# Enigmatisms/AdaPT

Measured on AMD Instinct MI355X. Metric: Msamples/s (W*H*spp/s), unidirectional MIS path tracing, higher is better.
Workload: dtype f32

## Files before the change

adapt_amd/_lib.py:

```python
from __future__ import annotations

import ctypes as C
import os

_HERE = os.path.dirname(os.path.abspath(__file__))
LIB_PATHS = {"fast": os.environ.get("ADAPT_MI_LIB") or os.path.join(_HERE, "libadapt_mi.so"),
             "exact": os.environ.get("ADAPT_MI_LIB_EXACT") or os.path.join(_HERE, "libadapt_mi_exact.so")}
_variant = "exact" if os.environ.get("APT_EXACT", "0") not in ("", "0") else "fast"
LIB_PATH = LIB_PATHS[_variant]

f32p = C.POINTER(C.c_float)
i32p = C.POINTER(C.c_int32)
u32p = C.POINTER(C.c_uint32)
u8p = C.POINTER(C.c_uint8)
f64p = C.POINTER(C.c_double)
APT_N_KERNELS = 5
KERNEL_NAMES = ("generate", "extend", "shade", "shadow", "finalize")


class AptError(RuntimeError):
    pass


class SceneDesc(C.Structure):
# ... 51 lines not shown
    "apt_bvh_wide_export": (C.c_int, [C.c_void_p, u32p, i32p]),
    "apt_bvh_wide_frame": (C.c_int, [C.c_void_p, f32p, f32p]),
    "apt_bvh_free": (None, [C.c_void_p]),
    "apt_bvh_build_device": (C.c_int, [f32p, C.c_int32, i32p, C.c_int32, C.c_int32, C.c_int32, C.POINTER(C.c_void_p), i32p]),
    "apt_bvh_build_linear": (C.c_int, [f32p, C.c_int32, i32p, i32p, C.c_int32, f32p, f32p, C.POINTER(C.c_void_p)]),
    "apt_linear_bvh_counts": (C.c_int, [C.c_void_p, i32p, i32p]),
    "apt_linear_bvh_export": (C.c_int, [C.c_void_p, f32p, f32p, i32p, i32p]),
    "apt_linear_bvh_free": (None, [C.c_void_p]),
    "apt_scene_create": (C.c_int, [C.POINTER(SceneDesc), C.c_int32, C.POINTER(C.c_void_p)]),
    "apt_scene_destroy": (None, [C.c_void_p]),
    "apt_scene_bvh_builder": (C.c_int, [C.c_void_p, i32p]),
    "apt_renderer_create": (C.c_int, [C.c_void_p, C.POINTER(RenderCfg), C.POINTER(C.c_void_p)]),
    "apt_renderer_destroy": (None, [C.c_void_p]),
    "apt_render": (C.c_int, [C.c_void_p, C.c_int32]),
    "apt_synchronize": (C.c_int, [C.c_void_p]),
    "apt_tile_shape": (C.c_int, [C.c_void_p, i32p, i32p]),
    "apt_read_pixels": (C.c_int, [C.c_void_p, f32p]),
    "apt_get_accum": (C.c_int, [C.c_void_p, f32p, i32p]),
    "apt_set_accum": (C.c_int, [C.c_void_p, f32p, C.c_int32]),
    "apt_reset": (C.c_int, [C.c_void_p]),
    "apt_read_transient": (C.c_int, [C.c_void_p, f32p]),
    "apt_set_transient": (C.c_int, [C.c_void_p, f32p]),
    "apt_read_path_lengths": (C.c_int, [C.c_void_p, f32p]),
    "apt_set_path_lengths": (C.c_int, [C.c_void_p, f32p]),
    "apt_read_light_groups": (C.c_int, [C.c_void_p, f32p]),
    "apt_set_light_groups": (C.c_int, [C.c_void_p, f32p]),
    "apt_relight": (C.c_int, [C.c_void_p, f32p, f32p]),
    "apt_read_sample_counts": (C.c_int, [C.c_void_p, i32p, u8p]),
    "apt_read_moments": (C.c_int, [C.c_void_p, f64p]),
    "apt_set_adaptive_state": (C.c_int, [C.c_void_p, i32p, f64p, u8p]),
    "apt_render_aov": (C.c_int, [C.c_void_p, C.c_int32, C.c_int32]),
    "apt_read_aov": (C.c_int, [C.c_void_p, f32p]),
    "apt_set_aov": (C.c_int, [C.c_void_p, f32p]),
    "apt_clear_aov": (C.c_int, [C.c_void_p]),
    "apt_denoise": (C.c_int, [C.c_void_p, C.POINTER(DenoiseCfg), f32p, f32p]),
    "apt_get_stats": (C.c_int, [C.c_void_p, C.POINTER(Stats)]),
    "apt_device_ptr": (C.c_int, [C.c_void_p, C.POINTER(C.c_void_p), i32p]),
    "apt_stream": (C.c_int, [C.c_void_p, C.POINTER(C.c_void_p)]),
    "apt_intersect": (C.c_int, [C.c_void_p, C.c_int32, f32p, f32p, i32p, f32p, f32p]),
    "apt_occluded": (C.c_int, [C.c_void_p, C.c_int32, f32p, f32p, f32p, i32p]),
    "apt_rng_stream": (C.c_int, [C.c_int32, C.c_uint32, C.c_uint32, C.c_uint32, C.c_int32, u32p]),
    "apt_bxdf_probe": (C.c_int, [C.c_int32, C.c_int32, i32p, f32p, f32p, C.c_float, C.c_int32, C.c_uint32, f32p]),
    "apt_medium_probe": (C.c_int, [C.c_int32, C.c_int32, i32p, f32p, C.c_int32, f32p, C.c_uint32, f32p]),
    "apt_volume_probe": (C.c_int, [C.c_int32, C.c_int32, i32p, f32p, f32p, C.c_int32, f32p, C.c_uint32, f32p]),
    "apt_emitter_probe": (C.c_int, [C.c_void_p, C.c_int32, f32p, C.c_uint32, f32p]),
    "apt_texture_probe": (C.c_int, [C.c_void_p, C.c_int32, i32p, f32p, f32p]),
    "apt_surface_maps_probe": (C.c_int, [C.c_void_p, C.c_int32, i32p, f32p, f32p]),
    "apt_transient_bin_probe": (C.c_int, [C.c_int32, C.c_int32, f32p, C.c_float, C.c_float, C.c_int32, i32p]),
    "apt_renderer_info": (C.c_int, [C.c_void_p, i32p, i32p, C.POINTER(C.c_int64), i32p, C.POINTER(C.c_char_p), i32p]),
    "apt_renderer_camera_fused": (C.c_int, [C.c_void_p, i32p]),
    "apt_renderer_light_strips": (C.c_int, [C.c_void_p, i32p]),
    "apt_renderer_record_staged": (C.c_int, [C.c_void_p, i32p]),
    "apt_renderer_live_rows": (C.c_int, [C.c_void_p, i32p]),
    "apt_measure_sclk_mhz": (C.c_int, [C.c_int32, f32p]),
    "apt_last_error": (C.c_char_p, []),
    "apt_version": (C.c_char_p, []),
}

_libs = {}


def use(variant: str) -> str:
    global _variant, LIB_PATH
    if variant not in LIB_PATHS:
        raise ValueError(f"unknown build variant {variant!r}")
    prev, _variant = _variant, variant
    LIB_PATH = LIB_PATHS[variant]
    return prev


def variant() -> str:
    return _variant


def load(variant: str | None = None):
    v = variant or _variant
    if v in _libs:
        return _libs[v]
    path = LIB_PATHS[v]
    if not os.path.exists(path):
        raise AptError(f"{path} is missing: build it with `python -m adapt_amd.build` (needs hipcc); "
                       "adapt_amd has no CPU fallback")
    lib = C.CDLL(path)
    for name, (res, args) in SYMBOLS.items():
        fn = getattr(lib, name)
        fn.restype, fn.argtypes = res, args
    tag = lib.apt_version()
    overridden = os.environ.get("ADAPT_MI_LIB" if v == "fast" else "ADAPT_MI_LIB_EXACT")
    if f"arithmetic: {v}".encode() not in tag and not overridden:
        raise AptError(f"{path} reports {tag!r}: not the {v} build")
    _libs[v] = lib
    return lib


def arithmetic(lib=None) -> str:
    tag = (lib or load()).apt_version().decode()
    return "exact" if "arithmetic: exact" in tag else "fast"


def check(rc: int, what: str = "", lib=None):
    if rc != 0:
        msg = (lib or load()).apt_last_error()
        raise AptError(f"{what or 'adapt_mi'} failed ({rc}): {msg.decode() if msg else '?'}")
```

adapt_amd/csrc/api.hip:

```cpp
#include <hip/hip_runtime.h>
#include <chrono>

#include <algorithm>
#include <cmath>
#include <cstdio>
#include <cstdlib>
#include <cstring>
#include <limits>
#include <memory>
#include <string>
#include <vector>

#include "../../include/adapt_mi.h"
#include "bvh_build.hpp"
#include "shade_stage.hpp"
#include "unit_kernels.hpp"
#include "aov.hpp"
#include "volumetric.hpp"

#define APT_EXPORT extern "C" __attribute__((visibility("default")))

static thread_local std::string g_err;
static int fail(int code, const std::string& msg) { g_err = msg; return code; }
#define HIP_TRY(expr)                                                                              \
    do {                                                                                           \
        hipError_t e_ = (expr);                                                                    \
        if (e_ != hipSuccess)                                                                      \
            return fail(APT_E_HIP, std::string(#expr) + ": " + hipGetErrorString(e_));             \
    } while (0)

typedef void (*shade_fn)(DevScene, Params, Queues, Counters*, ShadeIn, int, int);
typedef void (*shade_traced_fn)(DevScene, Params, Queues, Counters*, int, int);
typedef void (*shade_cam_fn)(DevScene, Params, Queues, Counters*, const unsigned long long*);
typedef void (*shade_tr_fn)(DevScene, Params, Queues, Counters*, ShadeIn, int, int, TransQ);
struct TracedKernels { shade_traced_fn queue[2][2]; shade_cam_fn cam[2]; };
struct ShadeVariant { int bm, sm; const char* name; shade_fn fn; shade_tr_fn transient; TracedKernels traced; };
#if APT_FAST
#define APT_FLAT_FN(...) __VA_ARGS__
#else
#define APT_FLAT_FN(...) nullptr
#endif
#define APT_TRACED_PLAIN(BM, SM, TEX) {{{APT_FLAT_FN(k_shade_traced<BM, SM, TEX>), nullptr}, {nullptr, nullptr}}, {APT_FLAT_FN(k_shade_traced_cam<BM, SM, TEX>), nullptr}}
#define APT_TRACED_LEAN(BM, SM, TEX) {{{APT_FLAT_FN(k_shade_traced_lean<BM, SM>), nullptr}, {APT_FLAT_FN(k_shade_traced_lean_staged<BM, SM>), APT_FLAT_FN(k_shade_traced_lean_staged_live<BM, SM>)}}, \
                                      {APT_FLAT_FN(k_shade_traced_lean_cam<BM, SM>), APT_FLAT_FN(k_shade_traced_lean_cam_live<BM, SM>)}}
#define APT_SHADE_VARIANT(BM, SM, TEX, NAME, TRACED) {BM, SM, NAME, k_shade<BM, SM, TEX>, k_shade_tr<BM, SM, TEX>, APT_TRACED_##TRACED(BM, SM, TEX)}
static const ShadeVariant kShadeVariants[] = {
    APT_SHADE_VARIANT(APT_BX_LAMBERTIAN, APT_SRC_POINT, 0, "lambertian/point", LEAN),
    APT_SHADE_VARIANT(APT_BX_BLINN_PHONG | APT_BX_LAMBERTIAN, APT_SRC_POINT_AREA, 0, "phong+lambertian/point+area", PLAIN),
    APT_SHADE_VARIANT(APT_BX_BLINN_PHONG | APT_BX_LAMBERTIAN | APT_BX_MIRROR | APT_BX_GLASS, APT_SRC_POINT_AREA, 0, "phong+lambertian+mirror+glass/point+area", PLAIN),
    APT_SHADE_VARIANT(APT_BX_ALL, APT_SRC_ALL, 0, "all models", PLAIN),
};
static const ShadeVariant kTexturedShade = APT_SHADE_VARIANT(APT_BX_ALL, APT_SRC_ALL, 1, "all models + image textures", PLAIN);
struct ClassDef { int mask; const char* name; int group, slot, vgroup, vslot; };
constexpr int APT_N_GROUPS = 2, APT_N_VGROUPS = 3, APT_VGROUP_SLOTS = 4;
static constexpr ClassDef kClass[] = {
    {APT_BX_LAMBERTIAN, "lambertian", 0, 0, 0, 0},
    {APT_BX_BLINN_PHONG, "blinn-phong", 1, 0, 2, 0},
    {APT_BX_OREN_NAYAR, "oren-nayar", 1, 1, 0, 1},
    {APT_BX_MIRROR | APT_BX_GLASS | APT_BX_NULL, "delta", 0, 1, 0, 2},
    {APT_BX_MOD_PHONG, "mod-phong", 1, 4, 2, 1},
    {APT_BX_FRESNEL_BLEND, "fresnel-blend", 1, 5, 2, 2},
    {APT_BX_THIN_COAT, "thin-coat", 1, 2, 1, 1},
    {APT_BX_LAMBERT_TRANS, "lambert-trans", 0, 2, 0, 3},
    {APT_BX_MICROFACET, "microfacet", 1, 3, 1, 2},
    {APT_BX_BLINN_PHONG | APT_BX_NO_LOBE, "blinn-phong(no lobe)", 0, 3, 2, 3},
};
constexpr int APT_N_CLASS_DEFS = sizeof(kClass) / sizeof(kClass[0]), APT_CLASS_PHONG = 1, APT_CLASS_PHONG_NO_LOBE = APT_N_CLASS_DEFS - 1;
static constexpr int group_mask(int g, int s) { for (const ClassDef& c : kClass) if (c.group == g && c.slot == s) return c.mask; return 0; }
static constexpr int vgroup_mask(int g, int s) {
    for (const ClassDef& c : kClass) if (c.vgroup == g && c.vslot == s) return c.mask & ~APT_BX_NO_LOBE;
    return (g == 1 && s == 0) ? APT_VEV_MEDIUM_CODE : 0;
}
static constexpr bool class_masks_partition_all() {
    int all = 0;
    for (int c = 0; c < APT_N_CLASS_DEFS - 1; c++) { if (all & kClass[c].mask) return false; all |= kClass[c].mask; }
    return all == APT_BX_ALL;
}
static constexpr bool class_slots_ok() {
    for (int a = 0; a < APT_N_CLASS_DEFS; a++) {
        const ClassDef& c = kClass[a];
        if ((unsigned)c.group >= APT_N_GROUPS || (unsigned)c.slot >= APT_GROUP_SLOTS || (unsigned)c.vgroup >= APT_N_VGROUPS || (unsigned)c.vslot >= APT_VGROUP_SLOTS) return false;
        if (c.vgroup == 1 && c.vslot == 0) return false;
        for (int b = 0; b < a; b++)
            if ((kClass[b].group == c.group && kClass[b].slot == c.slot) || (kClass[b].vgroup == c.vgroup && kClass[b].vslot == c.vslot)) return false;
    }
    return true;
}
static_assert(class_masks_partition_all(), "every surface model belongs to exactly one of the classes in front of the lobe-free one");
static_assert(class_slots_ok(), "every class needs a member slot of its own, inside APT_GROUP_SLOTS / APT_VGROUP_SLOTS, in a surface and in a volumetric group");
static_assert(kClass[APT_CLASS_PHONG].mask == APT_BX_BLINN_PHONG && kClass[APT_CLASS_PHONG_NO_LOBE].mask == (APT_BX_BLINN_PHONG | APT_BX_NO_LOBE), "APT_CLASS_PHONG / APT_CLASS_PHONG_NO_LOBE name these entries");
static int class_of(int is_bsdf, int type, bool no_lobe) {
    const int bit = bx_bit(is_bsdf, type);
    if (bit == APT_BX_BLINN_PHONG && no_lobe) return APT_CLASS_PHONG_NO_LOBE;
    for (int c = 0; c < APT_N_CLASS_DEFS - 1; c++) if (kClass[c].mask & bit) return c;
    return 0;
}
static int group_emitter_set(int src_mask) { return (src_mask & ~APT_SRC_POINT_AREA) == 0 ? 0 : ((src_mask & ~APT_SRC_POINT_SPOT) == 0 ? 2 : 1); }
static int vgroup_emitter_set(int src_mask) { return (src_mask & ~APT_SRC_POINT_AREA) == 0 ? 0 : 1; }
// ... 74 lines not shown
    std::vector<uint8_t> obj_null;
    float box_min[3] = {1e3f, 1e3f, 1e3f}, box_max[3] = {-1e3f, -1e3f, -1e3f};
    int n_classes = 0;
    int class_def[APT_N_CLASS_DEFS] = {};
    int n_prims = 0, n_objects = 0, n_sources = 0, max_obj_prims = 0;
    int bx_mask = 0, src_mask = 0;
    bool has_aabb = false;
    bool has_sweep = false;
};

struct EventPair { hipEvent_t a, b; int kernel; bool own_a; };

struct Lane {
    hipStream_t stream = nullptr;
    DevBuf pool, counters, ovf;
    Queues q{};
    hipEvent_t fin = nullptr;
    LdsPlan plan{};
    Counters* cnt() const { return counters.as<Counters>(); }
};

enum Pipeline { PIPE_STAGED, PIPE_SORTED, PIPE_TRACED, PIPE_VOLUMETRIC };

enum SplitMode { SPLIT_NONE, SPLIT_TRANSIENT, SPLIT_LENGTHS, SPLIT_LIGHTS };
struct SplitWords {
    const char* noun;
    const char* subject;
    bool plural;
    const char* field;
    const char* tag;
};
static constexpr SplitWords kSplit[] = {
    {"", "", false, "", ""},
    {"transient bins", "transient rendering", false, "transient_bins", " [transient]"},
    {"path-length planes", "path-length images", true, "path_lengths", " [path lengths]"},
    {"light-group planes", "light groups", true, "light_groups", " [light groups]"},
};

struct apt_renderer {
    const apt_scene* scene = nullptr;
    apt_render_cfg cfg{};
    Params par{};
    int n_cols = 0, npix = 0, spp_batch = 1;
    int cnt = 0;
    std::vector<Lane> lanes;
    int n_lanes = 1;
    hipStream_t stream() const { return lanes[0].stream; }
    DevBuf accum, scratch, pix_key;
    DevBuf cam_strips;
    int record_stage = 0;
    shade_traced_fn traced_fn = nullptr;
    int live_rows = 0;
    shade_cam_fn traced_cam_fn = nullptr;
    int camera_fuse = 0;
    int light_strips = 0;
    Counters host_counters{};
    int grid_small = 0, grid_trace = 0, nq = APT_MAX_NQ;
    const ShadeVariant* shade = nullptr;
    int trace_mode = TRACE_BVH;
    int trace_nt = BLOCK;
    int trace_items = BLOCK;
    Pipeline pipeline = PIPE_STAGED;
    int dyn_fetch = 0;
    bool tile_ok = false;
    extend_fn extend = nullptr, fix = nullptr;
    int ovf_levels = 0;
    int n_cq = 0;
    int vev_single = 0;
    vev_shade_fn vev_all = nullptr;
    bool vev_live[APT_MAX_CLASSES] = {};
    vev_group_fn vgroup_fn[APT_N_VGROUPS] = {};
    int vgroup_cls[APT_N_VGROUPS][APT_VGROUP_SLOTS] = {};
    group_fn group_fn_[APT_N_GROUPS] = {};
    int group_cls[APT_N_GROUPS][APT_GROUP_SLOTS] = {};
    std::string shade_name;
    size_t lds_bytes = 0, lds_bytes_any = 0;
    int grid_shadow = 0;
    int grid_fix = 0;
    int grid_vshadow = 0;
    int vshadow_nt = BLOCK;
    int vshadow_mode = TRACE_BVH;
    size_t vshadow_lds = 0;
    std::vector<EventPair> pending;
    std::vector<hipEvent_t> free_events;
    std::vector<std::pair<hipStream_t, hipEvent_t>> chain;
    double kernel_ms[APT_N_KERNELS] = {0, 0, 0, 0, 0};
    int64_t launches[APT_N_KERNELS] = {0, 0, 0, 0, 0};
    double render_ms = 0.0;
    hipEvent_t ev_r0 = nullptr, ev_r1 = nullptr;
    bool render_pending = false;
    SplitMode split_mode = SPLIT_NONE;
    bool split() const { return split_mode != SPLIT_NONE; }
    TransQ tq{};
    DevBuf tr_pool;
    DevBuf split_cells;
    group_tr_fn group_tr_[APT_N_GROUPS] = {};
    DevBuf lg_aux;
    int adaptive = 0;
    AdaptQ aq{};
    DevBuf ad_n, ad_s2, ad_active, ad_live;
    std::vector<uint8_t> ad_start;
    uint32_t* ad_live_host = nullptr;
    hipEvent_t ad_ev = nullptr;
    bool ad_pending = false;
    uint32_t n_live = 0;
    DevBuf aov_rec, aov_sum;
// ... 427 lines not shown
        B = (int)((32u << 20) / (uint32_t)r->npix); if (B < 1) B = 1; if (B > 1024) B = 1024;
        const size_t n_cq = c.volumetric ? (size_t)sc->n_classes + 1 : ((sc->n_classes >= 2 && sc->n_classes <= APT_MAX_CLASSES) ? (size_t)sc->n_classes : 1);
        while (B > 1 && n_cq * subcap_of(B) * nq >= ((size_t)1 << 28)) B--;
        size_t free_b = 0, total_b = 0;
        if (hipMemGetInfo(&free_b, &total_b) == hipSuccess) {
            const size_t per_path = 4u * (64u + 16u * n_cq + 11u * (size_t)std::max(1, c.num_shadow_ray));
            while (B > 1 && (size_t)r->npix * (size_t)B * (size_t)r->n_lanes * per_path > free_b / 3) B = (B + 1) / 2;
        }
    }
    r->spp_batch = B;
    const int S = c.num_shadow_ray;
    const size_t subcap = subcap_of(B), cap = subcap * nq;
    if (cap >= (1ull << 31)) { return fail(APT_E_INVALID, "apt_renderer_create: batch too large (spp_per_batch * pixels must stay below 2^31)"); }
    Params& p = r->par;
    memcpy(p.cam_r, c.cam_r, sizeof(p.cam_r)); memcpy(p.cam_t, c.cam_t, sizeof(p.cam_t));
    p.inv_focal = c.inv_focal; p.half_w = c.half_w; p.half_h = c.half_h;
    p.W = c.width; p.H = c.height; p.n_cols = r->n_cols; p.npix = r->npix;
    p.band_width = c.band_width; p.rank = c.rank; p.world = c.world_size;
    p.do_crop = c.do_crop; p.sx = c.start_x; p.ex = c.end_x; p.sy = c.start_y; p.ey = c.end_y;
    p.max_bounce = c.max_bounce; p.S = S; p.inv_S = (S > 0) ? 1.f / (float)S : 1.f;
    p.use_rr = c.use_rr; p.use_mis = c.use_mis; p.anti_alias = c.anti_alias; p.stratified = c.stratified; p.two_sides = c.brdf_two_sides;
    p.rr_bounce_th = c.rr_bounce_th; p.rr_threshold = c.rr_threshold; p.seed = c.seed; p.cap = (uint32_t)cap; p.subcap = (uint32_t)subcap; p.nq = r->nq;
    p.inv_ns = 1.f / (float)sc->n_sources; p.inv_ns1 = (sc->n_sources > 1) ? 1.f / (float)(sc->n_sources - 1) : 1.f;
    p.volumetric_flat = c.volumetric ? 1 : 0; p.fix_par = 0;
    p.pix_bits = 0; while ((1u << p.pix_bits) < (uint32_t)r->npix) p.pix_bits++;
    if (((uint64_t)B << p.pix_bits) > (1ull << 32)) { return fail(APT_E_INVALID, "apt_renderer_create: spp_per_batch x pixels does not fit the 32-bit path id"); }
    std::vector<uint32_t> key((size_t)r->npix);
    for (int lp = 0; lp < r->npix; lp++) {
        const int lc = lp / c.height, j = lp % c.height, lb = lc / c.band_width, w_ = lc % c.band_width;
        const int i = (lb * c.world_size + c.rank) * c.band_width + w_;
        key[(size_t)lp] = (uint32_t)(i * c.height + j);
    }
    hipError_t e_ = upload(r->pix_key, key);
    if (e_ != hipSuccess) { return fail(APT_E_HIP, std::string("upload pix_key: ") + hipGetErrorString(e_)); }
    p.pix_key = r->pix_key.as<uint32_t>();
    return APT_OK;
}

static int small_scene_sweep(const apt_renderer* r) { return (r->tile_ok && r->scene->max_obj_prims >= APT_SWEEP_LIST_MIN) ? TRACE_TILE : TRACE_SWEEP; }
static void pick_traversal(apt_renderer* r) {
    const apt_scene* sc = r->scene;
    r->tile_ok = sc->has_aabb && sc->has_sweep && sc->n_objects <= APT_TILE_MAX_OBJECTS && sc->n_prims < 65536 &&
                 APT_TILE_LDS_BYTES(APT_TILE_NT, sc->n_objects) <= 160 * 1024;
    const bool can[4] = {true, sc->has_aabb && sc->has_sweep, r->tile_ok, sc->has_flat};
    r->trace_mode = sc->has_flat ? TRACE_FLAT
                  : (sc->n_prims <= APT_SWEEP_MAX_PRIMS && can[TRACE_SWEEP]) ? small_scene_sweep(r) : TRACE_BVH;
    if (const char* force = getenv("APT_TRAVERSAL"))
        for (int m = TRACE_BVH; m <= TRACE_FLAT; m++) if (!strcmp(force, kTraversalName[m]) && can[m]) r->trace_mode = m;
    r->dyn_fetch = (r->trace_mode == TRACE_BVH) ? 1 : 0;
    if (const char* f = getenv("APT_DYN_FETCH")) r->dyn_fetch = (atoi(f) != 0 && r->trace_mode == TRACE_BVH) ? 1 : 0;
}

static void pick_traced_kernels(apt_renderer* r) {
    const TracedKernels& t = r->shade->traced;
    const bool traced = r->pipeline == PIPE_TRACED;
    const bool want_stage = !(getenv("APT_RECORD_STAGE") && atoi(getenv("APT_RECORD_STAGE")) == 0);
    const bool want_live = !(getenv("APT_LIVE_ROWS") && atoi(getenv("APT_LIVE_ROWS")) == 0);
    r->record_stage = (traced && want_stage && t.queue[1][0] != nullptr) ? 1 : 0;
    r->live_rows = (traced && want_live && t.queue[1][1] != nullptr && t.cam[1] != nullptr) ? 1 : 0;
    r->traced_fn = t.queue[r->record_stage][r->record_stage & r->live_rows];
    r->traced_cam_fn = t.cam[r->live_rows];
}

static int pick_shading(apt_renderer* r) {
    const apt_scene* sc = r->scene;
    const apt_render_cfg& c = r->cfg;
    Params& p = r->par;
    const int S = c.num_shadow_ray;
    for (const ShadeVariant& v : kShadeVariants)
        if ((sc->bx_mask & ~v.bm) == 0 && (sc->src_mask & ~v.sm) == 0) { r->shade = &v; break; }
    if (!r->shade) { return fail(APT_E_INVALID, "apt_renderer_create: scene uses a material or emitter type the kernels do not know"); }
    const bool textured = sc->dev.tex_i != nullptr;
    if (textured) r->shade = &kTexturedShade;
    const char* env_sorted = getenv("APT_SORTED");
    const bool fits = sc->n_classes <= APT_MAX_CLASSES;
    const bool sorted = !textured && fits && (env_sorted ? (atoi(env_sorted) != 0 && sc->n_classes >= 1) : sc->n_classes >= 2);
    bool want_traced = true;
    if (const char* f = getenv("APT_FUSED")) {
        const int want = atoi(f);
        if (want == 1) fprintf(stderr, "adapt_mi: APT_FUSED=1 (light samples only traced in place) was retired in round 5; running the staged pipeline (APT_FUSED=0). Use 2 for rays traced in place.\n");
        want_traced = want >= 2;
    }
    const bool can_trace = r->trace_mode == TRACE_FLAT && S == 1 && !r->split() && r->shade->traced.queue[0][0] != nullptr;
    r->pipeline = c.volumetric ? PIPE_VOLUMETRIC : (sorted ? PIPE_SORTED : ((can_trace && want_traced) ? PIPE_TRACED : PIPE_STAGED));
    p.traced = (r->pipeline == PIPE_TRACED) ? 1 : 0;
    pick_traced_kernels(r);
    p.nee_vm = (!c.volumetric && !r->split() && r->trace_mode == TRACE_FLAT && S > 1) ? 1 : 0;
    p.l_planes = (!p.nee_vm && S >= 2 && S <= 4) ? S : 1;
    if (r->pipeline == PIPE_VOLUMETRIC) {
        if (c.max_bounce > 255) { return fail(APT_E_INVALID, "apt_renderer_create: the volumetric tracer keeps the bounce count in 8 bits (max_bounce <= 255)"); }
        if (!sc->has_aabb) { return fail(APT_E_INVALID, "apt_renderer_create: the volumetric tracer needs the object boxes (world bound)"); }
        r->vev_single = (textured || sc->n_classes + 1 > APT_MAX_CLASSES) ? 1 : 0;
        const int n_surf = r->vev_single ? 1 : sc->n_classes;
        r->n_cq = n_surf + 1;
        const int smi = vgroup_emitter_set(sc->src_mask), vi = sc->has_volume ? 1 : 0;
        r->vev_all = kVEventAll[smi][vi];
        for (size_t o = 0; o < sc->obj_class.size(); o++)
            if (!sc->obj_null[o]) r->vev_live[r->vev_single ? 0 : sc->obj_class[o]] = true;
        r->vev_live[n_surf] = true;
        for (int g = 0; g < APT_N_VGROUPS; g++) { r->vgroup_fn[g] = kVGroup[smi][vi][g]; for (int k = 0; k < APT_VGROUP_SLOTS; k++) r->vgroup_cls[g][k] = -1; }
        if (!r->vev_single) for (int c = 0; c < n_surf; c++) if (r->vev_live[c]) r->vgroup_cls[kClass[sc->class_def[c]].vgroup][kClass[sc->class_def[c]].vslot] = c;
        r->vgroup_cls[1][0] = n_surf;
        for (int a = 0; a < 3; a++) {
            p.w_min[a] = std::min(c.cam_t[a], sc->box_min[a]) - 0.1f; p.w_max[a] = std::max(c.cam_t[a], sc->box_max[a]) + 0.1f;
        }
        r->shade_name = std::string(sc->has_volume ? "volumetric + grid volume, sorted by event: medium | " : "volumetric, sorted by event: medium | ");
        if (r->vev_single) r->shade_name += "all surface models";
        else for (int c = 0; c < sc->n_classes; c++) r->shade_name += std::string(c ? "+" : "") + kClass[sc->class_def[c]].name;
// ... 61 lines not shown
                                 uint64_t* masks, int32_t masks_cap, int32_t* n_strips, int32_t* n_pairs) {
    if (!prims || !obj_info || !cfg || n_prims <= 0 || n_objects <= 0 || !n_strips || !n_pairs) return fail(APT_E_INVALID, "apt_camera_strips: bad argument");
    apt_render_cfg c = *cfg;
    if (c.world_size <= 0) { c.world_size = 1; c.rank = 0; }
    if (c.band_width <= 0) c.band_width = c.width;
    if (c.width <= 0 || c.height <= 0 || c.rank < 0 || c.rank >= c.world_size || owned_columns(c) <= 0) return fail(APT_E_INVALID, "apt_camera_strips: bad film or rank");
    std::vector<float> st, tb; int cn[7];
    if (apt::build_flat(prims, n_prims, obj_info, n_objects, nullptr, st, tb, cn) != 0) return fail(APT_E_INVALID, "apt_camera_strips: obj_info range outside the primitive array");
    std::vector<uint64_t> m;
    if (apt::camera_strips(prims, n_prims, st, tb, cn, cam_film(c), cull != 0, m) != 0) return fail(APT_E_INVALID, "apt_camera_strips: bad record or film");
    *n_strips = (int32_t)m.size();
    *n_pairs = (cn[0] + cn[1] + 1) / 2 + (cn[2] + cn[3] + 1) / 2 + (cn[4] + cn[5] + 1) / 2 + (cn[6] + 1) / 2;
    if (masks) { if (masks_cap < (int32_t)m.size()) return fail(APT_E_INVALID, "apt_camera_strips: masks buffer too small"); memcpy(masks, m.data(), m.size() * 8); }
    return APT_OK;
}

APT_EXPORT int apt_light_strips(const float* prims, int32_t n_prims, const int32_t* obj_info, int32_t n_objects, const int32_t* src_i, const float* src_f, int32_t n_sources,
                                const apt_render_cfg* cfg, int32_t cull, uint64_t* masks, int32_t masks_cap, int32_t* n_strips, int32_t* n_pairs, float* origin_slack) {
    if (!prims || !obj_info || !src_i || !src_f || !cfg || n_prims <= 0 || n_objects <= 0 || n_sources <= 0 || !n_strips) return fail(APT_E_INVALID, "apt_light_strips: bad argument");
    apt_render_cfg c = *cfg;
    if (c.world_size <= 0) { c.world_size = 1; c.rank = 0; }
    if (c.band_width <= 0) c.band_width = c.width;
    if (c.width <= 0 || c.height <= 0 || c.rank < 0 || c.rank >= c.world_size || owned_columns(c) <= 0) return fail(APT_E_INVALID, "apt_light_strips: bad film or rank");
    std::vector<float> st, tb, pts, pr; std::vector<int32_t> off, tab8, np; std::vector<uint8_t> kp; int cn[7];
    if (apt::build_flat(prims, n_prims, obj_info, n_objects, nullptr, st, tb, cn) != 0) return fail(APT_E_INVALID, "apt_light_strips: obj_info range outside the primitive array");
    apt::emitter_points(prims, obj_info, n_objects, src_i, src_f, n_sources, pts, off);
    if (apt::flat_occluders(prims, n_prims, st, tb, cn, pts.data(), off.data(), n_sources, true, pr, tab8, kp) != 0) return fail(APT_E_INVALID, "apt_light_strips: bad record");
    std::vector<uint64_t> m; double slack = 0.0;
    if (apt::light_strips(prims, n_prims, st, tb, cn, cam_film(c), pts.data(), off.data(), n_sources, kp.data(), cull != 0, m, np, &slack) != 0) return fail(APT_E_INVALID, "apt_light_strips: bad record or film");
    *n_strips = (int32_t)((owned_columns(c) * c.height + 63) / 64);
    if (n_pairs) memcpy(n_pairs, np.data(), np.size() * 4);
    if (origin_slack) *origin_slack = (float)slack;
    if (masks) { if (masks_cap < (int32_t)m.size()) return fail(APT_E_INVALID, "apt_light_strips: masks buffer too small"); memcpy(masks, m.data(), m.size() * 8); }
    return APT_OK;
}

static int make_lanes(apt_renderer* r) {
    const apt_scene* sc = r->scene;
    const Params& p = r->par;
    const size_t cap = p.cap, sh_subcap = (size_t)p.subcap * (size_t)(p.S > 0 ? p.S : 1), sh_cap = sh_subcap * (size_t)p.nq;
    const int ncls = r->n_cq;
    if (cap >= ((size_t)1 << 30) || sh_cap >= ((size_t)1 << 30)) { return fail(APT_E_INVALID, "apt_renderer_create: batch too large (queue capacity must stay below 2^30 slots)"); }
    if (r->pipeline == PIPE_TRACED && cap >= ((size_t)1 << 28)) { return fail(APT_E_INVALID, "apt_renderer_create: batch too large (rays traced in place address 16-byte slots with 32-bit byte offsets: capacity must stay below 2^28)"); }
    if ((size_t)ncls * cap >= ((size_t)1 << 28)) { return fail(APT_E_INVALID, "apt_renderer_create: batch too large (packed class queues address 16-byte slots with 32-bit byte offsets: classes x capacity must stay below 2^28)"); }
    const bool staged = r->pipeline != PIPE_TRACED, tr_uv = !staged && (sc->dev.has_vn || sc->dev.tex_i != nullptr);
    const bool walk_lists = r->pipeline == PIPE_VOLUMETRIC && sc->has_null_surface;
    const size_t l_planes = (size_t)p.l_planes;
    auto carve = [&](float* base, Queues& q) -> size_t {
        size_t at = 0;
        auto take = [&](size_t n) { float* x = base ? base + at : nullptr; at += n; return x; };
        for (int k = 0; k < 2; k++) { q.ray_o[k] = (k == 0 || staged) ? take(3 * cap) : nullptr; q.ray_d[k] = (k == 0 || staged) ? take(3 * cap) : nullptr; }
        q.hit_t = take(cap); q.hit_prim = (int*)take(cap); q.hit_u = take(cap); q.hit_v = take(cap);
        for (int k = 0; k < 2; k++) {
            for (int a = 0; a < 4; a++) q.tr[k][a] = staged ? nullptr : (float4*)take(4 * cap);
            q.tr_uv[k] = tr_uv ? (float2*)take(2 * cap) : nullptr;
        }
        q.tr_ncls = staged ? 0 : 1; q.tr_stage_top = staged ? 0 : 1;
        q.fix_ext = (r->trace_mode == TRACE_FLAT) ? (uint32_t*)take(cap) : nullptr; q.fix_sh = (r->trace_mode == TRACE_FLAT) ? (uint32_t*)take(sh_cap) : nullptr;
        for (int k = 0; k < 2; k++) { q.thr[k] = staged ? take(3 * cap) : nullptr; q.id[k] = staged ? (uint32_t*)take(cap) : nullptr; q.meta[k] = staged ? (uint32_t*)take(cap) : nullptr; q.pdf[k] = staged ? take(cap) : nullptr; }
        q.L = take(4 * cap * l_planes);
        q.sh_o = take(3 * sh_cap); q.sh_d = take(3 * sh_cap); q.sh_tmax = take(sh_cap); q.sh_c = take(3 * sh_cap); q.sh_id = (uint32_t*)take(sh_cap);
        q.sh_cap = (uint32_t)sh_cap; q.sh_subcap = (uint32_t)sh_subcap;
        q.sh_walk[0] = walk_lists ? (uint32_t*)take(sh_cap) : nullptr; q.sh_walk[1] = walk_lists ? (uint32_t*)take(sh_cap) : nullptr;
        q.n_classes = ncls;
        for (int a = 0; a < 4; a++) q.cq[a] = (ncls > 0 && staged) ? (float4*)take(4 * cap * (size_t)ncls) : nullptr;
        return at;
    };
    Queues sizing{};
    const size_t pool_bytes = carve(nullptr, sizing) * 4;
    r->lanes.resize((size_t)r->n_lanes);
    hipError_t e;
    for (Lane& ln : r->lanes) {
        if ((e = ln.pool.alloc(pool_bytes)) != hipSuccess || (e = hipMemset(ln.pool.p, 0, pool_bytes)) != hipSuccess || (e = ln.counters.alloc(sizeof(Counters))) != hipSuccess)
            return fail(APT_E_NOMEM, std::string(&ln == &r->lanes[0] ? "queue pool: " : "queue pool (lane): ") + hipGetErrorString(e));
        carve(ln.pool.as<float>(), ln.q);
    }
    HIP_TRY(hipDeviceSynchronize());
    if ((e = r->accum.alloc((size_t)r->npix * 12)) != hipSuccess || (e = r->scratch.alloc((size_t)r->npix * 12)) != hipSuccess) { return fail(APT_E_NOMEM, std::string("framebuffer: ") + hipGetErrorString(e)); }
    for (Lane& ln : r->lanes) {
        HIP_TRY(hipStreamCreateWithFlags(&ln.stream, hipStreamNonBlocking));
        HIP_TRY(hipEventCreateWithFlags(&ln.fin, hipEventDisableTiming));
        HIP_TRY(hipMemsetAsync(ln.counters.p, 0, sizeof(Counters), ln.stream));
    }
    HIP_TRY(hipMemsetAsync(r->accum.p, 0, (size_t)r->npix * 12, r->stream()));
    HIP_TRY(hipEventCreate(&r->ev_r0)); HIP_TRY(hipEventCreate(&r->ev_r1));
    return APT_OK;
}

static void transient_window(TransQ& t, int32_t n_bins, float min_time, float interval) {
    t.n_bins = n_bins; t.min_time = min_time; t.interval = interval;
    t.max_time = (float)((double)min_time + (double)interval * (double)n_bins);
}

static int adaptive_restart(apt_renderer* r) {
    HIP_TRY(hipMemsetAsync(r->ad_n.p, 0, r->ad_n.bytes, r->stream()));
    HIP_TRY(hipMemsetAsync(r->ad_s2.p, 0, r->ad_s2.bytes, r->stream()));
    HIP_TRY(hipMemcpyAsync(r->ad_active.p, r->ad_start.data(), r->ad_start.size(), hipMemcpyHostToDevice, r->stream()));
    HIP_TRY(hipStreamSynchronize(r->stream()));
    r->n_live = 0;
    for (uint8_t a : r->ad_start) r->n_live += a;
    r->ad_pending = false;
    return APT_OK;
}
static int make_adaptive(apt_renderer* r) {
    if (!r->adaptive) return APT_OK;
    const apt_render_cfg& c = r->cfg;
    const size_t n = (size_t)r->npix;
// ... 341 lines not shown
                    }
                }
                is.cur ^= 1;
            }
            return APT_OK;
        };
        for (Issued& is : round) if (int rc = iterate(is, std::max(1, is.p.max_bounce))) return rc;
        for (Issued& is : round) {
            Lane& ln = *is.ln;
            if (r->scene->has_null_surface) {
                Counters* cnt = ln.cnt();
                unsigned long long live = 0;
                for (int k = 0; k < 4096; k++) {
                    unchain(r, ln.stream); HIP_TRY(hipMemcpyAsync(r->host_counters.n_active[is.cur], cnt->n_active[is.cur], sizeof(cnt->n_active[is.cur]), hipMemcpyDeviceToHost, ln.stream));
                    HIP_TRY(hipStreamSynchronize(ln.stream));
                    live = 0;
                    for (int sq = 0; sq < nq; sq++) live += r->host_counters.n_active[is.cur][sq * CNT_PAD];
                    if (!live) break;
                    if (int rc = iterate(is, 2)) return rc;
                }
                if (live) return fail(APT_E_STATE, "apt_render: paths still crossing null surfaces after 8192 extra iterations (a closed loop of null surfaces?)");
            }
            if (int rc = finalize_batch(r, ln, is.p, prev_fin)) return rc;
        }
    }
    return APT_OK;
}

static int render_surface(apt_renderer* r, int32_t n_spp) {
    const DevScene& sc = r->scene->dev;
    const int nq = r->nq;
    int done = 0, batch = 0;
    hipEvent_t prev_fin = nullptr;
    const int batch_cap = lane_batch(r, n_spp);
    while (done < n_spp) {
        const int B = (n_spp - done < batch_cap) ? (n_spp - done) : batch_cap;
        Lane& ln = r->lanes[(size_t)(batch % r->n_lanes)];
        hipStream_t st = ln.stream;
        const Queues& q = ln.q;
        Counters* cnt = ln.cnt();
        Params p = r->par; p.cnt_base = r->cnt; p.spp_batch = B;
        const size_t total = (size_t)r->npix * (size_t)B;
        if (int rc = begin_batch(r, ln)) return rc;
#if APT_FAST
        if (r->pipeline == PIPE_TRACED) {
            const unsigned long long* strips = r->cam_strips.as<unsigned long long>();
            int cur = 0, b0 = 0;
            if (r->camera_fuse) {
                { LaunchTimer t(r, APT_K_SHADE, st); hipLaunchKernelGGL(r->traced_cam_fn, dim3(grid_for(total, r->grid_small, nq)), dim3(BLOCK), 0, st, sc, p, q, cnt, strips); }
                { LaunchTimer t(r, APT_K_SHADE, st); hipLaunchKernelGGL(r->traced_fn, dim3(r->grid_fix), dim3(BLOCK), 0, st, sc, p, q, cnt, 0, 0); }
                cur = 1; b0 = 1;
            } else {
                LaunchTimer t(r, APT_K_GENERATE, st);
                if (r->adaptive) hipLaunchKernelGGL(k_generate_trace_ad, dim3(grid_for(total, r->grid_small, 1)), dim3(BLOCK), 0, st, sc, p, q, cnt, (const uint8_t*)r->aq.active, strips);
                else hipLaunchKernelGGL(k_generate_trace, dim3(grid_for(total, r->grid_small, 1)), dim3(BLOCK), 0, st, sc, p, q, cnt, strips);
            }
            for (int b = b0; b < p.max_bounce; b++) {
                { LaunchTimer t(r, APT_K_SHADE, st); hipLaunchKernelGGL(r->traced_fn, dim3(grid_for(total, r->grid_small, nq)), dim3(BLOCK), 0, st, sc, p, q, cnt, cur, b); }
                cur ^= 1;
            }
            if (p.max_bounce > 0) { LaunchTimer t(r, APT_K_SHADOW, st, false); hipLaunchKernelGGL(r->fix, dim3(r->grid_fix), dim3(BLOCK), 0, st, sc, p, q, cnt, cur, (const uint32_t*)cnt->n_active[cur], ln.plan); }
        } else
#endif
        {
        {
            LaunchTimer t(r, APT_K_GENERATE, st);
            if (r->adaptive) hipLaunchKernelGGL(k_generate_ad, dim3(grid_for(total, r->grid_small, 1)), dim3(BLOCK), 0, st, p, q, cnt, (const uint8_t*)r->aq.active);
            else hipLaunchKernelGGL(k_generate, dim3(grid_for(total, r->grid_small, 1)), dim3(BLOCK), 0, st, p, q, cnt);
        }
        auto bin = [&](int settled) {
            LaunchTimer t(r, APT_K_FINALIZE, st, false);
            const dim3 grid(grid_for((size_t)r->npix, r->grid_small, 1));
            float4* cells = r->split_cells.as<float4>();
            switch (r->split_mode) {
                case SPLIT_TRANSIENT: hipLaunchKernelGGL(k_bin_transient, grid, dim3(BLOCK), 0, st, p, q, r->tq, r->accum.as<float>()); break;
                case SPLIT_LENGTHS: hipLaunchKernelGGL(k_bin_lengths, grid, dim3(BLOCK), 0, st, p, q, r->tq, cells, settled, r->accum.as<float>()); break;
                case SPLIT_LIGHTS: hipLaunchKernelGGL(k_bin_lights, grid, dim3(BLOCK), 0, st, p, q, r->tq, cells, r->scene->n_sources, r->lg_aux.as<unsigned int>(), r->accum.as<float>()); break;
                case SPLIT_NONE: break;
            }
        };
        int cur = 0;
        for (int b = 0; b < p.max_bounce; b++) {
            if (r->dyn_fetch && !(p.S > 0)) { unchain(r, st); HIP_TRY(hipMemsetAsync(cnt->n_work[0], 0, sizeof(cnt->n_work[0]), st)); }
            launch_extend(r, ln, p, total, cur);
            if (r->split() && r->trace_mode == TRACE_FLAT && b > 0) bin(b - 1);
            if (r->pipeline != PIPE_SORTED) {
                ShadeIn in = {q.ray_o[cur], q.ray_d[cur], q.thr[cur], q.id[cur], q.meta[cur], q.pdf[cur],
                              q.hit_t, q.hit_prim, q.hit_u, q.hit_v, (const uint32_t*)cnt->n_active[cur]};
                LaunchTimer t(r, APT_K_SHADE, st);
                if (r->split()) hipLaunchKernelGGL(r->shade->transient, dim3(grid_for(total, r->grid_small, nq)), dim3(BLOCK), 0, st, sc, p, q, cnt, in, cur, b, r->tq);
                else hipLaunchKernelGGL(r->shade->fn, dim3(grid_for(total, r->grid_small, nq)), dim3(BLOCK), 0, st, sc, p, q, cnt, in, cur, b);
            } else {
                for (int g = 0; g < APT_N_GROUPS; g++) {
                    GroupIn gi; bool any = false;
                    for (int k = 0; k < APT_GROUP_SLOTS; k++) { const int c = r->group_cls[g][k]; gi.cls[k] = c; gi.counts[k] = c >= 0 ? (const uint32_t*)cnt->n_cls[c] : nullptr; any = any || c >= 0; }
                    if (!any) continue;
                    LaunchTimer t(r, APT_K_SHADE, st);
                    if (r->split()) hipLaunchKernelGGL(r->group_tr_[g], dim3(grid_for(total, r->grid_small, nq)), dim3(BLOCK), 0, st, sc, p, q, cnt, gi, cur, b, r->tq);
                    else hipLaunchKernelGGL(r->group_fn_[g], dim3(grid_for(total, r->grid_small, nq)), dim3(BLOCK), 0, st, sc, p, q, cnt, gi, cur, b);
                }
                if (p.S <= 0) { unchain(r, st); HIP_TRY(hipMemsetAsync(cnt->n_cls, 0, sizeof(cnt->n_cls), st)); }
            }
            if (p.S > 0 && r->dyn_fetch) {
                LaunchTimer t(r, APT_K_SHADOW, st); hipLaunchKernelGGL(k_shadow_dyn, dim3(grid_for(total * (size_t)p.S, r->grid_shadow, nq, r->trace_items)), dim3(r->trace_nt), r->lds_bytes_any, st, sc, p, q, cnt, ln.plan);
            } else if (p.S > 0) {
                p.fix_par = cur;
                LaunchTimer t(r, APT_K_SHADOW, st); hipLaunchKernelGGL(kShadow[r->trace_mode], dim3(grid_for(total * (size_t)p.S, r->grid_shadow, nq, r->trace_items)), dim3(r->trace_nt), r->lds_bytes_any, st, sc, p, q, cnt, ln.plan);
            }
// ... 522 lines not shown
}
APT_EXPORT int apt_surface_maps_probe(const apt_scene* sc, int32_t n, const int32_t* prim_first, const float* bary, float* out7) {
    if (!sc || n <= 0 || !prim_first || !bary || !out7) return fail(APT_E_INVALID, "apt_surface_maps_probe: bad argument");
    if (!sc->dev.tex_i) return fail(APT_E_INVALID, "apt_surface_maps_probe: the scene has no textures");
    for (int k = 0; k < n; k++)
        if (const int p = prim_first[2 * (size_t)k]; p < 0 || p >= sc->n_prims) return fail(APT_E_INVALID, "apt_surface_maps_probe: no such primitive");
    Probe pr; if (int rc = pr.begin("apt_surface_maps_probe", sc->device, (size_t)n * 28)) return rc;
    HIP_TRY(upload(pr.in[0], prim_first, 2 * (size_t)n)); HIP_TRY(upload(pr.in[1], bary, 2 * (size_t)n));
    hipLaunchKernelGGL(k_surface_maps_probe, dim3((n + 63) / 64), dim3(64), 0, 0, sc->dev, n, pr.in[0].as<int>(), pr.in[1].as<float>(), pr.out.as<float>());
    return pr.finish(out7);
}
APT_EXPORT int apt_measure_sclk_mhz(int32_t device, float* mhz) {
    if (!mhz) return fail(APT_E_INVALID, "apt_measure_sclk_mhz: bad argument");
    if (int rc = use_device("apt_measure_sclk_mhz", device)) return rc;
    hipDeviceProp_t prop;
    HIP_TRY(hipGetDeviceProperties(&prop, device));
    const int grid = std::max(1, prop.multiProcessorCount) * 8, n_waves = grid * (BLOCK / 64);
    DevBuf out, sink;
    HIP_TRY(out.alloc((size_t)n_waves * 16)); HIP_TRY(sink.alloc(16));
    for (int pass = 0; pass < 2; pass++) {
        hipLaunchKernelGGL(k_clock_probe, dim3(grid), dim3(BLOCK), 0, 0, 20000, 1.0f, out.as<unsigned long long>(), sink.as<float>());
        HIP_TRY(hipGetLastError());
        HIP_TRY(hipDeviceSynchronize());
    }
    std::vector<unsigned long long> h((size_t)n_waves * 2);
    HIP_TRY(hipMemcpy(h.data(), out.p, h.size() * 8, hipMemcpyDeviceToHost));
    std::vector<double> r;
    for (int w = 0; w < n_waves; w++) if (h[2 * (size_t)w + 1] > 0) r.push_back(100.0 * (double)h[2 * (size_t)w] / (double)h[2 * (size_t)w + 1]);
    if (r.empty()) return fail(APT_E_STATE, "apt_measure_sclk_mhz: the wall clock did not advance");
    std::nth_element(r.begin(), r.begin() + r.size() / 2, r.end());
    *mhz = (float)r[r.size() / 2];
    return APT_OK;
}
APT_EXPORT int apt_renderer_camera_fused(const apt_renderer* r, int32_t* out) {
    if (!r || !out) return fail(APT_E_INVALID, "apt_renderer_camera_fused: null argument");
    *out = r->camera_fuse;
    return APT_OK;
}
APT_EXPORT int apt_renderer_light_strips(const apt_renderer* r, int32_t* out) {
    if (!r || !out) return fail(APT_E_INVALID, "apt_renderer_light_strips: null argument");
    *out = r->light_strips;
    return APT_OK;
}
APT_EXPORT int apt_renderer_record_staged(const apt_renderer* r, int32_t* out) {
    if (!r || !out) return fail(APT_E_INVALID, "apt_renderer_record_staged: null argument");
    *out = r->record_stage;
    return APT_OK;
}
APT_EXPORT int apt_renderer_live_rows(const apt_renderer* r, int32_t* out) {
    if (!r || !out) return fail(APT_E_INVALID, "apt_renderer_live_rows: null argument");
    *out = r->live_rows;
    return APT_OK;
}
APT_EXPORT int apt_renderer_info(const apt_renderer* r, int32_t* spp_batch, int32_t* n_subqueues, int64_t* queue_bytes, int32_t* lds_bytes, const char** shade_variant, int32_t* trace_mode) {
    if (!r) return fail(APT_E_INVALID, "apt_renderer_info: null handle");
    if (spp_batch) *spp_batch = r->spp_batch;
    if (n_subqueues) *n_subqueues = r->nq;
    if (queue_bytes) *queue_bytes = (int64_t)r->lanes[0].pool.bytes * (int64_t)r->lanes.size();
    if (lds_bytes) *lds_bytes = (int32_t)r->lds_bytes;
    if (shade_variant) *shade_variant = r->shade_name.c_str();
    if (trace_mode) *trace_mode = r->trace_mode;
    return APT_OK;
}
```

adapt_amd/csrc/shade_stage.hpp:

```cpp
#pragma once
#include "stages.hpp"

APT_D float ti_fmod(float a, float b) { float q = floorf(a / b); return a - b * q; }
APT_D f3 mix3(f3 a, f3 b, float t) { return a * (1.0f - t) + b * t; }
APT_D f3 texture_query(const DevScene& sc, int map, int obj, float u, float v) {
    const int* ti_ = sc.tex_i + 15 * obj + 5 * map; const float* tf = sc.tex_f + 6 * obj + 2 * map;
    const float w = (float)ti_[3], h = (float)ti_[4];
    const float scaled_u = ti_fmod((u * tf[0]) * w, w - 1.f), scaled_v = ti_fmod((v * tf[1]) * h, h - 1.f);
    float floor_u = floorf(scaled_u), floor_v = floorf(scaled_v);
    const float ratio_u = fmaxf(scaled_u - floor_u, 0.f), ratio_v = fmaxf(scaled_v - floor_v, 0.f);
    floor_u = fminf(fmaxf(floor_u, 0.f), w - 1.f); floor_v = fminf(fmaxf(floor_v, 0.f), h - 1.f);
    const float ceil_u = fminf(floor_u + 1.f, w - 1.f), ceil_v = fminf(floor_v + 1.f, h - 1.f);
    const int fu = (int)(floor_u + (float)ti_[1]), fv = (int)(floor_v + (float)ti_[2]), cu = (int)(ceil_u + (float)ti_[1]), cv = (int)(ceil_v + (float)ti_[2]);
    const float* img = sc.atlas[map]; const int W = sc.atlas_w[map];
    const float* r0 = img + (size_t)fv * W * 3; const float* r1 = img + (size_t)cv * W * 3;
    const f3 q_ff = ld3(r0 + 3 * fu), q_cf = ld3(r0 + 3 * cu), q_fc = ld3(r1 + 3 * fu), q_cc = ld3(r1 + 3 * cu);
    return mix3(mix3(q_ff, q_cf, ratio_u), mix3(q_fc, q_cc, ratio_u), ratio_v);
}
APT_D bool get_uv_item(const DevScene& sc, int map, int obj, int prim, float bu, float bv, f3& out) {
    if (sc.atlas[map] == nullptr || !(sc.tex_i[15 * obj + 5 * map] > -255)) return false;
    const float* uv = sc.uvs + 6 * prim;
    const float w0 = 1.f - bu - bv;
    const float gu = (uv[2] * bu + uv[4] * bv) + uv[0] * w0, gv = (uv[3] * bu + uv[5] * bv) + uv[1] * w0;
    out = texture_query(sc, map, obj, gu, gv);
    return true;
}
APT_D int surface_maps(const DevScene& sc, Hit& it, int prim, float bu, float bv, bool first_hit, f3& k_d) {
    int applied = 0; f3 tx;
    if (first_hit) {
        if (get_uv_item(sc, 1, it.obj_id, prim, bu, bv, tx)) { m33 R; rotation_between(mk3(0.f, 1.f, 0.f), it.n_g, R); it.n_s = mul(R, tx); applied |= 2; }
        if (get_uv_item(sc, 2, it.obj_id, prim, bu, bv, tx)) { it.n_s = delocalize(it.n_s, tx); applied |= 4; }
    }
    if (get_uv_item(sc, 0, it.obj_id, prim, bu, bv, tx)) { k_d = tx; applied |= 1; }
    return applied;
}

APT_D void build_hit_rec(const DevScene& sc, float4 ra, float4 rb, int prim, float t, float u, float v, f3 o, f3 d, Hit& it, int& hit_light, f3& k_d, bool with_vn = true);
APT_D void build_hit(const DevScene& sc, int prim, float t, float u, float v, f3 o, f3 d, Hit& it, int& hit_light, f3& k_d) {
    build_hit_rec(sc, sc.prim_shade[2 * prim], sc.prim_shade[2 * prim + 1], prim, t, u, v, o, d, it, hit_light, k_d);
}
APT_D void build_hit_rec(const DevScene& sc, float4 ra, float4 rb, int prim, float t, float u, float v, f3 o, f3 d, Hit& it, int& hit_light, f3& k_d, bool with_vn) {
    const int code = __float_as_int(ra.w);
    it.prim_id = prim; it.min_depth = t;
    it.obj_id = (code < 0) ? ~code : code;
    hit_light = __float_as_int(rb.x);
    k_d = mk3(rb.y, rb.z, rb.w);
    if (code < 0) {
        it.n_g = normalize((o + d * t) - mk3(ra.x, ra.y, ra.z));
        it.n_s = it.n_g;
    } else {
        it.n_g = mk3(ra.x, ra.y, ra.z);
        if (with_vn && sc.has_vn) {
            const float4 v0 = sc.vnormals[3 * prim], v1 = sc.vnormals[3 * prim + 1], v2 = sc.vnormals[3 * prim + 2];
            it.n_s = (mk3(v0.x, v0.y, v0.z) * (1.f - u - v) + mk3(v1.x, v1.y, v1.z) * u) + mk3(v2.x, v2.y, v2.z) * v;
        } else it.n_s = it.n_g;
    }
}
APT_D void build_hit(const DevScene& sc, int prim, float t, float u, float v, f3 o, f3 d, Hit& it) {
    int light; f3 kd; build_hit(sc, prim, t, u, v, o, d, it, light, kd);
}

#if APT_FAST
APT_D void fix_prologue(const DevScene& sc, const Params& p, const Queues& q, Counters* cnt, int cur, int sq, int bounce) {
    const uint32_t epoch = (uint32_t)bounce + 1u;
    const int ncls = q.tr_ncls;
    uint32_t* n_def_p = &cnt->n_tr[bounce % 3][ncls][sq * CNT_PAD]; uint32_t* n_sh_p = &cnt->n_fix_sh[cur ^ 1][sq * CNT_PAD];
    const uint32_t n_def = __hip_atomic_load(n_def_p, __ATOMIC_RELAXED, __HIP_MEMORY_SCOPE_AGENT), n_sh = min(__hip_atomic_load(n_sh_p, __ATOMIC_RELAXED, __HIP_MEMORY_SCOPE_AGENT), q.sh_subcap);
    __builtin_amdgcn_fence(__ATOMIC_ACQUIRE, "workgroup");
    uint32_t old = __hip_atomic_load(&cnt->fix_claim[sq * CNT_PAD], __ATOMIC_RELAXED, __HIP_MEMORY_SCOPE_AGENT);
    if (old < epoch) {
        if ((n_def | n_sh) == 0u) return;
        if (lane_id() == 0) old = atomicMax(&cnt->fix_claim[sq * CNT_PAD], epoch);
        old = (uint32_t)__builtin_amdgcn_readlane((int)old, 0);
    }
    if (old >= epoch) {
        while (__hip_atomic_load(&cnt->fix_done[sq * CNT_PAD], __ATOMIC_ACQUIRE, __HIP_MEMORY_SCOPE_AGENT) < epoch) __builtin_amdgcn_s_sleep(16);
        return;
    }
    const uint32_t qbase = (uint32_t)sq * p.subcap, sh_qbase = (uint32_t)sq * q.sh_subcap;
    const bool need_uv = sc.has_vn || sc.tex_i != nullptr;
    for (uint32_t base = 0; base < n_def; base += 64u) {
        const uint32_t li = base + lane_id(); const bool valid = li < n_def;
        const uint32_t lj = valid ? li : n_def - 1u;
        const uint32_t io = (q.tr_stage_top ? qbase + p.subcap - n_def + lj : (uint32_t)ncls * p.cap + qbase + lj) << 4;
        const float4 ra = ldq(q.tr[cur][0], io), rb = ldq(q.tr[cur][1], io), rc = ldq(q.tr[cur][2], io), rd = ldq(q.tr[cur][3], io);
        const f3 o = mk3(ra.x, ra.y, ra.z), d = mk3(rb.x, rb.y, rb.z);
        HitRec r0, r1; r0.t = r1.t = 1e7f; r0.prim = r1.prim = -1; r0.u = r0.v = r1.u = r1.v = 0.f;
        int c0, c1;
        flat_closest2(sc.flat, sc.sweep, sc.prim_class, o, d, o, d, r0, r1, c0, c1);
        if (valid && r0.prim >= 0) {
            const int oc = ncls > 1 ? c0 : 0;
            const uint32_t pos = atomicAdd(&cnt->n_tr[bounce % 3][oc][sq * CNT_PAD], 1u);
            const uint32_t slot = (uint32_t)oc * p.cap + qbase + pos, so = slot << 4;
            stq(q.tr[cur][0], so, make_float4(ra.x, ra.y, ra.z, r0.t));
            stq(q.tr[cur][1], so, make_float4(rb.x, rb.y, rb.z, __uint_as_float((__float_as_uint(rb.w) & ~0xffu) | (uint32_t)r0.prim)));
            stq(q.tr[cur][2], so, rc); stq(q.tr[cur][3], so, rd);
            if (need_uv) { float2 uv_; uv_.x = r0.u; uv_.y = r0.v; stq(q.tr_uv[cur], slot << 3, uv_); }
        } else if (valid && !(rd.x == 0.f && rd.y == 0.f && rd.z == 0.f)) {
            add_radiance(q.L, p.cap, radiance_slot(p, __float_as_uint(rc.w)), mk3(rd.x, rd.y, rd.z), true);
        }
    }
    uint32_t t_lit = 0;
    for (uint32_t base = 0; base < n_sh; base += 64u) {
        const uint32_t li = base + lane_id(); const bool valid = li < n_sh;
        const uint32_t io = (sh_qbase + (valid ? li : n_sh - 1u)) << 2;
        const f3 o = ld3q(q.sh_o, q.sh_cap, io), d = ld3q(q.sh_d, q.sh_cap, io), c = ld3q(q.sh_c, q.sh_cap, io);
        const float dist = ldq(q.sh_tmax, io); const uint32_t slot = ldq(q.sh_id, io);
        bool occ, occ_b;
        const float lim = shadow_limit(dist);
        flat_any2(sc.flat, sc.sweep, o, d, o, d, lim, lim, occ, occ_b);
        const bool weird = !(isfinite(c.x) && isfinite(c.y) && isfinite(c.z));
        const bool add = valid && (!occ || weird);
        for (unsigned long long m = __ballot(add); m != 0ull; m &= m - 1ull) {
            if ((int)lane_id() == __ffsll((long long)m) - 1) add_radiance(q.L, p.cap, slot, occ ? c * 0.f : c, true);
        }
        t_lit += (valid && !occ) ? 1u : 0u;
    }
    flush_stat(t_lit, &cnt->stats[sq][ST_LIT]);
    if (lane_id() == 0) __hip_atomic_store(n_sh_p, 0u, __ATOMIC_RELAXED, __HIP_MEMORY_SCOPE_AGENT);
    __threadfence();
    if (lane_id() == 0) __hip_atomic_store(&cnt->fix_done[sq * CNT_PAD], epoch, __ATOMIC_RELEASE, __HIP_MEMORY_SCOPE_AGENT);
}
#endif
struct ShadeArgs3 { DevScene sc; Params p; Queues q; };
typedef const __attribute__((address_space(4))) ShadeArgs3* args3_ptr;
APT_D args3_ptr kernel_args3() { return (args3_ptr)__builtin_amdgcn_kernarg_segment_ptr(); }
APT_D const ShadeArgs3* args_fresh(args3_ptr a) {
    asm volatile("" : "+s"(a));
    return (const ShadeArgs3*)a;
}
#define APT_ARGS_PHASE() (A_ = args_fresh(A0))
struct Vertex {
    f3 o, d, thr, hit_point; uint32_t id, l_off, draw0; float emission_weight;
    Hit it; int hit_light; DevBxdf bx;
};
APT_D void vertex_reset(Vertex& vx) {
    vx.o = splat3(0.f); vx.d = mk3(0.f, 0.f, 1.f); vx.thr = splat3(0.f); vx.hit_point = splat3(0.f); vx.id = 0; vx.l_off = 0; vx.draw0 = 0; vx.emission_weight = 1.0f;
    vx.it.obj_id = -1; vx.it.prim_id = -1; vx.it.n_s = vx.it.n_g = mk3(1.f, 0.f, 0.f); vx.it.min_depth = 0.f; vx.hit_light = -1;
    vx.bx.type = 1; vx.bx.is_delta = 0; vx.bx.is_bsdf = 0; vx.bx.k_d = vx.bx.k_s = vx.bx.k_g = vx.bx.mean = splat3(0.f); vx.bx.ior = 1.f;
}
template <int BM, int SM, int TEX, typename RNG>
APT_D bool open_vertex(const ShadeArgs3* A_, Vertex& vx, RNG& rng, int prim, f3 rec_kd, uint32_t meta, float ray_pdf, float2 uv, int bounce, const uint32_t* jitter_tail = nullptr) {
    const bool was_spec = (meta >> 24) & 1u;
    if (BM == APT_BX_LAMBERTIAN) vx.bx.k_d = rec_kd;
    else vx.bx = ld_bxdf_lane((A_->sc).bxdf + vx.it.obj_id);
    if (TEX && (A_->sc).tex_i != nullptr) surface_maps((A_->sc), vx.it, prim, uv.x, uv.y, bounce == 0, vx.bx.k_d);
    const uint32_t lp = vx.id & ((1u << (A_->p).pix_bits) - 1u), s = vx.id >> (A_->p).pix_bits;
    vx.l_off = radiance_slot((A_->p), vx.id);
    vx.draw0 = meta & 0xffffu;
    const uint32_t key0 = ((A_->p).world == 1) ? lp : ldq((A_->p).pix_key, lp << 2), ctr0 = (uint32_t)((A_->p).cnt_base + (int)s + 1);
    rng_init(rng, key0, (A_->p).seed, ctr0, vx.draw0);
    if (bounce > 0 && (A_->p).use_mis) {
// ... 81 lines not shown
    else alive = alive && !(max3(vx.thr) < 1e-4f);
    const bool relight = vx.hit_light >= 0 && (A_->sc).n_sources > 1;
    const bool have_first = jitter_tail != nullptr && (A_->p).anti_alias != 0;
    uint32_t c[4] = {0u, 0u, have_first ? jitter_tail[0] : 0u, have_first ? jitter_tail[1] : 0u};
    const bool live = window_open(rng, key0, (A_->p).seed, ctr0, vx.draw0, roulette, mx, relight, c, have_first, [alive](bool v) { return __any(v && alive) != 0; });
    if (roulette) vx.thr = vx.thr * srcp(mx + 1e-7f);
    return alive && live;
}
template <int BM, int SM, typename R>
APT_D LightSample sample_light_live(const ShadeArgs3* A_, Vertex& vx, R& rng, const EmitterGeom& geom, const DevSrc src_only, bool active) {
    LightSample ls;
    const int ns = (A_->sc).n_sources;
    int sidx = rng_int(rng);
    sidx = (ns == 1) ? 0 : pymod(sidx, ns);
    float emitter_pdf = (A_->p).inv_ns;
    if (ns <= 1) active = active && vx.hit_light < 0;
    else if (vx.hit_light >= 0) {
        sidx = rng_int(rng);
        sidx = (ns == 2) ? 0 : pymod(sidx, ns - 1);
        if (sidx >= vx.hit_light) sidx += 1;
        emitter_pdf = (A_->p).inv_ns1;
    }
    DevSrc src = src_only;
    if (ns != 1) src = (A_->sc).src[sidx];
    ls.src = sidx;
    f3 shadow_int; float direct_pdf;
    const f3 to_emitter = emitter_sample_hit<SM>(src, geom, vx.hit_point, rng, shadow_int, direct_pdf) - vx.hit_point;
    ls.dist = fnorm(to_emitter);
    ls.dir = fdiv3(to_emitter, ls.dist);
    ls.sampled = active;
    const f3 direct_spec = surface_eval<BM>(vx.bx, vx.it, vx.d, ls.dir, (A_->sc).world_ior, (A_->p).two_sides);
    ls.mis_w = 1.0f;
    if ((A_->p).use_mis && !(src.bool_bits & 0x01)) ls.mis_w = balance(emitter_pdf * direct_pdf, surface_pdf<BM>(vx.bx, vx.it, ls.dir, vx.d, (A_->sc).world_ior, (A_->p).two_sides));
    ls.poisoned = active && isnan(ls.mis_w);
    f3 c = (direct_spec * shadow_int) * ls.mis_w;
    if (ns != 1) c = fdiv3(c, emitter_pdf);
    ls.contrib = (c * (A_->p).inv_S) * vx.thr;
    ls.want = active && !ls.poisoned && !(ls.contrib.x == 0.f && ls.contrib.y == 0.f && ls.contrib.z == 0.f);
    return ls;
}
APT_D void shadow_store(const Queues& q, uint32_t so, f3 o, f3 dir, float dist, f3 contrib) {
    st3q(q.sh_o, q.sh_cap, so, o); st3q(q.sh_d, q.sh_cap, so, dir); stq(q.sh_tmax, so, dist); st3q(q.sh_c, q.sh_cap, so, contrib);
}
struct ShadeTally { uint32_t shade, shadow, poison; };
APT_D void tally_flush(const ShadeTally& t, const uint32_t* s_draws, Counters* cnt, int sq) {
    flush_uniform(t.shade, &cnt->stats[sq][ST_SHADE]);
    flush_uniform(t.shadow, &cnt->stats[sq][ST_SHADOW]);
    if (lane_id() == 0 && s_draws[threadIdx.x >> 6]) atomicAdd(&cnt->stats[sq][ST_DRAWS], (unsigned long long)s_draws[threadIdx.x >> 6]);
    flush_uniform(t.poison, &cnt->stats[sq][ST_POISON]);
}
#if APT_FAST
APT_D uint32_t row_lane(uint32_t b, uint32_t n) { return min(b + threadIdx.x, n - 1u); }
struct RecordPlanes { const float4 *a, *b, *c, *d; };
APT_D uint32_t prefetch_prim(const RecordPlanes& tr, uint32_t qbase, uint32_t b, uint32_t n) { return ldq(reinterpret_cast<const uint32_t*>(tr.b), ((qbase + row_lane(b, n)) << 4) + 12u); }
struct StagedRecord { rec4* rec; rec4* prim; };
APT_D StagedRecord staged_record_open(const ShadeArgs3* A_) {
    __shared__ rec4 s_stage[(BLOCK / 64) * 4 * 64]; __shared__ rec4 s_shade[2 * APT_FLAT_MAX_PRIMS];
    static_assert(2 * APT_FLAT_MAX_PRIMS <= BLOCK, "one shading-record word per thread");
    if ((int)threadIdx.x < 2 * min((A_->sc).n_prims, APT_FLAT_MAX_PRIMS)) { const float4 w_ = (A_->sc).prim_shade[threadIdx.x]; s_shade[threadIdx.x] = rec4{w_.x, w_.y, w_.z, w_.w}; }
    __syncthreads();
    return StagedRecord{s_stage + (threadIdx.x >> 6) * (4 * 64), s_shade};
}
APT_D void stage_row(const StagedRecord& s, const RecordPlanes& tr, uint32_t qbase, uint32_t b, uint32_t n, int bounce) {
    const uint32_t off = (qbase + row_lane(b, n)) << 4;
    stage_plane(tr.a, off, s.rec); stage_plane(tr.b, off, s.rec + 64); stage_plane(tr.c, off, s.rec + 128);
    if (bounce > 0) stage_plane(tr.d, off, s.rec + 192);
}
APT_D void staged_row_read(const StagedRecord& s, float4& a, float4& b, float4& c, float4& d, float4& ra, float4& rb) {
    rec4 sa, sb, sc_, sd, pa, pb;
    staged_read(s.rec + lane_id(), sa, sb, sc_, sd);
    staged_read2(s.prim + 2 * max(tr_prim(__float_as_uint(sb.w)), 0), pa, pb);
    a = make_float4(sa.x, sa.y, sa.z, sa.w); b = make_float4(sb.x, sb.y, sb.z, sb.w); c = make_float4(sc_.x, sc_.y, sc_.z, sc_.w); d = make_float4(sd.x, sd.y, sd.z, sd.w);
    ra = make_float4(pa.x, pa.y, pa.z, pa.w); rb = make_float4(pb.x, pb.y, pb.z, pb.w);
}
struct RowTop { unsigned long long wait, rows, loop0; };
APT_D void staged_wait_stamped(RowTop& rt, bool row) {
#ifdef APT_ROWTOP_STATS
    const unsigned long long t0_ = __builtin_amdgcn_s_memtime(); staged_wait(); rt.wait += __builtin_amdgcn_s_memtime() - t0_; rt.rows += row ? 1u : 0u;
#else
    staged_wait();
#endif
}
template <bool UNORDERED> APT_D void tally_draws(uint32_t* s_draws, uint32_t n) { if constexpr (UNORDERED) lds_add_unordered(&s_draws[threadIdx.x >> 6], n); else atomicAdd(&s_draws[threadIdx.x >> 6], n); }
APT_D void unpack_record(float4 a, float4 b, float4 c, Vertex& vx) { vx.o = mk3(a.x, a.y, a.z); vx.d = mk3(b.x, b.y, b.z); vx.thr = mk3(c.x, c.y, c.z); vx.id = __float_as_uint(c.w); }
template <int BM, int SM, int TEX, bool REC, typename RNG>
APT_D bool open_record(const ShadeArgs3* A_, Vertex& vx, RNG& rng, float4 a, float4 b, float4 c, uint32_t pm, float4 ra, float4 rb, int cur, uint32_t idx, float ray_pdf, int bounce) {
    unpack_record(a, b, c, vx);
    const int prim = tr_prim(pm);
    if (prim < 0) return false;
    f3 rec_kd; float2 uv; uv.x = uv.y = 0.f;
    if ((A_->sc).has_vn || (TEX && (A_->sc).tex_i != nullptr)) uv = ldq((A_->q).tr_uv[cur], idx << 3);
    if (REC) build_hit_rec((A_->sc), ra, rb, prim, a.w, uv.x, uv.y, vx.o, vx.d, vx.it, vx.hit_light, rec_kd);
    else build_hit((A_->sc), prim, a.w, uv.x, uv.y, vx.o, vx.d, vx.it, vx.hit_light, rec_kd);
    return open_vertex<BM, SM, TEX>(A_, vx, rng, prim, rec_kd, tr_meta(pm, (uint32_t)bounce), ray_pdf, uv, bounce);
}
template <int BM, int SM, typename RNG>
APT_D bool open_record_live(const ShadeArgs3* A_, Vertex& vx, RNG& rng, float4 a, float4 b, float4 c, float4 d, float4 ra, float4 rb, int cur, uint32_t idx, int bounce, bool alive, uint32_t* s_draws, f3& Lc) {
    if (bounce > 0) Lc = mk3(d.x, d.y, d.z);
    unpack_record(a, b, c, vx);
    const uint32_t pm = __float_as_uint(b.w); const int prim = tr_prim(pm);
    alive = alive && prim >= 0;
    f3 rec_kd; float2 uv; uv.x = uv.y = 0.f;
    if ((A_->sc).has_vn) { if (alive) uv = ldq((A_->q).tr_uv[cur], idx << 3); }
    build_hit_rec((A_->sc), ra, rb, max(prim, 0), a.w, uv.x, uv.y, vx.o, vx.d, vx.it, vx.hit_light, rec_kd);
    const bool opened = alive; alive = open_vertex_live<BM, SM>(A_, vx, rng, rec_kd, pm, bounce, alive);
    if (opened && !alive && rng.draw != vx.draw0) tally_draws<true>(s_draws, rng.draw - vx.draw0);
    return alive;
}
APT_D uint32_t cam_wave(const ShadeArgs3* A_, uint32_t pos, int q) { return (uint32_t)__builtin_amdgcn_readfirstlane((int)(pos >> 6)) * (uint32_t)(A_->p).nq + (uint32_t)q; }
APT_D uint32_t cam_path(const ShadeArgs3* A_, uint32_t id_, bool zero, uint32_t& s, int& i, int& j) {
    const uint32_t lp = id_ % (uint32_t)(A_->p).npix; s = id_ / (uint32_t)(A_->p).npix;
    local_to_global((A_->p), lp, i, j);
    if (zero) for (int pl = 0; pl < (A_->p).l_planes; pl++) stL((A_->q).L, (A_->p).cap, (id_ << 2) | (uint32_t)pl, splat3(0.f));
    return (s << (A_->p).pix_bits) | lp;
}
APT_D bool cam_sweep(const ShadeArgs3* A_, const unsigned long long* strips, uint32_t w, bool valid, f3 cam_o, f3 dir, float& c_t, int& c_idx) {
    int c_run = -1; c_t = 0.f; c_idx = -1;
    if (__any(valid)) c_idx = flat_closest1<true>((A_->sc).flat, cam_o, dir, 1e7f, c_t, c_run, camera_strip_mask((A_->p), strips, w));
    return valid && (c_run >= 0 || flat_needs_cull((A_->sc).flat, dir));
}
struct StagedRayWords { float t; int prim; float u, v, one, zero, one_d; };
template <typename Words>
APT_D void stage_camera_ray(const ShadeArgs3* A_, Counters* cnt, int q, uint32_t qbase, bool c_defer, f3 cam_o, f3 dir, uint32_t draws, uint32_t id, Words&& words) {
    if (!__any(c_defer)) return;
    const int ncls = (A_->q).tr_ncls; const uint32_t dpos = wave_append(c_defer, &cnt->n_tr[0][ncls][q * CNT_PAD]);
    if (c_defer) {
        const uint32_t slot = (A_->q).tr_stage_top ? qbase + (A_->p).subcap - 1u - dpos : (uint32_t)ncls * (A_->p).cap + qbase + dpos, so = slot << 4;
        const StagedRayWords w = words();
        stq((A_->q).tr[0][0], so, make_float4(cam_o.x, cam_o.y, cam_o.z, w.t));
        stq((A_->q).tr[0][1], so, make_float4(dir.x, dir.y, dir.z, __uint_as_float(tr_pack(w.prim, draws, false))));
        stq((A_->q).tr[0][2], so, make_float4(w.one, w.one, w.one, __uint_as_float(id)));
        stq((A_->q).tr[0][3], so, make_float4(w.zero, w.zero, w.zero, w.one_d));
        if ((A_->sc).has_vn || (A_->sc).tex_i != nullptr) { float2 uv_; uv_.x = w.u; uv_.y = w.v; stq((A_->q).tr_uv[0], slot << 3, uv_); }
    }
}
template <int BM, int SM, int TEX, bool WINDOW, typename RNG>
APT_D bool camera_vertex(const ShadeArgs3* A_, Counters* cnt, int q, uint32_t qbase, uint32_t pos, bool in_row, uint32_t cam_total, const unsigned long long* strips, Vertex& vx, RNG& rng, uint32_t* s_draws, uint32_t& t_samples, uint32_t& t_extend, bool& entry) {
    const uint32_t w = cam_wave(A_, pos, q), id_ = w * 64u + lane_id(); const bool valid = in_row && id_ < cam_total;
    f3 dir = mk3(0.f, 0.f, 1.f); uint32_t draws = 0, jitter_tail[2] = {0u, 0u};
    if (valid) { uint32_t s; int i, j; vx.id = cam_path(A_, id_, true, s, i, j); dir = camera_ray_dir((A_->p), i, j, s, draws, WINDOW ? jitter_tail : nullptr); }
    if (draws) atomicAdd(&s_draws[threadIdx.x >> 6], draws);
    const f3 cam_o = mk3((A_->p).cam_t[0], (A_->p).cam_t[1], (A_->p).cam_t[2]);
    float c_t; int c_idx, hit_cls = 0;
    const bool c_defer = cam_sweep(A_, strips, w, valid, cam_o, dir, c_t, c_idx);
    HitRec hr; hr.t = 1e7f; hr.prim = -1; hr.u = hr.v = 0.f;
    if (valid && !c_defer && c_idx >= 0) flat_resolve((A_->sc).flat, c_idx, c_t, cam_o, dir, hr, hit_cls);
    { const uint32_t nv = wave_count(valid); t_samples += nv; t_extend += nv; }
    stage_camera_ray(A_, cnt, q, qbase, c_defer, cam_o, dir, draws, vx.id, [&] {
        float one = 1.f;
        if (WINDOW) asm volatile("" : "+v"(one));
        return StagedRayWords{hr.t, hr.prim, hr.u, hr.v, 1.f, 0.f, one};
    });
    entry = valid && !c_defer; bool alive = entry && hr.prim >= 0;
    if (alive) {
        vx.o = cam_o; vx.d = dir; vx.thr = splat3(1.f);
        f3 rec_kd; float2 uv; uv.x = hr.u; uv.y = hr.v;
        build_hit((A_->sc), hr.prim, hr.t, uv.x, uv.y, vx.o, vx.d, vx.it, vx.hit_light, rec_kd);
        alive = open_vertex<BM, SM, TEX>(A_, vx, rng, hr.prim, rec_kd, tr_meta(tr_pack(hr.prim, draws, false), 0u), 1.f, uv, 0, WINDOW ? jitter_tail : nullptr);
    }
    return alive;
}
template <int BM, int SM, bool WINDOW, typename RNG>
APT_D bool camera_vertex_live(const ShadeArgs3* A_, Counters* cnt, int q, uint32_t qbase, uint32_t pos, bool in_row, uint32_t cam_total, const unsigned long long* strips, Vertex& vx, RNG& rng, uint32_t* s_draws, uint32_t& t_samples, uint32_t& t_extend, bool& entry) {
    const uint32_t w = cam_wave(A_, pos, q), id_ = w * 64u + lane_id(); const bool valid = in_row && id_ < cam_total;
    uint32_t draws = 0, jitter_tail[2] = {0u, 0u}, s; int i, j;
    vx.id = cam_path(A_, id_, valid, s, i, j);
    const f3 dir = camera_ray_dir((A_->p), i, j, s, draws, WINDOW ? jitter_tail : nullptr);
    if (valid && draws) atomicAdd(&s_draws[threadIdx.x >> 6], draws);
    const f3 cam_o = mk3((A_->p).cam_t[0], (A_->p).cam_t[1], (A_->p).cam_t[2]);
    float c_t; int c_idx, hit_cls = 0;
    const bool c_defer = cam_sweep(A_, strips, w, valid, cam_o, dir, c_t, c_idx);
    HitRec hr;
    flat_resolve((A_->sc).flat, max(c_idx, 0), c_t, cam_o, dir, hr, hit_cls);
    { const uint32_t nv = wave_count(valid); t_samples += nv; t_extend += nv; }
    stage_camera_ray(A_, cnt, q, qbase, c_defer, cam_o, dir, draws, vx.id, [&] {
        float one = 1.f, far_ = 1e7f, zero = 0.f;
        asm volatile("" : "+v"(one), "+v"(far_), "+v"(zero));
        return StagedRayWords{far_, -1, zero, zero, one, zero, one};
    });
    entry = valid && !c_defer; bool alive = entry && c_idx >= 0 && hr.prim >= 0;
    vx.o = cam_o; vx.d = dir; vx.thr = splat3(1.f);
    f3 rec_kd; build_hit((A_->sc), max(hr.prim, 0), hr.t, hr.u, hr.v, vx.o, vx.d, vx.it, vx.hit_light, rec_kd);
    const bool opened = alive; alive = open_vertex_live<BM, SM>(A_, vx, rng, rec_kd, tr_pack(hr.prim, draws, false), 0, alive, WINDOW ? jitter_tail : nullptr);
    if (opened && !alive && rng.draw != vx.draw0) tally_draws<false>(s_draws, rng.draw - vx.draw0);
    return alive;
}
template <int BM, int SM, bool LDS_TALLY, typename RNG>
APT_D bool scatter(const ShadeArgs3* A_, Vertex& vx, RNG& rng, bool alive, int bounce, uint32_t* s_draws, f3& Lc, f3& new_d, float& new_pdf, bool& is_spec) {
    bool cont = false;
    if (alive) { new_d = emit_and_scatter<BM, SM>(A_, vx, rng, new_pdf, is_spec, [&](f3 add) { Lc = Lc + add; }); cont = (bounce + 1) < (A_->p).max_bounce; }
    if (rng.draw != vx.draw0) tally_draws<LDS_TALLY>(s_draws, rng.draw - vx.draw0);
    return cont;
}
template <int BM, int SM, bool LDS_TALLY, typename RNG>
APT_D bool scatter_live(const ShadeArgs3* A_, Vertex& vx, RNG& rng, bool alive, int bounce, uint32_t* s_draws, f3& Lc, f3& new_d, float& new_pdf, bool& is_spec) {
    bool cont = false;
    if ((bounce + 1) < (A_->p).max_bounce) { new_d = emit_and_scatter<BM, SM>(A_, vx, rng, new_pdf, is_spec, [&](f3 add) { Lc = Lc + add; }); cont = alive; }
    else rng.draw += 2u;
    if (alive) tally_draws<LDS_TALLY>(s_draws, rng.draw - vx.draw0);
    return cont;
}
APT_D int pick_occluder_list(const ShadeArgs3* A_, const LightSample& f) {
    int occ_e = 0;
    if ((A_->sc).n_sources != 1) {
        const unsigned long long wm = __ballot(f.want);
        occ_e = -1;
        if (wm != 0ull) { const int e0 = __builtin_amdgcn_readlane(f.src, __ffsll((long long)wm) - 1); if (!__any(f.want && f.src != e0)) occ_e = e0; }
    }
    return occ_e;
}
struct Continuation { float t, u, v; int hit, q; TrAppend app; };
APT_D bool trace_continuation(const ShadeArgs3* A_, const Vertex& vx, f3 new_d, bool cont, uint32_t* next_counter, uint32_t& t_extend, Continuation& ct) {
    ct.t = 0.f; ct.hit = -1; ct.u = ct.v = 0.f; int tr_idx = -1, tr_run = -1, hit_cls = 0;
    if (__any(cont)) tr_idx = flat_closest1((A_->sc).flat, vx.hit_point, new_d, 1e7f, ct.t, tr_run);
    const bool tr_defer = cont && (tr_run >= 0 || flat_needs_cull((A_->sc).flat, new_d));
    t_extend += wave_count(cont);
    cont = cont && (tr_idx >= 0 || tr_defer);
    if (cont && !tr_defer) { HitRec hr; flat_resolve((A_->sc).flat, tr_idx, ct.t, vx.hit_point, new_d, hr, hit_cls); ct.hit = hr.prim; ct.u = hr.u; ct.v = hr.v; }
    ct.q = !cont ? -1 : (tr_defer ? 1 : 0);
    const Append a_ = append_issue(ct.q == 0, next_counter); ct.app.raw = a_.raw; ct.app.rank = rank_in(a_.m);
    return cont;
}
template <bool CAM>
APT_D void sweep_light_sample(const ShadeArgs3* A_, Counters* cnt, const Vertex& vx, const LightSample& f, int occ_e, int cur, int q, uint32_t sh_qbase, uint32_t pos, const unsigned long long* strips, f3& Lc, uint32_t& t_traced, uint32_t& t_lit) {
    const bool defer = f.want && flat_needs_cull((A_->sc).flat, f.dir); bool occ = false;
    if (__any(f.want && !defer)) {
        const FlatList ls = (occ_e >= 0) ? flat_occ_list((A_->sc).flat, occ_e) : flat_full_list((A_->sc).flat);
        if constexpr (CAM) {
            unsigned long long lmask = ~0ull;
            if (occ_e >= 0 && occ_e < APT_LIGHT_STRIP_EMITTERS) lmask = light_strip_mask((A_->p), strips, cam_wave(A_, pos, q), occ_e);
            occ = flat_any1<true>(ls, vx.hit_point, f.dir, shadow_limit(f.dist), lmask);
        } else occ = flat_any1(ls, vx.hit_point, f.dir, shadow_limit(f.dist));
    }
    if (__any(defer)) {
        const uint32_t spos = wave_append(defer, &cnt->n_fix_sh[cur][q * CNT_PAD]);
        if (defer && spos < (A_->q).sh_subcap) { const uint32_t so = (sh_qbase + spos) << 2; shadow_store((A_->q), so, vx.hit_point, f.dir, f.dist, f.contrib); stq((A_->q).sh_id, so, vx.l_off); }
    }
    const bool traced = f.want && !defer;
    if (traced) {
        const bool weird = !(isfinite(f.contrib.x) && isfinite(f.contrib.y) && isfinite(f.contrib.z));
        if (!occ || weird) Lc = Lc + (occ ? f.contrib * 0.f : f.contrib);
    }
    t_traced += wave_count(f.want); t_lit += wave_count(traced && !occ);
}
APT_D void append_record(const ShadeArgs3* A_, int nxt, uint32_t qbase, uint32_t* next_counter, const Continuation& ct, bool cont, const Vertex& vx, f3 new_d, uint32_t draw, bool is_spec, f3 Lc, float new_pdf) {
    uint32_t npos = (uint32_t)__builtin_amdgcn_readlane((int)ct.app.raw, 0) + ct.app.rank;
    if (__any(ct.q == 1)) { const uint32_t dpos = wave_append(ct.q == 1, next_counter + APT_MAX_NQ * CNT_PAD); if (ct.q == 1) npos = dpos; }
    if (cont) {
        const uint32_t slot = (ct.q == 1) ? qbase + (A_->p).subcap - 1u - npos : qbase + npos, so = slot << 4;
        stq((A_->q).tr[nxt][0], so, make_float4(vx.hit_point.x, vx.hit_point.y, vx.hit_point.z, ct.t));
        stq((A_->q).tr[nxt][1], so, make_float4(new_d.x, new_d.y, new_d.z, __uint_as_float(tr_pack(ct.hit, draw, is_spec))));
        stq((A_->q).tr[nxt][2], so, make_float4(vx.thr.x, vx.thr.y, vx.thr.z, __uint_as_float(vx.id)));
        stq((A_->q).tr[nxt][3], so, make_float4(Lc.x, Lc.y, Lc.z, new_pdf));
        if ((A_->sc).has_vn || (A_->sc).tex_i != nullptr) { float2 uv_; uv_.x = ct.u; uv_.y = ct.v; stq((A_->q).tr_uv[nxt], slot << 3, uv_); }
    }
}
APT_D void end_path(const ShadeArgs3* A_, bool ended, uint32_t id, f3 Lc) { if (ended && !(Lc.x == 0.f && Lc.y == 0.f && Lc.z == 0.f)) add_radiance((A_->q).L, (A_->p).cap, radiance_slot((A_->p), id), Lc, true); }
template <int BM, int SM, int TEX, bool CAM = false, bool STAGE = false, bool LIVE_ = false>
APT_D void shade_traced(args3_ptr A0, Counters* cnt, int cur_, int bounce_, const unsigned long long* strips = nullptr) {
    static_assert(!(CAM && STAGE), "a camera-fed row loads no record");
    static_assert(!LIVE_ || ((CAM || STAGE) && TEX == 0), "live rows: the staged and the camera-fed form of the lean kernels");
    constexpr bool LIVE = LIVE_ && APT_DRAW_WINDOW != 0;
    const ShadeArgs3* A_ = args_fresh(A0);
    const int cur = CAM ? 0 : cur_, bounce = CAM ? 0 : bounce_, nxt = cur ^ 1;
    const SubLoop sl = sub_loop((A_->p).nq);
    const uint32_t qbase = (uint32_t)sl.q * (A_->p).subcap, sh_qbase = (uint32_t)sl.q * (A_->q).sh_subcap;
    uint32_t* next_counter = &cnt->n_tr[(bounce + 1) % 3][0][sl.q * CNT_PAD];
    if (sl.first == 0 && threadIdx.x == 0) { cnt->n_tr[(bounce + 2) % 3][0][sl.q * CNT_PAD] = 0; cnt->n_tr[(bounce + 2) % 3][(A_->q).tr_ncls][sl.q * CNT_PAD] = 0; }
    const EmitterGeom geom = {(A_->sc).precom, (A_->sc).normals, (A_->sc).obj_info};
    __shared__ uint32_t s_draws[BLOCK / 64];
    if (lane_id() == 0) s_draws[threadIdx.x >> 6] = 0;
    ShadeTally tl = {0u, 0u, 0u}; uint32_t t_traced = 0, t_lit = 0, t_extend = 0, t_samples = 0;
#ifdef APT_NEAR_STATS
    uint32_t t_near = 0;
#endif
    RowTop rt = {0ull, 0ull, 0ull};
    constexpr bool WINDOW = APT_DRAW_WINDOW != 0 && BM == APT_BX_LAMBERTIAN && !(SM & APT_SRC_AREA);
    typedef typename std::conditional<WINDOW, DrawWindow, Philox>::type Rng;
    constexpr bool PFP = TEX == 0 && !CAM && !STAGE;
    static_assert(APT_FLAT_MAX_PRIMS < (int)TR_NO_PRIM, "the packed record keeps the hit primitive in 8 bits");
    const RecordPlanes tr = {(A_->q).tr[cur][0], (A_->q).tr[cur][1], (A_->q).tr[cur][2], (A_->q).tr[cur][3]};
    StagedRecord stage = {nullptr, nullptr};
    if constexpr (STAGE) stage = staged_record_open(A_);
    uint32_t n, cam_total = 0;
    if constexpr (CAM) {
        cam_total = (uint32_t)(A_->p).npix * (uint32_t)(A_->p).spp_batch;
        const uint32_t n_waves = (cam_total + 63u) / 64u, nq_ = (uint32_t)(A_->p).nq;
        n = n_waves > (uint32_t)sl.q ? ((n_waves - (uint32_t)sl.q + nq_ - 1u) / nq_) * 64u : 0u;
    } else {
        fix_prologue((A_->sc), (A_->p), (A_->q), cnt, cur, sl.q, bounce);
        n = __hip_atomic_load(&cnt->n_tr[bounce % 3][0][sl.q * CNT_PAD], __ATOMIC_RELAXED, __HIP_MEMORY_SCOPE_AGENT);
    }
    uint32_t pf_pm = 0;
    if (PFP && n > 0) pf_pm = prefetch_prim(tr, qbase, sl.first, n);
    if (STAGE && sl.first < n) { stage_row(stage, tr, qbase, sl.first, n, bounce); staged_wait_stamped(rt, false); }
#ifdef APT_ROWTOP_STATS
    rt.loop0 = __builtin_amdgcn_s_memtime();
#endif
    for (uint32_t base = sl.first; base < n; base += sl.stride) {
        APT_ARGS_PHASE();
        const uint32_t pos = base + threadIdx.x, idx = qbase + pos;
        bool alive = pos < n;
        const uint32_t cu_pm = pf_pm; float4 cu_ra = make_float4(0.f, 0.f, 0.f, 0.f), cu_rb = cu_ra;
        if (PFP) { const int rp = max(tr_prim(cu_pm), 0); cu_ra = (A_->sc).prim_shade[2 * rp]; cu_rb = (A_->sc).prim_shade[2 * rp + 1]; pf_pm = prefetch_prim(tr, qbase, base + sl.stride, n); }
        Vertex vx; vertex_reset(vx); Rng rng; rng_init(rng, 0u, 0u, 0u, 0u);
        f3 Lc = splat3(0.f);
        bool entry = alive; float ray_pdf = 1.f;
        if constexpr (CAM && LIVE) alive = camera_vertex_live<BM, SM, WINDOW>(A_, cnt, sl.q, qbase, pos, alive, cam_total, strips, vx, rng, s_draws, t_samples, t_extend, entry);
        else if constexpr (CAM) alive = camera_vertex<BM, SM, TEX, WINDOW>(A_, cnt, sl.q, qbase, pos, alive, cam_total, strips, vx, rng, s_draws, t_samples, t_extend, entry);
        else if constexpr (STAGE) {
            float4 a, b_, c, d;
            staged_row_read(stage, a, b_, c, d, cu_ra, cu_rb);
            if constexpr (LIVE) alive = open_record_live<BM, SM>(A_, vx, rng, a, b_, c, d, cu_ra, cu_rb, cur, idx, bounce, alive, s_draws, Lc);
            else if (alive) {
                if (bounce > 0) { Lc = mk3(d.x, d.y, d.z); if (SM & APT_SRC_AREA) ray_pdf = d.w; }
                alive = open_record<BM, SM, TEX, true>(A_, vx, rng, a, b_, c, __float_as_uint(b_.w), cu_ra, cu_rb, cur, idx, ray_pdf, bounce);
            }
        } else {
            if (alive && bounce > 0) { const float4 d = ldq(tr.d, idx << 4); Lc = mk3(d.x, d.y, d.z); if (SM & APT_SRC_AREA) ray_pdf = d.w; }
            if (alive) {
                const float4 a = ldq(tr.a, idx << 4), b_ = ldq(tr.b, idx << 4), c = ldq(tr.c, idx << 4);
#ifdef APT_ROWTOP_STATS
                staged_wait_stamped(rt, true);
#endif
                alive = open_record<BM, SM, TEX, PFP>(A_, vx, rng, a, b_, c, PFP ? cu_pm : __float_as_uint(b_.w), cu_ra, cu_rb, cur, idx, ray_pdf, bounce);
            }
        }
        tl.shade += wave_count(alive);
#ifdef APT_NEAR_STATS
        t_near += wave_count(alive && bounce > 0 && vx.it.min_depth < 2e-3f);
#endif
        if constexpr (LIVE) vx.hit_point = vx.d * vx.it.min_depth + vx.o;
        else if (alive) vx.hit_point = vx.d * vx.it.min_depth + vx.o;
        APT_ARGS_PHASE();
        bool break_flag = false; DevSrc src_only;
        if ((A_->sc).n_sources == 1) src_only = ld_src_uniform((A_->sc).src);
        LightSample f;
        if constexpr (LIVE) f = sample_light_live<BM, SM>(A_, vx, rng, geom, src_only, alive);
        else f = sample_light<BM, SM, false>(A_, vx, rng, geom, src_only, alive, break_flag);
        if (f.poisoned) Lc = splat3(f.mis_w);
        tl.shadow += wave_count(f.sampled); tl.poison += wave_count(f.poisoned);
        const int occ_e = pick_occluder_list(A_, f);
        if constexpr (STAGE) if (base + sl.stride < n) stage_row(stage, tr, qbase, base + sl.stride, n, bounce);
        APT_ARGS_PHASE();
        bool cont, is_spec = false; float new_pdf = 1.f; f3 new_d = mk3(0.f, 1.f, 0.f);
        if constexpr (LIVE) cont = scatter_live<BM, SM, STAGE>(A_, vx, rng, alive, bounce, s_draws, Lc, new_d, new_pdf, is_spec);
        else cont = scatter<BM, SM, STAGE>(A_, vx, rng, alive, bounce, s_draws, Lc, new_d, new_pdf, is_spec);
        APT_ARGS_PHASE();
        Continuation ct; cont = trace_continuation(A_, vx, new_d, cont, next_counter, t_extend, ct);
        APT_ARGS_PHASE();
        sweep_light_sample<CAM>(A_, cnt, vx, f, occ_e, cur, sl.q, sh_qbase, pos, strips, Lc, t_traced, t_lit);
        if constexpr (STAGE) staged_wait_stamped(rt, true);
        append_record(A_, nxt, qbase, next_counter, ct, cont, vx, new_d, rng.draw, is_spec, Lc, new_pdf);
        end_path(A_, !cont && entry, vx.id, Lc);
    }
    flush_uniform(t_traced, &cnt->stats[sl.q][ST_SHADOW_TRACED]); flush_uniform(t_lit, &cnt->stats[sl.q][ST_LIT]); flush_uniform(t_extend, &cnt->stats[sl.q][ST_EXTEND]);
    if (CAM) flush_uniform(t_samples, &cnt->stats[sl.q][ST_SAMPLES]);
    tally_flush(tl, s_draws, cnt, sl.q);
#ifdef APT_NEAR_STATS
    flush_uniform(t_near, &cnt->stats[sl.q][14]);
#endif
#ifdef APT_ROWTOP_STATS
    if (!CAM && lane_id() == 0 && rt.rows) { atomicAdd(&cnt->stats[sl.q][12], rt.wait); atomicAdd(&cnt->stats[sl.q][13], (unsigned long long)__builtin_amdgcn_s_memtime() - rt.loop0); atomicAdd(&cnt->stats[sl.q][14], rt.rows); }
#endif
}
#endif
template <int BM, int SM, int TEX, bool CQ, bool TR = false>
APT_D void shade_staged(args3_ptr A0, Counters* cnt, const ShadeIn& in, int cur, int bounce, TransQ tq = TransQ{}) {
    const ShadeArgs3* A_ = args_fresh(A0);
    const int nxt = cur ^ 1;
    const SubLoop sl = sub_loop((A_->p).nq);
    const uint32_t n = in.counts[sl.q * CNT_PAD];
    const uint32_t qbase = (uint32_t)sl.q * (A_->p).subcap, sh_qbase = (uint32_t)sl.q * (A_->q).sh_subcap;
    uint32_t* next_counter = &cnt->n_active[nxt][sl.q * CNT_PAD];
    uint32_t* shadow_counter = &cnt->n_shadow[sl.q * CNT_PAD];
    const EmitterGeom geom = {(A_->sc).precom, (A_->sc).normals, (A_->sc).obj_info};
    __shared__ uint32_t s_draws[BLOCK / 64];
    if (lane_id() == 0) s_draws[threadIdx.x >> 6] = 0;
    ShadeTally tl = {0u, 0u, 0u};
#ifdef APT_NEAR_STATS
    uint32_t t_near = 0;
#endif
    constexpr bool PFP = TEX == 0;
    const uint32_t in_base = CQ ? (uint32_t)in.cls * (A_->p).cap + qbase : qbase;
    const float4* cqA = CQ ? (A_->q).cq[0] : nullptr; const float4* cqB = CQ ? (A_->q).cq[1] : nullptr; const float4* cqC = CQ ? (A_->q).cq[2] : nullptr; const float4* cqD = CQ ? (A_->q).cq[3] : nullptr;
    int pf_prim = -1;
    auto prefetch_prim = [&](uint32_t b) {
        const uint32_t ps = in_base + min(b + threadIdx.x, n - 1u);
        pf_prim = CQ ? ldq(reinterpret_cast<const int*>(cqB), (ps << 4) + 12u) : ldq(in.prim, ps << 2);
    };
    if (PFP && n > 0) prefetch_prim(sl.first);
    for (uint32_t base = sl.first; base < n; base += sl.stride) {
        APT_ARGS_PHASE();
        const uint32_t pos = base + threadIdx.x, idx = in_base + pos;
        bool alive = pos < n;
        const int cu_prim = pf_prim;
        float4 cu_ra = make_float4(0.f, 0.f, 0.f, 0.f), cu_rb = cu_ra;
        if (PFP) { const int rp = max(cu_prim, 0); cu_ra = (A_->sc).prim_shade[2 * rp]; cu_rb = (A_->sc).prim_shade[2 * rp + 1]; prefetch_prim(base + sl.stride); }
        Vertex vx; vertex_reset(vx);
        Philox rng; rng_init(rng, 0u, 0u, 0u, 0u);
        if (alive) {
            const uint32_t io = idx << 2;
            const int prim = PFP ? cu_prim : (CQ ? ldq(reinterpret_cast<const int*>(cqB), (idx << 4) + 12u) : ldq(in.prim, io));
            if (prim < 0) alive = false;
            else {
                uint32_t meta; float t_in, ray_pdf = 1.f; float2 uv; uv.x = uv.y = 0.f;
// ... 70 lines not shown
            stq((A_->q).id[nxt], so, vx.id);
            stq((A_->q).meta[nxt], so, pack_meta(rng.draw, (uint32_t)(bounce + 1), is_spec));
            if (SM & APT_SRC_AREA) stq((A_->q).pdf[nxt], so, new_pdf);
        }
    }
    tally_flush(tl, s_draws, cnt, sl.q);
#ifdef APT_NEAR_STATS
    flush_uniform(t_near, &cnt->stats[sl.q][14]);
#endif
}
template <int BM, int SM, int TEX = 0>
__global__ void __launch_bounds__(BLOCK) k_shade(DevScene sc, Params p, Queues q, Counters* cnt, ShadeIn in, int cur, int bounce) {
    shade_staged<BM, SM, TEX, false>(kernel_args3(), cnt, in, cur, bounce);
}
template <int BM, int SM, int TEX = 0>
__global__ void __launch_bounds__(BLOCK) k_shade_tr(DevScene sc, Params p, Queues q, Counters* cnt, ShadeIn in, int cur, int bounce, TransQ tq) {
    shade_staged<BM, SM, TEX, false, true>(kernel_args3(), cnt, in, cur, bounce, tq);
}
#if APT_FAST
template <int BM, int SM, int TEX = 0>
__global__ void __launch_bounds__(BLOCK) k_shade_traced(DevScene sc, Params p, Queues q, Counters* cnt, int cur, int bounce) {
    shade_traced<BM, SM, TEX>(kernel_args3(), cnt, cur, bounce);
}
#ifndef APT_TRACED_WAVES
#define APT_TRACED_WAVES 7
#endif
template <int BM, int SM>
__global__ void __launch_bounds__(BLOCK) __attribute__((amdgpu_waves_per_eu(APT_TRACED_WAVES, APT_TRACED_WAVES))) k_shade_traced_lean(DevScene sc, Params p, Queues q, Counters* cnt, int cur, int bounce) {
    shade_traced<BM, SM, 0>(kernel_args3(), cnt, cur, bounce);
}
template <int BM, int SM>
__global__ void __launch_bounds__(BLOCK) __attribute__((amdgpu_waves_per_eu(APT_TRACED_WAVES, APT_TRACED_WAVES))) k_shade_traced_lean_staged(DevScene sc, Params p, Queues q, Counters* cnt, int cur, int bounce) {
    shade_traced<BM, SM, 0, false, true>(kernel_args3(), cnt, cur, bounce);
}
template <int BM, int SM>
__global__ void __launch_bounds__(BLOCK) __attribute__((amdgpu_waves_per_eu(APT_TRACED_WAVES, APT_TRACED_WAVES))) k_shade_traced_lean_staged_live(DevScene sc, Params p, Queues q, Counters* cnt, int cur, int bounce) {
    shade_traced<BM, SM, 0, false, true, true>(kernel_args3(), cnt, cur, bounce);
}
template <int BM, int SM, int TEX = 0>
__global__ void __launch_bounds__(BLOCK) k_shade_traced_cam(DevScene sc, Params p, Queues q, Counters* cnt, const unsigned long long* strips) {
    shade_traced<BM, SM, TEX, true>(kernel_args3(), cnt, 0, 0, strips);
}
#ifndef APT_TRACED_CAM_WAVES
#define APT_TRACED_CAM_WAVES 7
#endif
template <int BM, int SM>
__global__ void __launch_bounds__(BLOCK) __attribute__((amdgpu_waves_per_eu(APT_TRACED_CAM_WAVES, APT_TRACED_CAM_WAVES))) k_shade_traced_lean_cam(DevScene sc, Params p, Queues q, Counters* cnt, const unsigned long long* strips) {
    shade_traced<BM, SM, 0, true>(kernel_args3(), cnt, 0, 0, strips);
}
template <int BM, int SM>
__global__ void __launch_bounds__(BLOCK) __attribute__((amdgpu_waves_per_eu(APT_TRACED_CAM_WAVES, APT_TRACED_CAM_WAVES))) k_shade_traced_lean_cam_live(DevScene sc, Params p, Queues q, Counters* cnt, const unsigned long long* strips) {
    shade_traced<BM, SM, 0, true, false, true>(kernel_args3(), cnt, 0, 0, strips);
}
#endif

#define APT_GROUP_SLOTS 6
struct GroupIn { const uint32_t* counts[APT_GROUP_SLOTS]; int cls[APT_GROUP_SLOTS]; };
template <int SM, int WAVES, int B0, int B1, int B2, int B3, int B4 = 0, int B5 = 0>
__global__ void __launch_bounds__(BLOCK, WAVES) k_shade_group(DevScene sc, Params p, Queues q, Counters* cnt, GroupIn g, int cur, int bounce) {
    ShadeIn in = {nullptr, nullptr, nullptr, nullptr, nullptr, nullptr, nullptr, nullptr, nullptr, nullptr, nullptr, 0};
    if constexpr (B0 != 0) if (g.cls[0] >= 0) { in.counts = g.counts[0]; in.cls = g.cls[0]; shade_staged<B0, SM, 0, true>(kernel_args3(), cnt, in, cur, bounce); }
    if constexpr (B1 != 0) if (g.cls[1] >= 0) { in.counts = g.counts[1]; in.cls = g.cls[1]; shade_staged<B1, SM, 0, true>(kernel_args3(), cnt, in, cur, bounce); }
    if constexpr (B2 != 0) if (g.cls[2] >= 0) { in.counts = g.counts[2]; in.cls = g.cls[2]; shade_staged<B2, SM, 0, true>(kernel_args3(), cnt, in, cur, bounce); }
    if constexpr (B4 != 0) if (g.cls[4] >= 0) { in.counts = g.counts[4]; in.cls = g.cls[4]; shade_staged<B4, SM, 0, true>(kernel_args3(), cnt, in, cur, bounce); }
    if constexpr (B5 != 0) if (g.cls[5] >= 0) { in.counts = g.counts[5]; in.cls = g.cls[5]; shade_staged<B5, SM, 0, true>(kernel_args3(), cnt, in, cur, bounce); }
    if constexpr (B3 != 0) if (g.cls[3] >= 0) { in.counts = g.counts[3]; in.cls = g.cls[3]; shade_staged<B3, SM, 0, true>(kernel_args3(), cnt, in, cur, bounce); }
}
template <int SM, int B0, int B1, int B2, int B3, int B4 = 0, int B5 = 0>
__global__ void __launch_bounds__(BLOCK) k_shade_group_tr(DevScene sc, Params p, Queues q, Counters* cnt, GroupIn g, int cur, int bounce, TransQ tq) {
    ShadeIn in = {nullptr, nullptr, nullptr, nullptr, nullptr, nullptr, nullptr, nullptr, nullptr, nullptr, nullptr, 0};
    if constexpr (B0 != 0) if (g.cls[0] >= 0) { in.counts = g.counts[0]; in.cls = g.cls[0]; shade_staged<B0, SM, 0, true, true>(kernel_args3(), cnt, in, cur, bounce, tq); }
    if constexpr (B1 != 0) if (g.cls[1] >= 0) { in.counts = g.counts[1]; in.cls = g.cls[1]; shade_staged<B1, SM, 0, true, true>(kernel_args3(), cnt, in, cur, bounce, tq); }
    if constexpr (B2 != 0) if (g.cls[2] >= 0) { in.counts = g.counts[2]; in.cls = g.cls[2]; shade_staged<B2, SM, 0, true, true>(kernel_args3(), cnt, in, cur, bounce, tq); }
    if constexpr (B4 != 0) if (g.cls[4] >= 0) { in.counts = g.counts[4]; in.cls = g.cls[4]; shade_staged<B4, SM, 0, true, true>(kernel_args3(), cnt, in, cur, bounce, tq); }
    if constexpr (B5 != 0) if (g.cls[5] >= 0) { in.counts = g.counts[5]; in.cls = g.cls[5]; shade_staged<B5, SM, 0, true, true>(kernel_args3(), cnt, in, cur, bounce, tq); }
    if constexpr (B3 != 0) if (g.cls[3] >= 0) { in.counts = g.counts[3]; in.cls = g.cls[3]; shade_staged<B3, SM, 0, true, true>(kernel_args3(), cnt, in, cur, bounce, tq); }
}
```

adapt_amd/csrc/stages.hpp:

```cpp
#pragma once
#include <hip/hip_runtime.h>

#include "rng.hpp"
#include "shading.hpp"
#include "traverse.hpp"
#include "vec.hpp"

struct DevMedium {
    int type;
    float ior;
    f3 u_s, u_a, u_e, par, pdf;
};
struct DevVolume {
    int type, xres, yres, zres;
    f3 albedo, trans, mini, maxi, majorant, pdf;
    f3 inv_r0, inv_r1, inv_r2;
    DevMedium ph;
    const float* grid;
};
struct DevScene {
    DevBvh bvh;
    SweepScene sweep;
    FlatScene flat;
    const float* normals;
// ... 167 lines not shown

struct TrAppend { uint32_t raw, rank; };
APT_D TrAppend tr_append_issue(int which, int nq_, uint32_t* counters, uint32_t stride) {
    TrAppend a; a.raw = 0u; a.rank = 0u;
    uint32_t cnt_vec = 0u;
    for (int c = 0; c < nq_; c++) {
        const unsigned long long m = __ballot(which == c);
        if (which == c) a.rank = rank_in(m);
        if ((int)lane_id() == c) cnt_vec = (uint32_t)__popcll(m);
    }
    if ((int)lane_id() < nq_ && cnt_vec) a.raw = atomicAdd(counters + (size_t)lane_id() * stride, cnt_vec);
    return a;
}
APT_D uint32_t tr_append_pos(const TrAppend& a, int which) { return (uint32_t)__shfl((int)a.raw, which < 0 ? 0 : which) + a.rank; }

APT_D void cq_store(const Queues& q, uint32_t slot, f3 o, f3 d, f3 thr, uint32_t id, uint32_t meta, float pdf, float t, int prim, float u, float v) {
    const uint32_t so = slot << 4;
    *reinterpret_cast<float4*>(reinterpret_cast<char*>(q.cq[0]) + so) = make_float4(o.x, o.y, o.z, t);
    *reinterpret_cast<float4*>(reinterpret_cast<char*>(q.cq[1]) + so) = make_float4(d.x, d.y, d.z, __int_as_float(prim));
    *reinterpret_cast<float4*>(reinterpret_cast<char*>(q.cq[2]) + so) = make_float4(thr.x, thr.y, thr.z, __uint_as_float(id));
    *reinterpret_cast<float4*>(reinterpret_cast<char*>(q.cq[3]) + so) = make_float4(__uint_as_float(meta), pdf, u, v);
}

APT_D void class_append(const Queues& q, const Params& p, Counters* cnt, int sq, uint32_t qbase, int cls, f3 o, f3 d, f3 thr, uint32_t id, uint32_t meta, float pdf, const HitRec& rec) {
    uint32_t my_rank = 0, cnt_vec = 0;
    for (int c = 0; c < q.n_classes; c++) {
        const unsigned long long m = __ballot(cls == c);
        if (cls == c) my_rank = rank_in(m);
        if ((int)lane_id() == c) cnt_vec = (uint32_t)__popcll(m);
    }
    uint32_t tail = 0;
    if ((int)lane_id() < q.n_classes && cnt_vec) tail = atomicAdd(&cnt->n_cls[lane_id()][sq * CNT_PAD], cnt_vec);
    const uint32_t cpos = (uint32_t)__shfl((int)tail, cls < 0 ? 0 : cls) + my_rank;
    if (cls >= 0) cq_store(q, (uint32_t)cls * p.cap + qbase + cpos, o, d, thr, id, meta, pdf, rec.t, rec.prim, rec.u, rec.v);
}

APT_D void begin_extend(Counters* cnt, int sq, int cur, uint32_t n) {
    cnt->n_shadow[sq * CNT_PAD] = 0; cnt->n_active[cur ^ 1][sq * CNT_PAD] = 0;
    for (int w = 0; w < 8; w++) cnt->n_walk[w][sq * CNT_PAD] = 0;
    cnt->stats[sq][ST_EXTEND] += n;
}
APT_D uint32_t shadow_count(const uint32_t* n_src, int sq, const Queues& q) { return min(n_src[sq * CNT_PAD], q.sh_subcap); }
APT_D void begin_shadow(Counters* cnt, const Queues& q, int sq, uint32_t n, bool tally = true) {
    if (tally) cnt->stats[sq][ST_SHADOW_TRACED] += n;
    for (int c = 0; c < q.n_classes; c++) cnt->n_cls[c][sq * CNT_PAD] = 0;
}

template <typename T> APT_D T ldq(const T* base, uint32_t off) { return *reinterpret_cast<const T*>(reinterpret_cast<const char*>(base) + off); }
template <typename T> APT_D void stq(T* base, uint32_t off, T v) { *reinterpret_cast<T*>(reinterpret_cast<char*>(base) + off) = v; }
typedef float rec4 __attribute__((ext_vector_type(4)));
APT_D void stage_plane(const float4* plane, uint32_t off, rec4* dst) {
    __builtin_amdgcn_global_load_lds((const __attribute__((address_space(1))) void*)(reinterpret_cast<const char*>(plane) + off), (__attribute__((address_space(3))) void*)dst, 16, 0, 0);
}
APT_D void staged_wait() { asm volatile("s_waitcnt vmcnt(0)" ::: "memory"); }
APT_D uint32_t lds_addr(const void* p) { return (uint32_t)(uintptr_t)(const __attribute__((address_space(3))) void*)p; }
APT_D void staged_read(const rec4* rec, rec4& a, rec4& b, rec4& c, rec4& d) {
    asm volatile("ds_read_b128 %0, %4\n\tds_read_b128 %1, %4 offset:1024\n\tds_read_b128 %2, %4 offset:2048\n\tds_read_b128 %3, %4 offset:3072\n\ts_waitcnt lgkmcnt(0)"
                 : "=&v"(a), "=&v"(b), "=&v"(c), "=&v"(d) : "v"(lds_addr(rec)) : "memory");
}
APT_D void staged_read2(const rec4* p, rec4& a, rec4& b) {
    asm volatile("ds_read_b128 %0, %2\n\tds_read_b128 %1, %2 offset:16\n\ts_waitcnt lgkmcnt(0)" : "=&v"(a), "=&v"(b) : "v"(lds_addr(p)) : "memory");
}
APT_D void lds_add_unordered(uint32_t* word, uint32_t v) {
    asm volatile("ds_add_u32 %0, %1" :: "v"((uint32_t)(uintptr_t)(__attribute__((address_space(3))) uint32_t*)word), "v"(v) : "memory");
}
APT_D f3 ld3q(const float* base, uint32_t stride, uint32_t off) { return mk3(ldq(base, off), ldq(base + stride, off), ldq(base + 2 * stride, off)); }
APT_D void st3q(float* base, uint32_t stride, uint32_t off, f3 v) { stq(base, off, v.x); stq(base + stride, off, v.y); stq(base + 2 * stride, off, v.z); }
APT_D uint32_t wave_count(bool flag) { return (uint32_t)__popcll(__ballot(flag)); }
APT_D void flush_uniform(uint32_t v, unsigned long long* counter) { if (lane_id() == 0 && v) atomicAdd(counter, (unsigned long long)v); }
APT_D void flush_stat(uint32_t v, unsigned long long* counter) {
    for (int off = 32; off > 0; off >>= 1) v += __shfl_down(v, off);
    if (lane_id() == 0 && v) atomicAdd(counter, (unsigned long long)v);
}

APT_D DevSrc ld_src_uniform(const DevSrc* p) {
    const ci_ptr w = (ci_ptr)reinterpret_cast<const int*>(p);
    DevSrc s; int* dst = reinterpret_cast<int*>(&s);
    for (int k = 0; k < (int)(sizeof(DevSrc) / 4); k++) dst[k] = w[k];
    return s;
}

APT_D DevSrc ld_src_lane(const DevSrc* p) {
    static_assert(sizeof(DevSrc) == 64, "DevSrc is read as four float4");
    const float4* q4 = reinterpret_cast<const float4*>(p);
    float4 a = q4[0], b = q4[1], c = q4[2], d = q4[3];
    asm volatile("" : "+v"(a.x), "+v"(a.y), "+v"(a.z), "+v"(a.w), "+v"(b.x), "+v"(b.y), "+v"(b.z), "+v"(b.w));
    asm volatile("" : "+v"(c.x), "+v"(c.y), "+v"(c.z), "+v"(c.w), "+v"(d.x), "+v"(d.y), "+v"(d.z), "+v"(d.w));
    DevSrc s;
    s.type = __float_as_int(a.x); s.bool_bits = __float_as_int(a.y); s.obj_ref_id = __float_as_int(a.z); s.prim_first = __float_as_int(a.w);
    s.intensity = mk3(b.x, b.y, b.z); s.dir = mk3(b.w, c.x, c.y); s.pos = mk3(c.z, c.w, d.x);
    s.inv_area = d.y; s.r = d.z; s.prim_count = __float_as_int(d.w);
    return s;
}

APT_D DevBxdf ld_bxdf_lane(const DevBxdf* p) {
    static_assert(sizeof(DevBxdf) == 80, "DevBxdf is read as five float4");
    const float4* q4 = reinterpret_cast<const float4*>(p);
    float4 a = q4[0], b = q4[1], c = q4[2], d = q4[3], e = q4[4];
    asm volatile("" : "+v"(a.x), "+v"(a.y), "+v"(a.z), "+v"(b.x), "+v"(b.y), "+v"(b.z), "+v"(b.w));
    asm volatile("" : "+v"(c.x), "+v"(c.y), "+v"(c.z), "+v"(c.w), "+v"(d.x), "+v"(d.y), "+v"(d.z), "+v"(d.w), "+v"(e.x));
    DevBxdf x;
    x.type = __float_as_int(a.x); x.is_delta = __float_as_int(a.y); x.is_bsdf = __float_as_int(a.z); x._pad = 0;
    x.k_d = mk3(b.x, b.y, b.z); x.k_s = mk3(b.w, c.x, c.y); x.k_g = mk3(c.z, c.w, d.x); x.mean = mk3(d.y, d.z, d.w);
    x.ior = e.x; x._pad2[0] = x._pad2[1] = x._pad2[2] = 0.f;
    return x;
}

APT_D void local_to_global(const Params& p, uint32_t lp, int& i, int& j) {
    int lc = (int)(lp / (uint32_t)p.H);
    j = (int)(lp % (uint32_t)p.H);
    int lb = lc / p.band_width, w = lc % p.band_width;
    i = (lb * p.world + p.rank) * p.band_width + w;
}

struct SubLoop { int q; uint32_t first, stride; };
APT_D SubLoop sub_loop(int nq, int nt = BLOCK) {
    SubLoop s;
    s.q = (int)(blockIdx.x % (uint32_t)nq);
    s.first = (blockIdx.x / (uint32_t)nq) * (uint32_t)nt;
    s.stride = (gridDim.x / (uint32_t)nq) * (uint32_t)nt;
    return s;
}
enum { TRACE_BVH = 0, TRACE_SWEEP = 1, TRACE_TILE = 2, TRACE_FLAT = 3, TRACE_VFLAT = 4 };
#ifndef APT_TILE_NT
#define APT_TILE_NT 512
#endif
#ifndef APT_TILE_WAVES
#define APT_TILE_WAVES 6
#endif
#define TRACE_NT(MODE) ((MODE) == TRACE_TILE ? APT_TILE_NT : BLOCK)

APT_D f3 camera_ray_dir(const Params& p, int i, int j, uint32_t s, uint32_t& draws, uint32_t* tail = nullptr) {
    int sample_cnt = p.cnt_base + (int)s + 1;
    Philox rng; rng_init(rng, (uint32_t)(i * p.H + j), p.seed, (uint32_t)sample_cnt, 0u);
    float vx = 0.5f, vy = 0.5f;
    if (p.anti_alias) {
        if (p.stratified) {
            int mod_val = pymod(sample_cnt, 16);
            vx = (float)(mod_val % 4) * 0.25f + rng_float(rng) * 0.25f;
            vy = (float)(mod_val / 4) * 0.25f + rng_float(rng) * 0.25f;
        } else {
            const float eps = 1e-4f, inv_eps = (float)(1 - 1e-4 * 2.);
            vx = rng_float(rng) * inv_eps + eps;
            vy = rng_float(rng) * inv_eps + eps;
        }
    }
    f3 cd = mk3((p.half_w + vx - (float)i) * p.inv_focal, ((float)j - p.half_h - vy) * p.inv_focal, 1.f);
    m33 R;
    for (int a = 0; a < 3; a++) for (int b = 0; b < 3; b++) R.m[a][b] = p.cam_r[3 * a + b];
    draws = rng.draw;
    if (tail) { tail[0] = rng.c[2]; tail[1] = rng.c[3]; }
    return normalize(mul(R, cd));
}
APT_D unsigned long long camera_strip_mask(const Params& p, const unsigned long long* strips, uint32_t w) {
    typedef const __attribute__((address_space(4))) unsigned long long* strip_ptr;
    const uint32_t lp0 = (uint32_t)__builtin_amdgcn_readfirstlane((int)((w * 64u) % (uint32_t)p.npix)), lp1 = lp0 + 63u, last = (uint32_t)p.npix - 1u;
    return ((strip_ptr)strips)[lp0 >> 6] | ((strip_ptr)strips)[(lp1 < last ? lp1 : last) >> 6] | ((strip_ptr)strips)[lp1 > last ? 0u : (lp0 >> 6)];
}
#ifndef APT_LIGHT_STRIP_EMITTERS
#define APT_LIGHT_STRIP_EMITTERS 16
#endif
APT_D unsigned long long light_strip_mask(const Params& p, const unsigned long long* strips, uint32_t w, int e) {
    const uint32_t n_blocks = ((uint32_t)p.npix + 63u) >> 6;
    return camera_strip_mask(p, strips + (size_t)((uint32_t)e + 1u) * n_blocks, w);
}

template <bool TRACE, bool ADAPTIVE = false>
APT_D void generate_body(const DevScene* sc, const Params& p, const Queues& q, Counters* cnt, const uint8_t* active = nullptr, const unsigned long long* strips = nullptr) {
    const uint32_t total = (uint32_t)p.npix * (uint32_t)p.spp_batch;
    const uint32_t n_waves = (total + 63u) / 64u;
    const uint32_t wave_stride = gridDim.x * (BLOCK / 64);
    uint32_t t_samples = 0, t_draws = 0;
    for (uint32_t w = blockIdx.x * (BLOCK / 64) + threadIdx.x / 64u; w < n_waves; w += wave_stride) {
        const uint32_t idx = w * 64u + lane_id();
        const int sq = (int)(w % (uint32_t)p.nq);
        bool valid = idx < total, alive = false;
        f3 dir = mk3(0.f, 0.f, 1.f);
        uint32_t draws = 0;
        if (valid) {
            uint32_t lp = idx % (uint32_t)p.npix, s = idx / (uint32_t)p.npix;
            int i, j; local_to_global(p, lp, i, j);
            for (int pl = 0; pl < p.l_planes; pl++) stL(q.L, p.cap, (idx << 2) | (uint32_t)pl, splat3(0.f));
            alive = !p.do_crop || (i >= p.sx && i < p.ex && j >= p.sy && j < p.ey);
            if (ADAPTIVE) alive = alive && active[lp] != 0;
            if (alive) {
                dir = camera_ray_dir(p, i, j, s, draws);
            }
        }
        uint32_t pos;
        uint32_t* q0_counter = &cnt->n_active[0][sq * CNT_PAD];
        if (TRACE) pos = 0;
        else if (p.do_crop || ADAPTIVE) pos = wave_append(alive, q0_counter);
        else {
            pos = (w / (uint32_t)p.nq) * 64u + lane_id();
            unsigned long long m = __ballot(alive);
            if (lane_id() == 0) atomicAdd(q0_counter, (uint32_t)__popcll(m));
        }
#if APT_FAST
        if (TRACE) {
            const f3 cam_o = mk3(p.cam_t[0], p.cam_t[1], p.cam_t[2]);
            float tr_t = 0.f; int tr_run = -1, tr_idx = -1;
            if (__any(alive)) {
                const unsigned long long mask = camera_strip_mask(p, strips, w);
                tr_idx = flat_closest1<true>(sc->flat, cam_o, dir, 1e7f, tr_t, tr_run, mask);
            }
            const bool defer = alive && (tr_run >= 0 || flat_needs_cull(sc->flat, dir));
            HitRec hr; hr.t = 1e7f; hr.prim = -1; hr.u = hr.v = 0.f;
            int hit_cls = 0;
            if (alive && !defer && tr_idx >= 0) flat_resolve(sc->flat, tr_idx, tr_t, cam_o, dir, hr, hit_cls);
            const int ocls = !alive ? -1 : (defer ? q.tr_ncls : (hr.prim >= 0 ? (q.tr_ncls > 1 ? hit_cls : 0) : -1));
            const TrAppend app = tr_append_issue(ocls, q.tr_ncls + 1, &cnt->n_tr[0][0][sq * CNT_PAD], APT_MAX_NQ * CNT_PAD);
            pos = tr_append_pos(app, ocls);
            if (alive) t_samples++;
            if (ocls >= 0) {
                const uint32_t slot = (q.tr_stage_top && ocls == q.tr_ncls) ? (uint32_t)sq * p.subcap + p.subcap - 1u - pos : (uint32_t)ocls * p.cap + (uint32_t)sq * p.subcap + pos, so = slot << 4;
                stq(q.tr[0][0], so, make_float4(cam_o.x, cam_o.y, cam_o.z, hr.t));
                stq(q.tr[0][1], so, make_float4(dir.x, dir.y, dir.z, __uint_as_float(tr_pack(hr.prim, draws, false))));
                stq(q.tr[0][2], so, make_float4(1.f, 1.f, 1.f, __uint_as_float(((idx / (uint32_t)p.npix) << p.pix_bits) | (idx % (uint32_t)p.npix))));
                stq(q.tr[0][3], so, make_float4(0.f, 0.f, 0.f, 1.f));
                if (sc->has_vn || sc->tex_i != nullptr) { float2 uv_; uv_.x = hr.u; uv_.y = hr.v; stq(q.tr_uv[0], slot << 3, uv_); }
            }
        }
#endif
        if (alive && !TRACE) {
            const uint32_t so = ((uint32_t)sq * p.subcap + pos) << 2;
            st3q(q.ray_o[0], p.cap, so, mk3(p.cam_t[0], p.cam_t[1], p.cam_t[2]));
            st3q(q.ray_d[0], p.cap, so, dir);
            st3q(q.thr[0], p.cap, so, splat3(1.f));
            stq(q.id[0], so, ((idx / (uint32_t)p.npix) << p.pix_bits) | (idx % (uint32_t)p.npix));
            stq(q.meta[0], so, pack_meta(draws, 0u, false));
            stq(q.pdf[0], so, 1.f);
            t_samples++;
        }
        t_draws += draws;
    }
    const int sq0 = (int)((blockIdx.x * (BLOCK / 64) + threadIdx.x / 64u) % (uint32_t)p.nq);
    flush_stat(t_samples, &cnt->stats[sq0][ST_SAMPLES]);
    if (TRACE) flush_stat(t_samples, &cnt->stats[sq0][ST_EXTEND]);
    flush_stat(t_draws, &cnt->stats[sq0][ST_DRAWS]);
}
__global__ void __launch_bounds__(BLOCK) k_generate(Params p, Queues q, Counters* cnt) { generate_body<false>(nullptr, p, q, cnt); }
__global__ void __launch_bounds__(BLOCK) k_generate_ad(Params p, Queues q, Counters* cnt, const uint8_t* active) { generate_body<false, true>(nullptr, p, q, cnt, active); }
#if APT_FAST
__global__ void __launch_bounds__(BLOCK) k_generate_trace(DevScene sc, Params p, Queues q, Counters* cnt, const unsigned long long* strips) { generate_body<true>(&sc, p, q, cnt, nullptr, strips); }
__global__ void __launch_bounds__(BLOCK) k_generate_trace_ad(DevScene sc, Params p, Queues q, Counters* cnt, const uint8_t* active, const unsigned long long* strips) { generate_body<true, true>(&sc, p, q, cnt, active, strips); }
#endif

template <int MODE, int SORTED>
__global__ void __launch_bounds__(TRACE_NT(MODE), (MODE == TRACE_TILE ? APT_TILE_WAVES : 1)) k_extend(DevScene sc, Params p, Queues q, Counters* cnt, int cur, const uint32_t* n_src, LdsPlan plan) {
    __shared__ float s_sweep[MODE == TRACE_SWEEP ? APT_SWEEP_LDS_FLOATS(BLOCK) : 1];
    const SubLoop sl = sub_loop(p.nq, TRACE_NT(MODE));
    const uint32_t n = n_src[sl.q * CNT_PAD];
    if (cnt && sl.first == 0 && threadIdx.x == 0) begin_extend(cnt, sl.q, cur, n);
    const float* ro = q.ray_o[cur]; const float* rd = q.ray_d[cur];
    const uint32_t qbase = (uint32_t)sl.q * p.subcap;
    for (uint32_t base = sl.first; base < n; base += sl.stride) {
        const uint32_t pos = base + threadIdx.x;
        const bool valid = pos < n;
        const uint32_t idx = qbase + (valid ? pos : n - 1);
        const uint32_t io = idx << 2;
        const f3 o = ld3q(ro, p.cap, io);
        const f3 d = ld3q(rd, p.cap, io);
        HitRec rec; rec.t = 1e7f; rec.prim = -1; rec.u = 0.f; rec.v = 0.f;
        if (MODE == TRACE_BVH) traverse<false>(sc.bvh, make_stack(plan), o, d, rec);
        else if (MODE == TRACE_SWEEP) sweep_wg<false, BLOCK>(sc.sweep, o, d, rec, valid, s_sweep);
        else sweep_tile<false, APT_TILE_NT>(sc.sweep, o, d, rec, valid, reinterpret_cast<float*>(s_dyn));
        if (!SORTED) {
            if (valid) { stq(q.hit_t, io, rec.t); stq(q.hit_prim, io, rec.prim); stq(q.hit_u, io, rec.u); stq(q.hit_v, io, rec.v); }
        } else {
            const f3 st_thr = ld3q(q.thr[cur], p.cap, io); const uint32_t st_id = ldq(q.id[cur], io), st_meta = ldq(q.meta[cur], io); const float st_pdf = ldq(q.pdf[cur], io);
            const int cls = (valid && rec.prim >= 0) ? sc.prim_class[rec.prim] : -1;
            class_append(q, p, cnt, sl.q, qbase, cls, o, d, st_thr, st_id, st_meta, st_pdf, rec);
        }
    }
}



#ifndef APT_DYN_MIN_ACTIVE_SH
#define APT_DYN_MIN_ACTIVE_SH 32
#endif
#ifndef APT_DYN_MIN_ACTIVE
#define APT_DYN_MIN_ACTIVE 32
#endif
#ifndef APT_VOTE_TRI_WEIGHT
#define APT_VOTE_TRI_WEIGHT 2
#endif
#ifndef APT_VOTE_TRI_WEIGHT_SH
#define APT_VOTE_TRI_WEIGHT_SH APT_VOTE_TRI_WEIGHT
#endif
APT_D void walk_settle(const TravStack& ts, int& sp, grp_t& ng, const grp_t& tg, int& state) {
    if (state == 1 && tg.y == 0u && !APT_GROUP_HAS_NODES(ng)) {
        if (sp == 0) state = 2; else ng = tpop(ts, sp);
    }
}
struct WalkDbg {
#ifdef APT_WALK_STATS
    uint32_t wd[8] = {0, 0, 0, 0, 0, 0, 0, 0};
// ... 537 lines not shown
```

adapt_amd/renderer.py:

```python
from __future__ import annotations

import ctypes as C
import time
from collections import namedtuple
from typing import List, Optional

import numpy as np

from . import _lib
from .scene_pack import FlatScene, RenderConfig, make_config, pack_scene
from .tiles import TilePlan

__all__ = ["Renderer", "VolumeRenderer", "DeviceScene", "bxdf_probe", "medium_probe", "volume_probe", "rng_stream", "adaptive_config", "adaptive_segments", "relative_error", "DENOISE_DEFAULTS"]

ADAPTIVE_DEFAULTS = {"min_spp": 64, "step": 32}
DENOISE_DEFAULTS = {"firefly_threshold": 0.0, "iterations": 3, "sigma_n": 128.0, "sigma_z": 0.1, "sigma_a": 0.1, "sigma_c": 1.0, "demodulate": True}
TRAVERSAL_NAMES = dict(enumerate(("bvh", "sweep", "tile", "flat")))
BVH_BUILDER_NAMES = dict(enumerate(("sah", "lbvh", "ploc")))
_Split = namedtuple("_Split", "n inner read set key missing")
SPLIT_MODES = {
    "transient": _Split("n_bins", (), "apt_read_transient", "apt_set_transient", "transient_bins",
                        "this renderer was created without transient=...: there are no time bins"),
    "path_lengths": _Split("n_lengths", (2,), "apt_read_path_lengths", "apt_set_path_lengths", "path_length_planes",
                           "this renderer was created without path_lengths=True: there are no path-length planes"),
# ... 512 lines not shown

    def intersect(self, o, d):
        o = np.ascontiguousarray(o, np.float32).reshape(-1, 3); d = np.ascontiguousarray(d, np.float32).reshape(-1, 3)
        n = o.shape[0]
        prim, t, uv = np.zeros(n, np.int32), np.zeros(n, np.float32), np.zeros((n, 2), np.float32)
        _lib.check(self.lib.apt_intersect(self.handle, n, _fp(o), _fp(d), _ip(prim), _fp(t), _fp(uv)), "apt_intersect", self.lib)
        return prim, t, uv

    def occluded(self, o, d, tmax):
        o = np.ascontiguousarray(o, np.float32).reshape(-1, 3); d = np.ascontiguousarray(d, np.float32).reshape(-1, 3)
        tmax = np.ascontiguousarray(tmax, np.float32).reshape(-1)
        occ = np.zeros(o.shape[0], np.int32)
        _lib.check(self.lib.apt_occluded(self.handle, o.shape[0], _fp(o), _fp(d), _fp(tmax), _ip(occ)), "apt_occluded", self.lib)
        return occ

    def emitter_probe(self, in11, seed: int = 0) -> np.ndarray:
        x = np.ascontiguousarray(in11, np.float32).reshape(-1, 11)
        out = np.zeros((x.shape[0], 12), np.float32)
        _lib.check(self.lib.apt_emitter_probe(self.scene.handle, x.shape[0], _fp(x), int(seed) & 0xffffffff, _fp(out)), "apt_emitter_probe", self.lib)
        return out

    def info(self) -> dict:
        b, nq, lds, tm = C.c_int32(0), C.c_int32(0), C.c_int32(0), C.c_int32(0)
        qb = C.c_int64(0)
        name = C.c_char_p()
        _lib.check(self.lib.apt_renderer_info(self.handle, C.byref(b), C.byref(nq), C.byref(qb), C.byref(lds), C.byref(name), C.byref(tm)), "apt_renderer_info", self.lib)
        bb = C.c_int32(0)
        _lib.check(self.lib.apt_scene_bvh_builder(self.scene.handle, C.byref(bb)), "apt_scene_bvh_builder", self.lib)
        return {"spp_per_batch": b.value, "n_subqueues": nq.value, "queue_bytes": qb.value, "lds_bytes": lds.value,
                "shade_variant": name.value.decode() if name.value else "",
                "traversal": TRAVERSAL_NAMES.get(tm.value, str(tm.value)), "bvh_builder": BVH_BUILDER_NAMES.get(bb.value, str(bb.value)), "arithmetic": self.arithmetic,
                "sampling": "adaptive" if self.adaptive else "uniform", **({"adaptive": dict(self.adaptive)} if self.adaptive else {})}

    def camera_fused(self) -> bool:
        f = C.c_int32(0)
        _lib.check(self.lib.apt_renderer_camera_fused(self.handle, C.byref(f)), "apt_renderer_camera_fused", self.lib)
        return bool(f.value)

    def light_strips(self) -> bool:
        f = C.c_int32(0)
        _lib.check(self.lib.apt_renderer_light_strips(self.handle, C.byref(f)), "apt_renderer_light_strips", self.lib)
        return bool(f.value)

    def record_staged(self) -> bool:
        f = C.c_int32(0)
        _lib.check(self.lib.apt_renderer_record_staged(self.handle, C.byref(f)), "apt_renderer_record_staged", self.lib)
        return bool(f.value)

    def live_rows(self) -> bool:
        f = C.c_int32(0)
        _lib.check(self.lib.apt_renderer_live_rows(self.handle, C.byref(f)), "apt_renderer_live_rows", self.lib)
        return bool(f.value)

    def get_check_point(self) -> dict:
        return {"w": self.w, "h": self.h, "crop_x": self.crop_x, "crop_y": self.crop_y, "crop_rx": self.crop_rx,
                "crop_ry": self.crop_ry, "focal": self.focal, "num_objects": self.num_objects, "num_prims": self.num_prims,
                "cam_orient": np.array(self.cam_orient), "src_num": self.src_num, "cam_t": np.array(self.cam_t),
                "accumulation": self.color.to_numpy(), "counter": self._cnt,
                **{m.key: self._read_split(mode) for mode, m in SPLIT_MODES.items() if getattr(self, m.n)},
                **({"aov_sums": self.tile_aov(), "aov_samples": self._aov_n} if self._aov_n else {}),
                **(self._adaptive_check_point() if self.adaptive else {})}

    _ADAPTIVE_KEYS = ("adaptive", "sample_counts", "moments", "active")

    def _adaptive_check_point(self) -> dict:
        n, act = self.tile_sample_counts(with_mask=True)
        return {"adaptive": dict(self.adaptive), "sample_counts": n, "moments": self.tile_moments(), "active": act}

    def load_check_point(self, check_point: dict):
        if self.adaptive and "moments" not in check_point:
            raise ValueError("this checkpoint has no per-pixel moments (a uniform render's): an adaptive renderer cannot continue it")
        if not self.adaptive and any(k in check_point for k in self._ADAPTIVE_KEYS):
            raise ValueError("this checkpoint is an adaptive render's: continue it with Renderer(..., adaptive=...)")
        for key, val in check_point.items():
            if key in ("accumulation", "counter", "aov_sums", "aov_samples") + tuple(m.key for m in SPLIT_MODES.values()) + self._ADAPTIVE_KEYS:
                continue
            if key in ("cam_t", "cam_orient"):
                ok = np.abs(np.asarray(val) - np.asarray(getattr(self, key))).max() < 1e-4
            else:
                ok = val == getattr(self, key)
            if not ok:
                raise ValueError(f"'{key}' from the checkpoint is different.")
        self._set_accum(np.asarray(check_point["accumulation"], np.float32), int(check_point["counter"]))
        if self.adaptive:
            self._set_adaptive_state(check_point["sample_counts"], check_point["moments"], check_point["active"])
        self._clear_aov()
        sums = check_point.get("aov_sums")
        if sums is not None and np.shape(sums) == (self.n_cols, self.h, 8) and 0 < int(check_point.get("aov_samples", 0)) <= min(self._cnt, self.aov_spp):
            sums = np.ascontiguousarray(sums, np.float32)
            _lib.check(self.lib.apt_set_aov(self.handle, _fp(sums)), "apt_set_aov", self.lib)
            self._aov_n = int(check_point["aov_samples"])
        for mode, m in SPLIT_MODES.items():
            cells = check_point.get(m.key)
            if getattr(self, m.n) and cells is not None and np.shape(cells) == self._split_shape(mode):
                self._set_split(mode, cells)

    def summary(self) -> str:
        self.synchronize()
        msg = f"{'VPT' if self.volumetric else 'PT'} SPP = {self._cnt}. Rendering time: {time.time() - self._t0:.3f} s"
        if self.adaptive:
            n = self.tile_sample_counts()[self._crop_mask()]
            msg += f". Adaptive: mean spp {n.mean() if n.size else 0.0:.1f}, {100.0 * (1.0 - self.active_fraction()):.1f} % of the pixels converged"
        print(msg)
        return msg

    def close(self):
# ... 16 lines not shown
```

include/adapt_mi.h:

```cpp
#ifndef ADAPT_MI_H
#define ADAPT_MI_H

#include <stdint.h>

#ifdef __cplusplus
extern "C" {
#endif

#define APT_OK            0
#define APT_E_INVALID    -1
#define APT_E_NO_DEVICE  -2
#define APT_E_HIP        -3
#define APT_E_NOMEM      -4
#define APT_E_STATE      -5

typedef struct apt_bvh apt_bvh;
typedef struct apt_scene apt_scene;
typedef struct apt_renderer apt_renderer;

typedef struct apt_scene_desc {
    int32_t n_prims, n_objects, n_sources, has_vertex_normal;
    const float*   prims;
    const float*   normals;
    const float*   v_normals;
// ... 101 lines not shown

int apt_scene_create(const apt_scene_desc* desc, int32_t device, apt_scene** out);
void apt_scene_destroy(apt_scene*);
int apt_scene_bvh_builder(const apt_scene*, int32_t* builder);
int apt_renderer_create(const apt_scene*, const apt_render_cfg* cfg, apt_renderer** out);
void apt_renderer_destroy(apt_renderer*);

int apt_render(apt_renderer*, int32_t n_spp);
int apt_synchronize(apt_renderer*);
int apt_tile_shape(const apt_renderer*, int32_t* n_cols, int32_t* height);
int apt_read_pixels(apt_renderer*, float* out);
int apt_get_accum(apt_renderer*, float* out, int32_t* cnt);
int apt_set_accum(apt_renderer*, const float* in, int32_t cnt);
int apt_reset(apt_renderer*);
int apt_read_transient(apt_renderer*, float* out);
int apt_set_transient(apt_renderer*, const float* in);
int apt_read_path_lengths(apt_renderer*, float* out);
int apt_set_path_lengths(apt_renderer*, const float* in);
int apt_read_light_groups(apt_renderer*, float* out);
int apt_set_light_groups(apt_renderer*, const float* in);
int apt_relight(apt_renderer*, const float* gains , float* out );
int apt_read_sample_counts(apt_renderer*, int32_t* counts, uint8_t* active);
int apt_read_moments(apt_renderer*, double* s2);
int apt_set_adaptive_state(apt_renderer*, const int32_t* counts, const double* s2, const uint8_t* active);
int apt_render_aov(apt_renderer*, int32_t first_sample, int32_t n_spp);
int apt_read_aov(apt_renderer*, float* out);
int apt_set_aov(apt_renderer*, const float* in);
int apt_clear_aov(apt_renderer*);
int apt_denoise(apt_renderer*, const apt_denoise_cfg* cfg, const float* colour_in, float* out);
int apt_get_stats(apt_renderer*, apt_stats* out);
int apt_device_ptr(apt_renderer*, void** accum_dev, int32_t* cnt);
int apt_stream(apt_renderer*, void** hip_stream);

int apt_intersect(apt_renderer*, int32_t n, const float* o, const float* d,
                  int32_t* prim_out, float* t_out, float* uv_out);
int apt_occluded(apt_renderer*, int32_t n, const float* o, const float* d, const float* tmax, int32_t* occ_out);
int apt_rng_stream(int32_t device, uint32_t pixel, uint32_t seed, uint32_t sample, int32_t n, uint32_t* out);
int apt_bxdf_probe(int32_t device, int32_t n, const int32_t* bxdf_i, const float* bxdf_f, const float* dirs12,
                   float world_ior, int32_t do_sample, uint32_t seed, float* out);
int apt_texture_probe(const apt_scene*, int32_t n, const int32_t* map_obj, const float* uv, float* out3);
int apt_surface_maps_probe(const apt_scene*, int32_t n, const int32_t* prim_first, const float* bary, float* out7);
int apt_medium_probe(int32_t device, int32_t n, const int32_t* med_i, const float* med_f, int32_t mode, const float* in7,
                     uint32_t seed, float* out8);
int apt_volume_probe(int32_t device, int32_t n, const int32_t* vol_i, const float* vol_f, const float* vol_grid, int32_t mode,
                     const float* in10, uint32_t seed, float* out8);
int apt_emitter_probe(const apt_scene*, int32_t n, const float* in11, uint32_t seed, float* out12);
int apt_transient_bin_probe(int32_t device, int32_t n, const float* t, float min_time, float interval, int32_t n_bins, int32_t* out);
int apt_renderer_info(const apt_renderer*, int32_t* spp_batch, int32_t* n_subqueues, int64_t* queue_bytes,
                      int32_t* lds_bytes, const char** shade_variant, int32_t* trace_mode);
int apt_renderer_camera_fused(const apt_renderer*, int32_t* fused);
int apt_renderer_light_strips(const apt_renderer*, int32_t* in_use);
int apt_renderer_record_staged(const apt_renderer*, int32_t* staged);
int apt_renderer_live_rows(const apt_renderer*, int32_t* live);

int apt_measure_sclk_mhz(int32_t device, float* mhz);

const char* apt_last_error(void);
const char* apt_version(void);

#ifdef __cplusplus
}
#endif
#endif
```

Baseline: 6401.

## Compact traced-path queue record from 64 to 56 bytes storing hit point

Adds a 56-byte record layout for the traced pipeline's lean shading kernels. It stores the hit point instead of origin plus t, moves the pixel id and one radiance component into spare lanes, and shrinks the fourth plane to a float2. The layout is used by generation, the fix prologue and the staged LDS reads, and is on by default when the lean traced kernels exist. The aim is to cut global-memory and LDS traffic per path vertex, at the cost of more template variants and index reshuffling across stages.

Result: faster. 6597 (median of 6 runs) (+3.1%).

```diff
diff --git a/adapt_amd/_lib.py b/adapt_amd/_lib.py
--- a/adapt_amd/_lib.py
+++ b/adapt_amd/_lib.py
@@ -127,6 +127,7 @@
     "apt_renderer_light_strips": (C.c_int, [C.c_void_p, i32p]),
     "apt_renderer_record_staged": (C.c_int, [C.c_void_p, i32p]),
     "apt_renderer_live_rows": (C.c_int, [C.c_void_p, i32p]),
+    "apt_renderer_record_compact": (C.c_int, [C.c_void_p, i32p]),
     "apt_measure_sclk_mhz": (C.c_int, [C.c_int32, f32p]),
     "apt_last_error": (C.c_char_p, []),
     "apt_version": (C.c_char_p, []),
diff --git a/adapt_amd/csrc/api.hip b/adapt_amd/csrc/api.hip
--- a/adapt_amd/csrc/api.hip
+++ b/adapt_amd/csrc/api.hip
@@ -34,7 +34,7 @@
 typedef void (*shade_cam_fn)(DevScene, Params, Queues, Counters*, const unsigned long long*);
 typedef void (*shade_tr_fn)(DevScene, Params, Queues, Counters*, ShadeIn, int, int, TransQ);
 struct TracedKernels { shade_traced_fn queue[2][2]; shade_cam_fn cam[2]; };
-struct ShadeVariant { int bm, sm; const char* name; shade_fn fn; shade_tr_fn transient; TracedKernels traced; };
+struct ShadeVariant { int bm, sm; const char* name; shade_fn fn; shade_tr_fn transient; TracedKernels traced, traced56; };
 #if APT_FAST
 #define APT_FLAT_FN(...) __VA_ARGS__
 #else
@@ -43,7 +43,10 @@
 #define APT_TRACED_PLAIN(BM, SM, TEX) {{{APT_FLAT_FN(k_shade_traced<BM, SM, TEX>), nullptr}, {nullptr, nullptr}}, {APT_FLAT_FN(k_shade_traced_cam<BM, SM, TEX>), nullptr}}
 #define APT_TRACED_LEAN(BM, SM, TEX) {{{APT_FLAT_FN(k_shade_traced_lean<BM, SM>), nullptr}, {APT_FLAT_FN(k_shade_traced_lean_staged<BM, SM>), APT_FLAT_FN(k_shade_traced_lean_staged_live<BM, SM>)}}, \
                                       {APT_FLAT_FN(k_shade_traced_lean_cam<BM, SM>), APT_FLAT_FN(k_shade_traced_lean_cam_live<BM, SM>)}}
-#define APT_SHADE_VARIANT(BM, SM, TEX, NAME, TRACED) {BM, SM, NAME, k_shade<BM, SM, TEX>, k_shade_tr<BM, SM, TEX>, APT_TRACED_##TRACED(BM, SM, TEX)}
+#define APT_TRACED56_PLAIN(BM, SM, TEX) {{{nullptr, nullptr}, {nullptr, nullptr}}, {nullptr, nullptr}}
+#define APT_TRACED56_LEAN(BM, SM, TEX) {{{APT_FLAT_FN(k_shade_traced_lean56<BM, SM>), nullptr}, {APT_FLAT_FN(k_shade_traced_lean56_staged<BM, SM>), APT_FLAT_FN(k_shade_traced_lean56_staged_live<BM, SM>)}}, \
+                                        {APT_FLAT_FN(k_shade_traced_lean56_cam<BM, SM>), APT_FLAT_FN(k_shade_traced_lean56_cam_live<BM, SM>)}}
+#define APT_SHADE_VARIANT(BM, SM, TEX, NAME, TRACED) {BM, SM, NAME, k_shade<BM, SM, TEX>, k_shade_tr<BM, SM, TEX>, APT_TRACED_##TRACED(BM, SM, TEX), APT_TRACED56_##TRACED(BM, SM, TEX)}
 static const ShadeVariant kShadeVariants[] = {
     APT_SHADE_VARIANT(APT_BX_LAMBERTIAN, APT_SRC_POINT, 0, "lambertian/point", LEAN),
     APT_SHADE_VARIANT(APT_BX_BLINN_PHONG | APT_BX_LAMBERTIAN, APT_SRC_POINT_AREA, 0, "phong+lambertian/point+area", PLAIN),
@@ -224,6 +227,7 @@
     shade_traced_fn traced_fn = nullptr;
     int live_rows = 0;
     shade_cam_fn traced_cam_fn = nullptr;
+    int record_compact = 0;
     int camera_fuse = 0;
     int light_strips = 0;
     Counters host_counters{};
@@ -757,8 +761,10 @@
 }
 
 static void pick_traced_kernels(apt_renderer* r) {
-    const TracedKernels& t = r->shade->traced;
     const bool traced = r->pipeline == PIPE_TRACED;
+    const bool want_compact = !(getenv("APT_RECORD_COMPACT") && atoi(getenv("APT_RECORD_COMPACT")) == 0);
+    r->record_compact = (traced && want_compact && r->shade->traced56.queue[0][0] != nullptr) ? 1 : 0;
+    const TracedKernels& t = r->record_compact ? r->shade->traced56 : r->shade->traced;
     const bool want_stage = !(getenv("APT_RECORD_STAGE") && atoi(getenv("APT_RECORD_STAGE")) == 0);
     const bool want_live = !(getenv("APT_LIVE_ROWS") && atoi(getenv("APT_LIVE_ROWS")) == 0);
     r->record_stage = (traced && want_stage && t.queue[1][0] != nullptr) ? 1 : 0;
@@ -926,7 +932,7 @@
         for (int k = 0; k < 2; k++) { q.ray_o[k] = (k == 0 || staged) ? take(3 * cap) : nullptr; q.ray_d[k] = (k == 0 || staged) ? take(3 * cap) : nullptr; }
         q.hit_t = take(cap); q.hit_prim = (int*)take(cap); q.hit_u = take(cap); q.hit_v = take(cap);
         for (int k = 0; k < 2; k++) {
-            for (int a = 0; a < 4; a++) q.tr[k][a] = staged ? nullptr : (float4*)take(4 * cap);
+            for (int a = 0; a < 4; a++) q.tr[k][a] = staged ? nullptr : (float4*)take((a == 3 && r->record_compact ? 2 : 4) * cap);
             q.tr_uv[k] = tr_uv ? (float2*)take(2 * cap) : nullptr;
         }
         q.tr_ncls = staged ? 0 : 1; q.tr_stage_top = staged ? 0 : 1;
@@ -1374,8 +1380,8 @@
                 cur = 1; b0 = 1;
             } else {
                 LaunchTimer t(r, APT_K_GENERATE, st);
-                if (r->adaptive) hipLaunchKernelGGL(k_generate_trace_ad, dim3(grid_for(total, r->grid_small, 1)), dim3(BLOCK), 0, st, sc, p, q, cnt, (const uint8_t*)r->aq.active, strips);
-                else hipLaunchKernelGGL(k_generate_trace, dim3(grid_for(total, r->grid_small, 1)), dim3(BLOCK), 0, st, sc, p, q, cnt, strips);
+                if (r->adaptive) hipLaunchKernelGGL(r->record_compact ? k_generate_trace56_ad : k_generate_trace_ad, dim3(grid_for(total, r->grid_small, 1)), dim3(BLOCK), 0, st, sc, p, q, cnt, (const uint8_t*)r->aq.active, strips);
+                else hipLaunchKernelGGL(r->record_compact ? k_generate_trace56 : k_generate_trace, dim3(grid_for(total, r->grid_small, 1)), dim3(BLOCK), 0, st, sc, p, q, cnt, strips);
             }
             for (int b = b0; b < p.max_bounce; b++) {
                 { LaunchTimer t(r, APT_K_SHADE, st); hipLaunchKernelGGL(r->traced_fn, dim3(grid_for(total, r->grid_small, nq)), dim3(BLOCK), 0, st, sc, p, q, cnt, cur, b); }
@@ -2004,6 +2010,11 @@
     *out = r->live_rows;
     return APT_OK;
 }
+APT_EXPORT int apt_renderer_record_compact(const apt_renderer* r, int32_t* out) {
+    if (!r || !out) return fail(APT_E_INVALID, "apt_renderer_record_compact: null argument");
+    *out = r->record_compact;
+    return APT_OK;
+}
 APT_EXPORT int apt_renderer_info(const apt_renderer* r, int32_t* spp_batch, int32_t* n_subqueues, int64_t* queue_bytes, int32_t* lds_bytes, const char** shade_variant, int32_t* trace_mode) {
     if (!r) return fail(APT_E_INVALID, "apt_renderer_info: null handle");
     if (spp_batch) *spp_batch = r->spp_batch;
diff --git a/adapt_amd/csrc/shade_stage.hpp b/adapt_amd/csrc/shade_stage.hpp
--- a/adapt_amd/csrc/shade_stage.hpp
+++ b/adapt_amd/csrc/shade_stage.hpp
@@ -35,10 +35,12 @@
     return applied;
 }
 
+template <bool AT = false>
 APT_D void build_hit_rec(const DevScene& sc, float4 ra, float4 rb, int prim, float t, float u, float v, f3 o, f3 d, Hit& it, int& hit_light, f3& k_d, bool with_vn = true);
 APT_D void build_hit(const DevScene& sc, int prim, float t, float u, float v, f3 o, f3 d, Hit& it, int& hit_light, f3& k_d) {
     build_hit_rec(sc, sc.prim_shade[2 * prim], sc.prim_shade[2 * prim + 1], prim, t, u, v, o, d, it, hit_light, k_d);
 }
+template <bool AT>
 APT_D void build_hit_rec(const DevScene& sc, float4 ra, float4 rb, int prim, float t, float u, float v, f3 o, f3 d, Hit& it, int& hit_light, f3& k_d, bool with_vn) {
     const int code = __float_as_int(ra.w);
     it.prim_id = prim; it.min_depth = t;
@@ -46,7 +48,7 @@
     hit_light = __float_as_int(rb.x);
     k_d = mk3(rb.y, rb.z, rb.w);
     if (code < 0) {
-        it.n_g = normalize((o + d * t) - mk3(ra.x, ra.y, ra.z));
+        it.n_g = normalize((AT ? o : (o + d * t)) - mk3(ra.x, ra.y, ra.z));
         it.n_s = it.n_g;
     } else {
         it.n_g = mk3(ra.x, ra.y, ra.z);
@@ -61,7 +63,9 @@
 }
 
 #if APT_FAST
+template <bool C56 = false>
 APT_D void fix_prologue(const DevScene& sc, const Params& p, const Queues& q, Counters* cnt, int cur, int sq, int bounce) {
+    typedef TrRecord<C56> Rec;
     const uint32_t epoch = (uint32_t)bounce + 1u;
     const int ncls = q.tr_ncls;
     uint32_t* n_def_p = &cnt->n_tr[bounce % 3][ncls][sq * CNT_PAD]; uint32_t* n_sh_p = &cnt->n_fix_sh[cur ^ 1][sq * CNT_PAD];
@@ -82,22 +86,29 @@
     for (uint32_t base = 0; base < n_def; base += 64u) {
         const uint32_t li = base + lane_id(); const bool valid = li < n_def;
         const uint32_t lj = valid ? li : n_def - 1u;
-        const uint32_t io = (q.tr_stage_top ? qbase + p.subcap - n_def + lj : (uint32_t)ncls * p.cap + qbase + lj) << 4;
-        const float4 ra = ldq(q.tr[cur][0], io), rb = ldq(q.tr[cur][1], io), rc = ldq(q.tr[cur][2], io), rd = ldq(q.tr[cur][3], io);
-        const f3 o = mk3(ra.x, ra.y, ra.z), d = mk3(rb.x, rb.y, rb.z);
+        const uint32_t is = q.tr_stage_top ? qbase + p.subcap - n_def + lj : (uint32_t)ncls * p.cap + qbase + lj, io = is << 4;
+        const float4 ra = ldq(q.tr[cur][0], io), rb = ldq(q.tr[cur][1], io), rc = ldq(q.tr[cur][2], io);
+        float4 rd = make_float4(0.f, 0.f, 0.f, 0.f);
+        if (!C56 || bounce > 0) rd = Rec::load_d(q.tr[cur][3], is);
+        const f3 o = mk3(ra.x, ra.y, ra.z), d = mk3(rb.x, rb.y, rb.z), lc = Rec::Lc(rc, rd);
         HitRec r0, r1; r0.t = r1.t = 1e7f; r0.prim = r1.prim = -1; r0.u = r0.v = r1.u = r1.v = 0.f;
         int c0, c1;
         flat_closest2(sc.flat, sc.sweep, sc.prim_class, o, d, o, d, r0, r1, c0, c1);
         if (valid && r0.prim >= 0) {
             const int oc = ncls > 1 ? c0 : 0;
             const uint32_t pos = atomicAdd(&cnt->n_tr[bounce % 3][oc][sq * CNT_PAD], 1u);
-            const uint32_t slot = (uint32_t)oc * p.cap + qbase + pos, so = slot << 4;
-            stq(q.tr[cur][0], so, make_float4(ra.x, ra.y, ra.z, r0.t));
-            stq(q.tr[cur][1], so, make_float4(rb.x, rb.y, rb.z, __uint_as_float((__float_as_uint(rb.w) & ~0xffu) | (uint32_t)r0.prim)));
-            stq(q.tr[cur][2], so, rc); stq(q.tr[cur][3], so, rd);
+            const uint32_t slot = (uint32_t)oc * p.cap + qbase + pos;
+            if constexpr (C56) {
+                auto pm = [pm0 = Rec::pm(ra, rb), prim = r0.prim] { return (pm0 & ~0xffu) | (uint32_t)prim; };
+                Rec::put_a(q.tr[cur][0], slot, hit_point_of(o, d, r0.t), r0.t, pm); Rec::put_b(q.tr[cur][1], slot, d, pm, Rec::id(rb, rc));
+            } else {
+                stq(q.tr[cur][0], slot << 4, make_float4(ra.x, ra.y, ra.z, r0.t));
+                stq(q.tr[cur][1], slot << 4, make_float4(rb.x, rb.y, rb.z, __uint_as_float((__float_as_uint(rb.w) & ~0xffu) | (uint32_t)r0.prim)));
+            }
+            Rec::copy_c(q.tr[cur][2], slot, rc); if (!C56 || bounce > 0) Rec::copy_d(q.tr[cur][3], slot, rd);
             if (need_uv) { float2 uv_; uv_.x = r0.u; uv_.y = r0.v; stq(q.tr_uv[cur], slot << 3, uv_); }
-        } else if (valid && !(rd.x == 0.f && rd.y == 0.f && rd.z == 0.f)) {
-            add_radiance(q.L, p.cap, radiance_slot(p, __float_as_uint(rc.w)), mk3(rd.x, rd.y, rd.z), true);
+        } else if (valid && !(lc.x == 0.f && lc.y == 0.f && lc.z == 0.f)) {
+            add_radiance(q.L, p.cap, radiance_slot(p, Rec::id(rb, rc)), lc, true);
         }
     }
     uint32_t t_lit = 0;
@@ -285,24 +296,36 @@
 #if APT_FAST
 APT_D uint32_t row_lane(uint32_t b, uint32_t n) { return min(b + threadIdx.x, n - 1u); }
 struct RecordPlanes { const float4 *a, *b, *c, *d; };
-APT_D uint32_t prefetch_prim(const RecordPlanes& tr, uint32_t qbase, uint32_t b, uint32_t n) { return ldq(reinterpret_cast<const uint32_t*>(tr.b), ((qbase + row_lane(b, n)) << 4) + 12u); }
+template <bool C56 = false>
+APT_D uint32_t prefetch_prim(const RecordPlanes& tr, uint32_t qbase, uint32_t b, uint32_t n) { return ldq(TrRecord<C56>::pm_plane(tr.a, tr.b), ((qbase + row_lane(b, n)) << 4) + 12u); }
 struct StagedRecord { rec4* rec; rec4* prim; };
+template <bool C56 = false>
 APT_D StagedRecord staged_record_open(const ShadeArgs3* A_) {
-    __shared__ rec4 s_stage[(BLOCK / 64) * 4 * 64]; __shared__ rec4 s_shade[2 * APT_FLAT_MAX_PRIMS];
+    constexpr int WAVE_RECS = C56 ? 3 * 64 + 32 : 4 * 64;
+    __shared__ rec4 s_stage[(BLOCK / 64) * WAVE_RECS]; __shared__ rec4 s_shade[2 * APT_FLAT_MAX_PRIMS];
     static_assert(2 * APT_FLAT_MAX_PRIMS <= BLOCK, "one shading-record word per thread");
     if ((int)threadIdx.x < 2 * min((A_->sc).n_prims, APT_FLAT_MAX_PRIMS)) { const float4 w_ = (A_->sc).prim_shade[threadIdx.x]; s_shade[threadIdx.x] = rec4{w_.x, w_.y, w_.z, w_.w}; }
     __syncthreads();
-    return StagedRecord{s_stage + (threadIdx.x >> 6) * (4 * 64), s_shade};
-}
+    return StagedRecord{s_stage + (C56 ? 0 : (threadIdx.x >> 6) * WAVE_RECS), s_shade};
+}
+template <bool C56 = false>
 APT_D void stage_row(const StagedRecord& s, const RecordPlanes& tr, uint32_t qbase, uint32_t b, uint32_t n, int bounce) {
     const uint32_t off = (qbase + row_lane(b, n)) << 4;
+    if constexpr (C56) {
+        rec4* row = s.rec + (threadIdx.x >> 6) * 64;
+        stage_plane(tr.a, off, row); stage_plane(tr.b, off, row + BLOCK); stage_plane(tr.c, off, row + 2 * BLOCK);
+        if (bounce > 0) { float* w_ = reinterpret_cast<float*>(s.rec + 3 * BLOCK) + (threadIdx.x >> 6) * 64; stage_word(reinterpret_cast<const float*>(tr.d), off >> 1, w_); stage_word(reinterpret_cast<const float*>(tr.d), (off >> 1) + 4u, w_ + BLOCK); }
+        return;
+    }
     stage_plane(tr.a, off, s.rec); stage_plane(tr.b, off, s.rec + 64); stage_plane(tr.c, off, s.rec + 128);
     if (bounce > 0) stage_plane(tr.d, off, s.rec + 192);
 }
+template <bool C56 = false>
 APT_D void staged_row_read(const StagedRecord& s, float4& a, float4& b, float4& c, float4& d, float4& ra, float4& rb) {
     rec4 sa, sb, sc_, sd, pa, pb;
-    staged_read(s.rec + lane_id(), sa, sb, sc_, sd);
-    staged_read2(s.prim + 2 * max(tr_prim(__float_as_uint(sb.w)), 0), pa, pb);
+    if constexpr (C56) { float d0, d1; staged_read56(s.rec, sa, sb, sc_, d0, d1); sd = rec4{d0, d1, 0.f, 0.f}; }
+    else staged_read(s.rec + lane_id(), sa, sb, sc_, sd);
+    staged_read2(s.prim + 2 * max(tr_prim(__float_as_uint(C56 ? sa.w : sb.w)), 0), pa, pb);
     a = make_float4(sa.x, sa.y, sa.z, sa.w); b = make_float4(sb.x, sb.y, sb.z, sb.w); c = make_float4(sc_.x, sc_.y, sc_.z, sc_.w); d = make_float4(sd.x, sd.y, sd.z, sd.w);
     ra = make_float4(pa.x, pa.y, pa.z, pa.w); rb = make_float4(pb.x, pb.y, pb.z, pb.w);
 }
@@ -315,27 +338,34 @@
 #endif
 }
 template <bool UNORDERED> APT_D void tally_draws(uint32_t* s_draws, uint32_t n) { if constexpr (UNORDERED) lds_add_unordered(&s_draws[threadIdx.x >> 6], n); else atomicAdd(&s_draws[threadIdx.x >> 6], n); }
-APT_D void unpack_record(float4 a, float4 b, float4 c, Vertex& vx) { vx.o = mk3(a.x, a.y, a.z); vx.d = mk3(b.x, b.y, b.z); vx.thr = mk3(c.x, c.y, c.z); vx.id = __float_as_uint(c.w); }
-template <int BM, int SM, int TEX, bool REC, typename RNG>
+template <bool C56 = false>
+APT_D void unpack_record(float4 a, float4 b, float4 c, Vertex& vx) {
+    if constexpr (C56) vx.hit_point = mk3(a.x, a.y, a.z); else vx.o = mk3(a.x, a.y, a.z);
+    vx.d = mk3(b.x, b.y, b.z); vx.thr = mk3(c.x, c.y, c.z); vx.id = TrRecord<C56>::id(b, c);
+}
+template <int BM, int SM, int TEX, bool REC, bool C56 = false, typename RNG>
 APT_D bool open_record(const ShadeArgs3* A_, Vertex& vx, RNG& rng, float4 a, float4 b, float4 c, uint32_t pm, float4 ra, float4 rb, int cur, uint32_t idx, float ray_pdf, int bounce) {
-    unpack_record(a, b, c, vx);
+    static_assert(!C56 || REC, "the 56-byte record's kernels hold the hit primitive's shading record");
+    unpack_record<C56>(a, b, c, vx);
     const int prim = tr_prim(pm);
     if (prim < 0) return false;
     f3 rec_kd; float2 uv; uv.x = uv.y = 0.f;
     if ((A_->sc).has_vn || (TEX && (A_->sc).tex_i != nullptr)) uv = ldq((A_->q).tr_uv[cur], idx << 3);
-    if (REC) build_hit_rec((A_->sc), ra, rb, prim, a.w, uv.x, uv.y, vx.o, vx.d, vx.it, vx.hit_light, rec_kd);
+    if constexpr (C56) build_hit_rec<true>((A_->sc), ra, rb, prim, 0.f, uv.x, uv.y, vx.hit_point, vx.d, vx.it, vx.hit_light, rec_kd);
+    else if (REC) build_hit_rec((A_->sc), ra, rb, prim, a.w, uv.x, uv.y, vx.o, vx.d, vx.it, vx.hit_light, rec_kd);
     else build_hit((A_->sc), prim, a.w, uv.x, uv.y, vx.o, vx.d, vx.it, vx.hit_light, rec_kd);
     return open_vertex<BM, SM, TEX>(A_, vx, rng, prim, rec_kd, tr_meta(pm, (uint32_t)bounce), ray_pdf, uv, bounce);
 }
-template <int BM, int SM, typename RNG>
+template <int BM, int SM, bool C56 = false, typename RNG>
 APT_D bool open_record_live(const ShadeArgs3* A_, Vertex& vx, RNG& rng, float4 a, float4 b, float4 c, float4 d, float4 ra, float4 rb, int cur, uint32_t idx, int bounce, bool alive, uint32_t* s_draws, f3& Lc) {
-    if (bounce > 0) Lc = mk3(d.x, d.y, d.z);
-    unpack_record(a, b, c, vx);
-    const uint32_t pm = __float_as_uint(b.w); const int prim = tr_prim(pm);
+    if (bounce > 0) Lc = TrRecord<C56>::Lc(c, d);
+    unpack_record<C56>(a, b, c, vx);
+    const uint32_t pm = TrRecord<C56>::pm(a, b); const int prim = tr_prim(pm);
     alive = alive && prim >= 0;
     f3 rec_kd; float2 uv; uv.x = uv.y = 0.f;
     if ((A_->sc).has_vn) { if (alive) uv = ldq((A_->q).tr_uv[cur], idx << 3); }
-    build_hit_rec((A_->sc), ra, rb, max(prim, 0), a.w, uv.x, uv.y, vx.o, vx.d, vx.it, vx.hit_light, rec_kd);
+    if constexpr (C56) build_hit_rec<true>((A_->sc), ra, rb, max(prim, 0), 0.f, uv.x, uv.y, vx.hit_point, vx.d, vx.it, vx.hit_light, rec_kd);
+    else build_hit_rec((A_->sc), ra, rb, max(prim, 0), a.w, uv.x, uv.y, vx.o, vx.d, vx.it, vx.hit_light, rec_kd);
     const bool opened = alive; alive = open_vertex_live<BM, SM>(A_, vx, rng, rec_kd, pm, bounce, alive);
     if (opened && !alive && rng.draw != vx.draw0) tally_draws<true>(s_draws, rng.draw - vx.draw0);
     return alive;
@@ -353,21 +383,23 @@
     return valid && (c_run >= 0 || flat_needs_cull((A_->sc).flat, dir));
 }
 struct StagedRayWords { float t; int prim; float u, v, one, zero, one_d; };
-template <typename Words>
+template <bool C56 = false, typename Words>
 APT_D void stage_camera_ray(const ShadeArgs3* A_, Counters* cnt, int q, uint32_t qbase, bool c_defer, f3 cam_o, f3 dir, uint32_t draws, uint32_t id, Words&& words) {
     if (!__any(c_defer)) return;
     const int ncls = (A_->q).tr_ncls; const uint32_t dpos = wave_append(c_defer, &cnt->n_tr[0][ncls][q * CNT_PAD]);
     if (c_defer) {
-        const uint32_t slot = (A_->q).tr_stage_top ? qbase + (A_->p).subcap - 1u - dpos : (uint32_t)ncls * (A_->p).cap + qbase + dpos, so = slot << 4;
+        const uint32_t slot = (A_->q).tr_stage_top ? qbase + (A_->p).subcap - 1u - dpos : (uint32_t)ncls * (A_->p).cap + qbase + dpos;
         const StagedRayWords w = words();
-        stq((A_->q).tr[0][0], so, make_float4(cam_o.x, cam_o.y, cam_o.z, w.t));
-        stq((A_->q).tr[0][1], so, make_float4(dir.x, dir.y, dir.z, __uint_as_float(tr_pack(w.prim, draws, false))));
-        stq((A_->q).tr[0][2], so, make_float4(w.one, w.one, w.one, __uint_as_float(id)));
-        stq((A_->q).tr[0][3], so, make_float4(w.zero, w.zero, w.zero, w.one_d));
+        typedef TrRecord<C56> Rec;
+        auto pm = [&] { return tr_pack(w.prim, draws, false); };
+        Rec::put_a((A_->q).tr[0][0], slot, cam_o, w.t, pm);
+        Rec::put_b((A_->q).tr[0][1], slot, dir, pm, id);
+        Rec::put_c((A_->q).tr[0][2], slot, mk3(w.one, w.one, w.one), id, mk3(w.zero, w.zero, w.zero));
+        if constexpr (!C56) Rec::put_d((A_->q).tr[0][3], slot, mk3(w.zero, w.zero, w.zero), w.one_d);
         if ((A_->sc).has_vn || (A_->sc).tex_i != nullptr) { float2 uv_; uv_.x = w.u; uv_.y = w.v; stq((A_->q).tr_uv[0], slot << 3, uv_); }
     }
 }
-template <int BM, int SM, int TEX, bool WINDOW, typename RNG>
+template <int BM, int SM, int TEX, bool WINDOW, bool C56 = false, typename RNG>
 APT_D bool camera_vertex(const ShadeArgs3* A_, Counters* cnt, int q, uint32_t qbase, uint32_t pos, bool in_row, uint32_t cam_total, const unsigned long long* strips, Vertex& vx, RNG& rng, uint32_t* s_draws, uint32_t& t_samples, uint32_t& t_extend, bool& entry) {
     const uint32_t w = cam_wave(A_, pos, q), id_ = w * 64u + lane_id(); const bool valid = in_row && id_ < cam_total;
     f3 dir = mk3(0.f, 0.f, 1.f); uint32_t draws = 0, jitter_tail[2] = {0u, 0u};
@@ -379,10 +411,12 @@
     HitRec hr; hr.t = 1e7f; hr.prim = -1; hr.u = hr.v = 0.f;
     if (valid && !c_defer && c_idx >= 0) flat_resolve((A_->sc).flat, c_idx, c_t, cam_o, dir, hr, hit_cls);
     { const uint32_t nv = wave_count(valid); t_samples += nv; t_extend += nv; }
-    stage_camera_ray(A_, cnt, q, qbase, c_defer, cam_o, dir, draws, vx.id, [&] {
+    stage_camera_ray<C56>(A_, cnt, q, qbase, c_defer, cam_o, dir, draws, vx.id, [&] {
         float one = 1.f;
-        if (WINDOW) asm volatile("" : "+v"(one));
-        return StagedRayWords{hr.t, hr.prim, hr.u, hr.v, 1.f, 0.f, one};
+        if (WINDOW && !C56) asm volatile("" : "+v"(one));
+        float zero = 0.f;
+        if constexpr (C56) { if (WINDOW) asm volatile("" : "+v"(zero)); }
+        return StagedRayWords{hr.t, C56 ? -1 : hr.prim, hr.u, hr.v, 1.f, zero, one};
     });
     entry = valid && !c_defer; bool alive = entry && hr.prim >= 0;
     if (alive) {
@@ -393,7 +427,7 @@
     }
     return alive;
 }
-template <int BM, int SM, bool WINDOW, typename RNG>
+template <int BM, int SM, bool WINDOW, bool C56 = false, typename RNG>
 APT_D bool camera_vertex_live(const ShadeArgs3* A_, Counters* cnt, int q, uint32_t qbase, uint32_t pos, bool in_row, uint32_t cam_total, const unsigned long long* strips, Vertex& vx, RNG& rng, uint32_t* s_draws, uint32_t& t_samples, uint32_t& t_extend, bool& entry) {
     const uint32_t w = cam_wave(A_, pos, q), id_ = w * 64u + lane_id(); const bool valid = in_row && id_ < cam_total;
     uint32_t draws = 0, jitter_tail[2] = {0u, 0u}, s; int i, j;
@@ -406,9 +440,10 @@
     HitRec hr;
     flat_resolve((A_->sc).flat, max(c_idx, 0), c_t, cam_o, dir, hr, hit_cls);
     { const uint32_t nv = wave_count(valid); t_samples += nv; t_extend += nv; }
-    stage_camera_ray(A_, cnt, q, qbase, c_defer, cam_o, dir, draws, vx.id, [&] {
+    stage_camera_ray<C56>(A_, cnt, q, qbase, c_defer, cam_o, dir, draws, vx.id, [&] {
         float one = 1.f, far_ = 1e7f, zero = 0.f;
-        asm volatile("" : "+v"(one), "+v"(far_), "+v"(zero));
+        if constexpr (C56) asm volatile("" : "+v"(one), "+v"(zero));
+        else asm volatile("" : "+v"(one), "+v"(far_), "+v"(zero));
         return StagedRayWords{far_, -1, zero, zero, one, zero, one};
     });
     entry = valid && !c_defer; bool alive = entry && c_idx >= 0 && hr.prim >= 0;
@@ -476,22 +511,42 @@
     }
     t_traced += wave_count(f.want); t_lit += wave_count(traced && !occ);
 }
+template <bool C56 = false, bool TURN = false>
 APT_D void append_record(const ShadeArgs3* A_, int nxt, uint32_t qbase, uint32_t* next_counter, const Continuation& ct, bool cont, const Vertex& vx, f3 new_d, uint32_t draw, bool is_spec, f3 Lc, float new_pdf) {
     uint32_t npos = (uint32_t)__builtin_amdgcn_readlane((int)ct.app.raw, 0) + ct.app.rank;
+    auto pm = [&] { return tr_pack(ct.hit, draw, is_spec); };
+    if constexpr (C56) {
+        typedef TrRecord<true> Rec;
+        if (__any(ct.q == 1)) {
+            const uint32_t dpos = wave_append(ct.q == 1, next_counter + APT_MAX_NQ * CNT_PAD);
+            if (ct.q == 1) { npos = TURN ? (A_->p).subcap - 1u - dpos : dpos; Rec::put_a((A_->q).tr[nxt][0], qbase + (A_->p).subcap - 1u - dpos, vx.hit_point, ct.t, [&] { return tr_pack(-1, draw, is_spec); }); }
+        }
+        const uint32_t slot = (!TURN && ct.q == 1) ? qbase + (A_->p).subcap - 1u - npos : qbase + npos;
+        float t_hit = ct.t;
+        asm volatile("" : "+v"(t_hit));
+        if (ct.q == 0) Rec::put_a((A_->q).tr[nxt][0], slot, hit_point_of(vx.hit_point, new_d, t_hit), t_hit, [&] { return (uint32_t)ct.hit | ((draw & 0xffffu) << 8) | (is_spec ? (1u << 24) : 0u); });
+        if (cont) {
+            Rec::put_b((A_->q).tr[nxt][1], slot, new_d, pm, vx.id);
+            Rec::put_c((A_->q).tr[nxt][2], slot, vx.thr, vx.id, Lc); Rec::put_d((A_->q).tr[nxt][3], slot, Lc, new_pdf);
+            if ((A_->sc).has_vn || (A_->sc).tex_i != nullptr) { float2 uv_; uv_.x = ct.u; uv_.y = ct.v; stq((A_->q).tr_uv[nxt], slot << 3, uv_); }
+        }
+        return;
+    }
     if (__any(ct.q == 1)) { const uint32_t dpos = wave_append(ct.q == 1, next_counter + APT_MAX_NQ * CNT_PAD); if (ct.q == 1) npos = dpos; }
     if (cont) {
-        const uint32_t slot = (ct.q == 1) ? qbase + (A_->p).subcap - 1u - npos : qbase + npos, so = slot << 4;
-        stq((A_->q).tr[nxt][0], so, make_float4(vx.hit_point.x, vx.hit_point.y, vx.hit_point.z, ct.t));
-        stq((A_->q).tr[nxt][1], so, make_float4(new_d.x, new_d.y, new_d.z, __uint_as_float(tr_pack(ct.hit, draw, is_spec))));
-        stq((A_->q).tr[nxt][2], so, make_float4(vx.thr.x, vx.thr.y, vx.thr.z, __uint_as_float(vx.id)));
-        stq((A_->q).tr[nxt][3], so, make_float4(Lc.x, Lc.y, Lc.z, new_pdf));
+        const uint32_t slot = (ct.q == 1) ? qbase + (A_->p).subcap - 1u - npos : qbase + npos;
+        typedef TrRecord<false> Rec;
+        Rec::put_a((A_->q).tr[nxt][0], slot, vx.hit_point, ct.t, pm); Rec::put_b((A_->q).tr[nxt][1], slot, new_d, pm, vx.id);
+        Rec::put_c((A_->q).tr[nxt][2], slot, vx.thr, vx.id, Lc); Rec::put_d((A_->q).tr[nxt][3], slot, Lc, new_pdf);
         if ((A_->sc).has_vn || (A_->sc).tex_i != nullptr) { float2 uv_; uv_.x = ct.u; uv_.y = ct.v; stq((A_->q).tr_uv[nxt], slot << 3, uv_); }
     }
 }
 APT_D void end_path(const ShadeArgs3* A_, bool ended, uint32_t id, f3 Lc) { if (ended && !(Lc.x == 0.f && Lc.y == 0.f && Lc.z == 0.f)) add_radiance((A_->q).L, (A_->p).cap, radiance_slot((A_->p), id), Lc, true); }
-template <int BM, int SM, int TEX, bool CAM = false, bool STAGE = false, bool LIVE_ = false>
+template <int BM, int SM, int TEX, bool CAM = false, bool STAGE = false, bool LIVE_ = false, bool C56 = false>
 APT_D void shade_traced(args3_ptr A0, Counters* cnt, int cur_, int bounce_, const unsigned long long* strips = nullptr) {
     static_assert(!(CAM && STAGE), "a camera-fed row loads no record");
+    static_assert(!C56 || (TEX == 0 && BM == APT_BX_LAMBERTIAN && !(SM & APT_SRC_AREA)), "the 56-byte record: Lambertian surfaces, no area light - nobody reads the ray's origin, its hit distance or its pdf");
+    typedef TrRecord<C56> Rec;
     static_assert(!LIVE_ || ((CAM || STAGE) && TEX == 0), "live rows: the staged and the camera-fed form of the lean kernels");
     constexpr bool LIVE = LIVE_ && APT_DRAW_WINDOW != 0;
     const ShadeArgs3* A_ = args_fresh(A0);
@@ -514,19 +569,19 @@
     static_assert(APT_FLAT_MAX_PRIMS < (int)TR_NO_PRIM, "the packed record keeps the hit primitive in 8 bits");
     const RecordPlanes tr = {(A_->q).tr[cur][0], (A_->q).tr[cur][1], (A_->q).tr[cur][2], (A_->q).tr[cur][3]};
     StagedRecord stage = {nullptr, nullptr};
-    if constexpr (STAGE) stage = staged_record_open(A_);
+    if constexpr (STAGE) stage = staged_record_open<C56>(A_);
     uint32_t n, cam_total = 0;
     if constexpr (CAM) {
         cam_total = (uint32_t)(A_->p).npix * (uint32_t)(A_->p).spp_batch;
         const uint32_t n_waves = (cam_total + 63u) / 64u, nq_ = (uint32_t)(A_->p).nq;
         n = n_waves > (uint32_t)sl.q ? ((n_waves - (uint32_t)sl.q + nq_ - 1u) / nq_) * 64u : 0u;
     } else {
-        fix_prologue((A_->sc), (A_->p), (A_->q), cnt, cur, sl.q, bounce);
+        fix_prologue<C56>((A_->sc), (A_->p), (A_->q), cnt, cur, sl.q, bounce);
         n = __hip_atomic_load(&cnt->n_tr[bounce % 3][0][sl.q * CNT_PAD], __ATOMIC_RELAXED, __HIP_MEMORY_SCOPE_AGENT);
     }
     uint32_t pf_pm = 0;
-    if (PFP && n > 0) pf_pm = prefetch_prim(tr, qbase, sl.first, n);
-    if (STAGE && sl.first < n) { stage_row(stage, tr, qbase, sl.first, n, bounce); staged_wait_stamped(rt, false); }
+    if (PFP && n > 0) pf_pm = prefetch_prim<C56>(tr, qbase, sl.first, n);
+    if (STAGE && sl.first < n) { stage_row<C56>(stage, tr, qbase, sl.first, n, bounce); staged_wait_stamped(rt, false); }
 #ifdef APT_ROWTOP_STATS
     rt.loop0 = __builtin_amdgcn_s_memtime();
 #endif
@@ -535,36 +590,39 @@
         const uint32_t pos = base + threadIdx.x, idx = qbase + pos;
         bool alive = pos < n;
         const uint32_t cu_pm = pf_pm; float4 cu_ra = make_float4(0.f, 0.f, 0.f, 0.f), cu_rb = cu_ra;
-        if (PFP) { const int rp = max(tr_prim(cu_pm), 0); cu_ra = (A_->sc).prim_shade[2 * rp]; cu_rb = (A_->sc).prim_shade[2 * rp + 1]; pf_pm = prefetch_prim(tr, qbase, base + sl.stride, n); }
+        if (PFP) { const int rp = max(tr_prim(cu_pm), 0); cu_ra = (A_->sc).prim_shade[2 * rp]; cu_rb = (A_->sc).prim_shade[2 * rp + 1]; pf_pm = prefetch_prim<C56>(tr, qbase, base + sl.stride, n); }
         Vertex vx; vertex_reset(vx); Rng rng; rng_init(rng, 0u, 0u, 0u, 0u);
         f3 Lc = splat3(0.f);
         bool entry = alive; float ray_pdf = 1.f;
-        if constexpr (CAM && LIVE) alive = camera_vertex_live<BM, SM, WINDOW>(A_, cnt, sl.q, qbase, pos, alive, cam_total, strips, vx, rng, s_draws, t_samples, t_extend, entry);
-        else if constexpr (CAM) alive = camera_vertex<BM, SM, TEX, WINDOW>(A_, cnt, sl.q, qbase, pos, alive, cam_total, strips, vx, rng, s_draws, t_samples, t_extend, entry);
+        if constexpr (CAM && LIVE) alive = camera_vertex_live<BM, SM, WINDOW, C56>(A_, cnt, sl.q, qbase, pos, alive, cam_total, strips, vx, rng, s_draws, t_samples, t_extend, entry);
+        else if constexpr (CAM) alive = camera_vertex<BM, SM, TEX, WINDOW, C56>(A_, cnt, sl.q, qbase, pos, alive, cam_total, strips, vx, rng, s_draws, t_samples, t_extend, entry);
         else if constexpr (STAGE) {
             float4 a, b_, c, d;
-            staged_row_read(stage, a, b_, c, d, cu_ra, cu_rb);
-            if constexpr (LIVE) alive = open_record_live<BM, SM>(A_, vx, rng, a, b_, c, d, cu_ra, cu_rb, cur, idx, bounce, alive, s_draws, Lc);
+            staged_row_read<C56>(stage, a, b_, c, d, cu_ra, cu_rb);
+            if constexpr (LIVE) alive = open_record_live<BM, SM, C56>(A_, vx, rng, a, b_, c, d, cu_ra, cu_rb, cur, idx, bounce, alive, s_draws, Lc);
             else if (alive) {
-                if (bounce > 0) { Lc = mk3(d.x, d.y, d.z); if (SM & APT_SRC_AREA) ray_pdf = d.w; }
-                alive = open_record<BM, SM, TEX, true>(A_, vx, rng, a, b_, c, __float_as_uint(b_.w), cu_ra, cu_rb, cur, idx, ray_pdf, bounce);
+                if (bounce > 0) { Lc = Rec::Lc(c, d); if (SM & APT_SRC_AREA) ray_pdf = d.w; }
+                alive = open_record<BM, SM, TEX, true, C56>(A_, vx, rng, a, b_, c, Rec::pm(a, b_), cu_ra, cu_rb, cur, idx, ray_pdf, bounce);
             }
         } else {
-            if (alive && bounce > 0) { const float4 d = ldq(tr.d, idx << 4); Lc = mk3(d.x, d.y, d.z); if (SM & APT_SRC_AREA) ray_pdf = d.w; }
+            if constexpr (!C56) if (alive && bounce > 0) { const float4 d = Rec::load_d(tr.d, idx); Lc = Rec::Lc(d, d); if (SM & APT_SRC_AREA) ray_pdf = d.w; }
             if (alive) {
                 const float4 a = ldq(tr.a, idx << 4), b_ = ldq(tr.b, idx << 4), c = ldq(tr.c, idx << 4);
+                if constexpr (C56) if (bounce > 0) Lc = Rec::Lc(c, Rec::load_d(tr.d, idx));
 #ifdef APT_ROWTOP_STATS
                 staged_wait_stamped(rt, true);
 #endif
-                alive = open_record<BM, SM, TEX, PFP>(A_, vx, rng, a, b_, c, PFP ? cu_pm : __float_as_uint(b_.w), cu_ra, cu_rb, cur, idx, ray_pdf, bounce);
+                alive = open_record<BM, SM, TEX, PFP, C56>(A_, vx, rng, a, b_, c, PFP ? cu_pm : Rec::pm(a, b_), cu_ra, cu_rb, cur, idx, ray_pdf, bounce);
             }
         }
         tl.shade += wave_count(alive);
 #ifdef APT_NEAR_STATS
-        t_near += wave_count(alive && bounce > 0 && vx.it.min_depth < 2e-3f);
-#endif
-        if constexpr (LIVE) vx.hit_point = vx.d * vx.it.min_depth + vx.o;
-        else if (alive) vx.hit_point = vx.d * vx.it.min_depth + vx.o;
+        if constexpr (!C56) t_near += wave_count(alive && bounce > 0 && vx.it.min_depth < 2e-3f);
+#endif
+        if constexpr (!C56 || CAM) {
+            if constexpr (LIVE) vx.hit_point = hit_point_of(vx.o, vx.d, vx.it.min_depth);
+            else if (alive) vx.hit_point = hit_point_of(vx.o, vx.d, vx.it.min_depth);
+        }
         APT_ARGS_PHASE();
         bool break_flag = false; DevSrc src_only;
         if ((A_->sc).n_sources == 1) src_only = ld_src_uniform((A_->sc).src);
@@ -574,7 +632,7 @@
         if (f.poisoned) Lc = splat3(f.mis_w);
         tl.shadow += wave_count(f.sampled); tl.poison += wave_count(f.poisoned);
         const int occ_e = pick_occluder_list(A_, f);
-        if constexpr (STAGE) if (base + sl.stride < n) stage_row(stage, tr, qbase, base + sl.stride, n, bounce);
+        if constexpr (STAGE) if (base + sl.stride < n) stage_row<C56>(stage, tr, qbase, base + sl.stride, n, bounce);
         APT_ARGS_PHASE();
         bool cont, is_spec = false; float new_pdf = 1.f; f3 new_d = mk3(0.f, 1.f, 0.f);
         if constexpr (LIVE) cont = scatter_live<BM, SM, STAGE>(A_, vx, rng, alive, bounce, s_draws, Lc, new_d, new_pdf, is_spec);
@@ -584,7 +642,10 @@
         APT_ARGS_PHASE();
         sweep_light_sample<CAM>(A_, cnt, vx, f, occ_e, cur, sl.q, sh_qbase, pos, strips, Lc, t_traced, t_lit);
         if constexpr (STAGE) staged_wait_stamped(rt, true);
-        append_record(A_, nxt, qbase, next_counter, ct, cont, vx, new_d, rng.draw, is_spec, Lc, new_pdf);
+#ifdef APT_NEAR_STATS
+        if constexpr (C56) t_near += wave_count(cont && ct.q == 0 && ct.t < 2e-3f);
+#endif
+        append_record<C56, C56 && CAM && !LIVE>(A_, nxt, qbase, next_counter, ct, cont, vx, new_d, rng.draw, is_spec, Lc, new_pdf);
         end_path(A_, !cont && entry, vx.id, Lc);
     }
     flush_uniform(t_traced, &cnt->stats[sl.q][ST_SHADOW_TRACED]); flush_uniform(t_lit, &cnt->stats[sl.q][ST_LIT]); flush_uniform(t_extend, &cnt->stats[sl.q][ST_EXTEND]);
@@ -761,6 +822,12 @@
 __global__ void __launch_bounds__(BLOCK) __attribute__((amdgpu_waves_per_eu(APT_TRACED_CAM_WAVES, APT_TRACED_CAM_WAVES))) k_shade_traced_lean_cam_live(DevScene sc, Params p, Queues q, Counters* cnt, const unsigned long long* strips) {
     shade_traced<BM, SM, 0, true, false, true>(kernel_args3(), cnt, 0, 0, strips);
 }
+#define APT_LEAN56_KERNEL(NAME, WAVES) template <int BM, int SM> __global__ void __launch_bounds__(BLOCK) __attribute__((amdgpu_waves_per_eu(WAVES, WAVES))) NAME
+APT_LEAN56_KERNEL(k_shade_traced_lean56, APT_TRACED_WAVES)(DevScene sc, Params p, Queues q, Counters* cnt, int cur, int bounce) { shade_traced<BM, SM, 0, false, false, false, true>(kernel_args3(), cnt, cur, bounce); }
+APT_LEAN56_KERNEL(k_shade_traced_lean56_staged, APT_TRACED_WAVES)(DevScene sc, Params p, Queues q, Counters* cnt, int cur, int bounce) { shade_traced<BM, SM, 0, false, true, false, true>(kernel_args3(), cnt, cur, bounce); }
+APT_LEAN56_KERNEL(k_shade_traced_lean56_staged_live, APT_TRACED_WAVES)(DevScene sc, Params p, Queues q, Counters* cnt, int cur, int bounce) { shade_traced<BM, SM, 0, false, true, true, true>(kernel_args3(), cnt, cur, bounce); }
+APT_LEAN56_KERNEL(k_shade_traced_lean56_cam, APT_TRACED_CAM_WAVES)(DevScene sc, Params p, Queues q, Counters* cnt, const unsigned long long* strips) { shade_traced<BM, SM, 0, true, false, false, true>(kernel_args3(), cnt, 0, 0, strips); }
+APT_LEAN56_KERNEL(k_shade_traced_lean56_cam_live, APT_TRACED_CAM_WAVES)(DevScene sc, Params p, Queues q, Counters* cnt, const unsigned long long* strips) { shade_traced<BM, SM, 0, true, false, true, true>(kernel_args3(), cnt, 0, 0, strips); }
 #endif
 
 #define APT_GROUP_SLOTS 6
diff --git a/adapt_amd/csrc/stages.hpp b/adapt_amd/csrc/stages.hpp
--- a/adapt_amd/csrc/stages.hpp
+++ b/adapt_amd/csrc/stages.hpp
@@ -243,12 +243,22 @@
 APT_D void stage_plane(const float4* plane, uint32_t off, rec4* dst) {
     __builtin_amdgcn_global_load_lds((const __attribute__((address_space(1))) void*)(reinterpret_cast<const char*>(plane) + off), (__attribute__((address_space(3))) void*)dst, 16, 0, 0);
 }
+APT_D void stage_word(const float* plane, uint32_t off, float* dst) {
+    __builtin_amdgcn_global_load_lds((const __attribute__((address_space(1))) void*)(reinterpret_cast<const char*>(plane) + off), (__attribute__((address_space(3))) void*)dst, 4, 0, 0);
+}
 APT_D void staged_wait() { asm volatile("s_waitcnt vmcnt(0)" ::: "memory"); }
 APT_D uint32_t lds_addr(const void* p) { return (uint32_t)(uintptr_t)(const __attribute__((address_space(3))) void*)p; }
 APT_D void staged_read(const rec4* rec, rec4& a, rec4& b, rec4& c, rec4& d) {
     asm volatile("ds_read_b128 %0, %4\n\tds_read_b128 %1, %4 offset:1024\n\tds_read_b128 %2, %4 offset:2048\n\tds_read_b128 %3, %4 offset:3072\n\ts_waitcnt lgkmcnt(0)"
                  : "=&v"(a), "=&v"(b), "=&v"(c), "=&v"(d) : "v"(lds_addr(rec)) : "memory");
 }
+APT_D void staged_read56(const rec4* area, rec4& a, rec4& b, rec4& c, float& d0, float& d1) {
+    uint32_t at16, at4;
+    asm volatile("v_lshl_add_u32 %5, %7, 4, %8\n\tv_lshl_add_u32 %6, %7, 2, %8\n\t"
+                 "ds_read_b128 %0, %5\n\tds_read_b128 %1, %5 offset:%9\n\tds_read_b128 %2, %5 offset:%10\n\tds_read_b32 %3, %6 offset:%11\n\tds_read_b32 %4, %6 offset:%12\n\ts_waitcnt lgkmcnt(0)"
+                 : "=&v"(a), "=&v"(b), "=&v"(c), "=&v"(d0), "=&v"(d1), "=&v"(at16), "=&v"(at4)
+                 : "v"(threadIdx.x), "s"(lds_addr(area)), "i"(16 * BLOCK), "i"(32 * BLOCK), "i"(48 * BLOCK), "i"(52 * BLOCK) : "memory");
+}
 APT_D void staged_read2(const rec4* p, rec4& a, rec4& b) {
     asm volatile("ds_read_b128 %0, %2\n\tds_read_b128 %1, %2 offset:16\n\ts_waitcnt lgkmcnt(0)" : "=&v"(a), "=&v"(b) : "v"(lds_addr(p)) : "memory");
 }
@@ -257,6 +267,36 @@
 }
 APT_D f3 ld3q(const float* base, uint32_t stride, uint32_t off) { return mk3(ldq(base, off), ldq(base + stride, off), ldq(base + 2 * stride, off)); }
 APT_D void st3q(float* base, uint32_t stride, uint32_t off, f3 v) { stq(base, off, v.x); stq(base + stride, off, v.y); stq(base + 2 * stride, off, v.z); }
+APT_D f3 hit_point_of(f3 o, f3 d, float t) { return d * t + o; }
+template <bool C56> struct TrRecord {
+    static constexpr uint32_t D_BYTES = C56 ? 8u : 16u;
+    APT_D static float4 load_d(const float4* d, uint32_t slot) {
+        if constexpr (C56) { const float2 v = ldq(reinterpret_cast<const float2*>(d), slot << 3); return make_float4(v.x, v.y, 0.f, 0.f); }
+        else return ldq(d, slot << 4);
+    }
+    APT_D static const uint32_t* pm_plane(const float4* a, const float4* b) { return reinterpret_cast<const uint32_t*>(C56 ? a : b); }
+    APT_D static uint32_t pm(float4 a, float4 b) { return __float_as_uint(C56 ? a.w : b.w); }
+    APT_D static uint32_t id(float4 b, float4 c) { return __float_as_uint(C56 ? b.w : c.w); }
+    APT_D static f3 Lc(float4 c, float4 d) { if constexpr (C56) return mk3(c.w, d.x, d.y); else return mk3(d.x, d.y, d.z); }
+    template <typename PM> APT_D static void put_a(float4* plane, uint32_t slot, f3 p, float t, PM&& pm) {
+        const uint32_t so = slot << 4;
+        if constexpr (C56) stq(plane, so, make_float4(p.x, p.y, p.z, __uint_as_float(pm()))); else stq(plane, so, make_float4(p.x, p.y, p.z, t));
+    }
+    template <typename PM> APT_D static void put_b(float4* plane, uint32_t slot, f3 d, PM&& pm, uint32_t id) {
+        if constexpr (C56) stq(plane, slot << 4, make_float4(d.x, d.y, d.z, __uint_as_float(id))); else stq(plane, slot << 4, make_float4(d.x, d.y, d.z, __uint_as_float(pm())));
+    }
+    APT_D static void put_c(float4* plane, uint32_t slot, f3 thr, uint32_t id, f3 Lc) { stq(plane, slot << 4, make_float4(thr.x, thr.y, thr.z, C56 ? Lc.x : __uint_as_float(id))); }
+    APT_D static void copy_a(float4* plane, uint32_t slot, float4 a) { stq(plane, slot << 4, a); }
+    APT_D static void copy_c(float4* plane, uint32_t slot, float4 c) { stq(plane, slot << 4, c); }
+    APT_D static void copy_d(float4* plane, uint32_t slot, float4 d) {
+        if constexpr (C56) { float2 d_; d_.x = d.x; d_.y = d.y; stq(reinterpret_cast<float2*>(plane), slot << 3, d_); }
+        else stq(plane, slot << 4, d);
+    }
+    APT_D static void put_d(float4* plane, uint32_t slot, f3 Lc, float pdf) {
+        if constexpr (C56) { float2 d_; d_.x = Lc.y; d_.y = Lc.z; stq(reinterpret_cast<float2*>(plane), slot << 3, d_); }
+        else stq(plane, slot << 4, make_float4(Lc.x, Lc.y, Lc.z, pdf));
+    }
+};
 APT_D uint32_t wave_count(bool flag) { return (uint32_t)__popcll(__ballot(flag)); }
 APT_D void flush_uniform(uint32_t v, unsigned long long* counter) { if (lane_id() == 0 && v) atomicAdd(counter, (unsigned long long)v); }
 APT_D void flush_stat(uint32_t v, unsigned long long* counter) {
@@ -356,7 +396,7 @@
     return camera_strip_mask(p, strips + (size_t)((uint32_t)e + 1u) * n_blocks, w);
 }
 
-template <bool TRACE, bool ADAPTIVE = false>
+template <bool TRACE, bool ADAPTIVE = false, bool C56 = false>
 APT_D void generate_body(const DevScene* sc, const Params& p, const Queues& q, Counters* cnt, const uint8_t* active = nullptr, const unsigned long long* strips = nullptr) {
     const uint32_t total = (uint32_t)p.npix * (uint32_t)p.spp_batch;
     const uint32_t n_waves = (total + 63u) / 64u;
@@ -404,11 +444,14 @@
             pos = tr_append_pos(app, ocls);
             if (alive) t_samples++;
             if (ocls >= 0) {
-                const uint32_t slot = (q.tr_stage_top && ocls == q.tr_ncls) ? (uint32_t)sq * p.subcap + p.subcap - 1u - pos : (uint32_t)ocls * p.cap + (uint32_t)sq * p.subcap + pos, so = slot << 4;
-                stq(q.tr[0][0], so, make_float4(cam_o.x, cam_o.y, cam_o.z, hr.t));
-                stq(q.tr[0][1], so, make_float4(dir.x, dir.y, dir.z, __uint_as_float(tr_pack(hr.prim, draws, false))));
-                stq(q.tr[0][2], so, make_float4(1.f, 1.f, 1.f, __uint_as_float(((idx / (uint32_t)p.npix) << p.pix_bits) | (idx % (uint32_t)p.npix))));
-                stq(q.tr[0][3], so, make_float4(0.f, 0.f, 0.f, 1.f));
+                const uint32_t slot = (q.tr_stage_top && ocls == q.tr_ncls) ? (uint32_t)sq * p.subcap + p.subcap - 1u - pos : (uint32_t)ocls * p.cap + (uint32_t)sq * p.subcap + pos;
+                const f3 rec_p = (C56 && ocls != q.tr_ncls) ? hit_point_of(cam_o, dir, hr.t) : cam_o;
+                typedef TrRecord<C56> Rec;
+                auto pm = [&] { return tr_pack(hr.prim, draws, false); };
+                Rec::put_a(q.tr[0][0], slot, rec_p, hr.t, pm);
+                Rec::put_b(q.tr[0][1], slot, dir, pm, ((idx / (uint32_t)p.npix) << p.pix_bits) | (idx % (uint32_t)p.npix));
+                Rec::put_c(q.tr[0][2], slot, splat3(1.f), ((idx / (uint32_t)p.npix) << p.pix_bits) | (idx % (uint32_t)p.npix), splat3(0.f));
+                if constexpr (!C56) Rec::put_d(q.tr[0][3], slot, splat3(0.f), 1.f);
                 if (sc->has_vn || sc->tex_i != nullptr) { float2 uv_; uv_.x = hr.u; uv_.y = hr.v; stq(q.tr_uv[0], slot << 3, uv_); }
             }
         }
@@ -435,6 +478,8 @@
 #if APT_FAST
 __global__ void __launch_bounds__(BLOCK) k_generate_trace(DevScene sc, Params p, Queues q, Counters* cnt, const unsigned long long* strips) { generate_body<true>(&sc, p, q, cnt, nullptr, strips); }
 __global__ void __launch_bounds__(BLOCK) k_generate_trace_ad(DevScene sc, Params p, Queues q, Counters* cnt, const uint8_t* active, const unsigned long long* strips) { generate_body<true, true>(&sc, p, q, cnt, active, strips); }
+__global__ void __launch_bounds__(BLOCK) k_generate_trace56(DevScene sc, Params p, Queues q, Counters* cnt, const unsigned long long* strips) { generate_body<true, false, true>(&sc, p, q, cnt, nullptr, strips); }
+__global__ void __launch_bounds__(BLOCK) k_generate_trace56_ad(DevScene sc, Params p, Queues q, Counters* cnt, const uint8_t* active, const unsigned long long* strips) { generate_body<true, true, true>(&sc, p, q, cnt, active, strips); }
 #endif
 
 template <int MODE, int SORTED>
diff --git a/adapt_amd/renderer.py b/adapt_amd/renderer.py
--- a/adapt_amd/renderer.py
+++ b/adapt_amd/renderer.py
@@ -588,6 +588,11 @@
         _lib.check(self.lib.apt_renderer_live_rows(self.handle, C.byref(f)), "apt_renderer_live_rows", self.lib)
         return bool(f.value)
 
+    def record_compact(self) -> bool:
+        f = C.c_int32(0)
+        _lib.check(self.lib.apt_renderer_record_compact(self.handle, C.byref(f)), "apt_renderer_record_compact", self.lib)
+        return bool(f.value)
+
     def get_check_point(self) -> dict:
         return {"w": self.w, "h": self.h, "crop_x": self.crop_x, "crop_y": self.crop_y, "crop_rx": self.crop_rx,
                 "crop_ry": self.crop_ry, "focal": self.focal, "num_objects": self.num_objects, "num_prims": self.num_prims,
diff --git a/include/adapt_mi.h b/include/adapt_mi.h
--- a/include/adapt_mi.h
+++ b/include/adapt_mi.h
@@ -177,6 +177,7 @@
 int apt_renderer_light_strips(const apt_renderer*, int32_t* in_use);
 int apt_renderer_record_staged(const apt_renderer*, int32_t* staged);
 int apt_renderer_live_rows(const apt_renderer*, int32_t* live);
+int apt_renderer_record_compact(const apt_renderer*, int32_t* compact);
 
 int apt_measure_sclk_mhz(int32_t device, float* mhz);
 
```
